# Runki2018/litehandnet

Hardware: AMD Instinct MI355X
Metric: images/sec fwd+bwd @256x256 bs64 litehandnet (higher is better)
Workload: dtype f32; 1 GPU; litehandnet variant B (MSRB hourglass litehourglass.py) C=128, 256x256x3 -> 21x64x64, per-GPU batch 64, train-mode BN, fwd + TopdownHeatmapLoss + bwd + fused Adam; global_batch=64, parallelism=dp1

## Files before the change

### include/lhn.h

```cpp
#ifndef LHN_H
#define LHN_H
#include <stdint.h>
#ifdef __cplusplus
extern "C" {
#endif

#define LHN_VERSION 3
#define LHN_STAT_REPLICAS 32

typedef struct lhn_view {
  float*       data;
  const float* table;
  const float* gate;
  int32_t N, H, W;
  int32_t cstride;
  int32_t coff;
  int32_t C;
  const void* pend;
} lhn_view;

typedef struct lhn_gradview {
  const float* dz;
  const float* dpool;
  const float* coef;
// ... 190 lines not shown
                   void* stream);

int lhn_att_mlp_fwd(const float* pooled, const float* gamma, const float* beta, float* rmean, float* rvar,
                    int64_t* nbt, const float* w3 , const float* b3, const float* wl ,
                    const float* bl, const float* dropmask , float* gate, int gate_stride,
                    int gate_coff, float* save, int N, int C, float eps, float momentum, int training, int stage,
                    double* gsum, double count_scale, void* stream);
int lhn_att_mlp_bwd(const float* pooled, const float* gamma, const float* beta, const float* w3, const float* wl,
                    const float* dropmask, float* save, const float* dgate , float* dpool, int cstride,
                    int coff, int H, int W, float* dgamma, float* dbeta, float* dw3, float* db3, float* dwl,
                    float* dbl, int N, int C, int stage, double* gsum, double count_scale, float pgrad_scale,
                    void* stream);

int lhn_se_mlp_fwd(const float* pooled, const float* w1 , const float* b1, const float* w2 ,
                   const float* b2, float* gate, int gate_stride, int gate_coff, float* save, int N, int C, int J,
                   void* stream);
int lhn_se_mlp_fwd2(const float* pooled, const float* w1, const float* b1, const float* w2, const float* b2, float* gate,
                    int gate_stride, int gate_coff, float* save, int N, int C, int J, int mode, void* stream);
int lhn_se_mlp_bwd2(const float* pooled, const float* w1, const float* w2, const float* save, const float* dgate,
                    float* dpool, int cstride, int coff, int H, int W, float* dw1, float* db1, float* dw2, float* db2, int N,
                    int C, int J, int mode, void* stream);
int lhn_se_mlp_bwd(const float* pooled, const float* w1, const float* w2, const float* save, const float* dgate ,
                   float* dpool , int cstride, int coff, int H, int W, float* dw1, float* db1, float* dw2,
                   float* db2, int N, int C, int J, void* stream);

int lhn_bn_bwd_reduce(const lhn_view* y, const lhn_gradview* g, const float* save_mean_invstd,
                      double* sums , const lhn_bnbwdfin* fin , void* stream);
int lhn_bn_bwd_finalize(const double* sums, const float* gamma, const float* save_mean_invstd,
                        float* coef, int cstride, int coff, int C, double count, float* dgamma, float* dbeta,
                        float pgrad_scale , void* stream);
int lhn_bn_bwd_finalize2(const double* sums, const float* gamma, const float* save_mean_invstd, float* coef, int cstride,
                         int coff, int C, int stat_channels, double count, float* dgamma, float* dbeta, float pgrad_scale,
                         void* stream);
int lhn_conv_pw_bwd(const lhn_view* x, const float* w, const lhn_view* y, const lhn_gradview* gy,
                    float* dx , int dx_accumulate, float* dw,
                    float* dbias, int stride, const float* dy_nchw, int nrep, int64_t rep_stride, void* stream);
int lhn_conv_pw_bwd2(const lhn_view* x, const float* w, const lhn_view* y, const lhn_gradview* gy, float* dx,
                     int dx_accumulate, float* dw, float* dbias, int stride, const float* dy_nchw, int nrep, int64_t rep_stride,
                     const lhn_pw_opts* opts, void* stream);
int lhn_conv_dw_bwd(const lhn_view* x, const float* w, const lhn_view* y, const lhn_gradview* gy, float* dx,
                    int dx_accumulate, float* dw, int k, int stride, int pad, int dil, int nrep, int64_t rep_stride,
                    void* stream);
int lhn_conv_dw_bwd2(const lhn_view* x, const float* w, const lhn_view* y, const lhn_gradview* gy, float* dx, int dx_accumulate,
                     float* dw, int k, int stride, int pad, int dil, int nrep, int64_t rep_stride, double* bn_sums,
                     const float* bn_save, int bn_C, int bn_coff, void* stream);
int lhn_conv_dw_bwd3(const lhn_view* x, const float* w, const lhn_view* y, const lhn_gradview* gy, float* dx, int dx_accumulate,
                     float* dw, int k, int stride, int pad, int dil, int nrep, int64_t rep_stride, const float* dx_add0,
                     const float* dx_add1, void* stream);
int lhn_conv_stem_bwd(const float* img, const lhn_view* y, const lhn_gradview* gy, float* dw, int Hi, int Wi,
                      int k, int stride, int pad, int nrep, int64_t rep_stride, void* stream);
int lhn_conv_kxk_bwd(const lhn_view* x, const float* w, const lhn_view* y, const lhn_gradview* gy, float* dx,
                     int dx_accumulate, float* dw, int stride, int nrep, int64_t rep_stride,
                     float* wt_scratch , void* stream);
int lhn_plan_run_range(void* plan, int phase, int64_t step_begin, int64_t step_end, void* workspace,
                       void* const* params, void* const* grads, void* const* io, int training, int grad_replicas,
                       int64_t grad_rep_stride, double count_scale, float pgrad_scale, void* stream);
int lhn_fold_stat_replicas(double* stats, int64_t n, int nrep, void* stream);
int lhn_reduce_replicas(float* out, const float* part, int64_t n, int nrep, int64_t rep_stride, void* stream);
int lhn_ew_bwd(const lhn_view* srcs, int nsrc, const lhn_view* dst, const float* ddst, float out_slope,
               float* const* dsrcs, const int* accumulate, void* stream);
int lhn_ew_bwd2(const lhn_view* src, const lhn_view* dst, const float* ddst, const float* dst_dpool, float out_slope,
                float* dsrc, int accumulate, void* stream);
int lhn_maxpool2_bwd(const lhn_view* x, const lhn_view* y, const float* dy, float* dx, int dx_accumulate,
                     void* stream);
int lhn_maxpool2_bwd2(const lhn_view* x, const lhn_view* y, const float* dy, float* dx, int dx_accumulate, const lhn_bnsum* bns,
                      void* stream);
int lhn_maxpool2_bwd3(const lhn_view* x, const lhn_view* y, const float* dy, float* dx, int dx_accumulate, const lhn_bnsum* bns,
                      const lhn_grad_adds* adds , void* stream);
int lhn_ew_bwd3(const lhn_view* src, const lhn_view* dst, const float* ddst, const float* dst_dpool, float out_slope, float* dsrc,
                int accumulate, const lhn_bnsum* bns, void* stream);
int lhn_ew_bwd_multi(const lhn_view* srcs, int nsrc, const lhn_view* dst, const float* ddst, const float* dst_dpool, float out_slope,
                     float* const* dsrcs, const int* accumulate, const lhn_bnsum* const* bns, void* stream);
int lhn_avgpool_bwd3(const lhn_view* x, const float* dout, int OH, int OW, int out_cstride, int out_coff, float* dx,
                     int dx_accumulate, const lhn_bnsum* bns, void* stream);
int lhn_conv_pw_bwd3(const lhn_view* x, const float* w, const lhn_view* y, const lhn_gradview* gy, float* dx, int dx_accumulate,
                     float* dw, float* dbias, int stride, const float* dy_nchw, int nrep, int64_t rep_stride,
                     const lhn_pw_opts* opts, const lhn_bnsum* bns , void* stream);
int lhn_conv_dw_bwd4(const lhn_view* x, const float* w, const lhn_view* y, const lhn_gradview* gy, float* dx, int dx_accumulate,
                     float* dw, int k, int stride, int pad, int dil, int nrep, int64_t rep_stride, const lhn_bnsum* bns,
                     const float* dx_add0, const float* dx_add1, const lhn_bnbwdsrc* fin, void* stream);
int lhn_conv_pw_bwd4(const lhn_view* x, const float* w, const lhn_view* y, const lhn_gradview* gy, float* dx, int dx_accumulate,
                     float* dw, float* dbias, int stride, const float* dy_nchw, int nrep, int64_t rep_stride,
                     const lhn_pw_opts* opts, const lhn_bnsum* bns, const lhn_bnbwdsrc* fin, void* stream);
int lhn_avgpool_bwd(const lhn_view* x, const float* dout , int OH, int OW, float* dx,
                    int dx_accumulate, void* stream);
int lhn_gate_bwd_reduce(const lhn_view* y, const float* dz, float* dgate , void* stream);
typedef struct lhn_bn_slices {
  const float* save[2];
  double*      sums[2];
  int32_t      lo[2], C[2];
  int32_t      n;
} lhn_bn_slices;
int lhn_gate_bwd_reduce2(const lhn_view* y, const float* dz, float* dgate , float* tsum,
                         const lhn_bn_slices* slices, void* stream);
int lhn_gate_bwd_reduce3(const lhn_view* y, const float* dz, float* dgate, float* tsum, const lhn_bn_slices* slices, int prezeroed,
                         void* stream);
typedef struct lhn_gatesum {
  float*               dgate;
  const lhn_bn_slices* slices;
} lhn_gatesum;
int lhn_conv_pw_bwd5(const lhn_view* x, const float* w, const lhn_view* y, const lhn_gradview* gy, float* dx, int dx_accumulate,
                     float* dw, float* dbias, int stride, const float* dy_nchw, int nrep, int64_t rep_stride,
                     const lhn_pw_opts* opts, const lhn_bnsum* bns, const lhn_bnbwdsrc* fin, const lhn_gatesum* gs, void* stream);
#define LHN_PW_BWD_DZ_DEAD 1
int lhn_conv_pw_bwd6(const lhn_view* x, const float* w, const lhn_view* y, const lhn_gradview* gy, float* dx, int dx_accumulate,
                     float* dw, float* dbias, int stride, const float* dy_nchw, int nrep, int64_t rep_stride,
                     const lhn_pw_opts* opts, const lhn_bnsum* bns, const lhn_bnbwdsrc* fin, const lhn_gatesum* gs, int flags,
                     void* stream);
int lhn_avgpool_fwd3(const lhn_view* x, float* out , int OH, int OW, float* pstat ,
                     const lhn_bn_slices* slices, void* stream);
int lhn_ca_mlp_bwd2(const float* pooled, const float* w3, const float* gamma, const float* w1, const float* w2,
                    const float* dropmask, const float* save, const float* dgate, float* dpool, int cstride, int coff, int H,
                    int W, float* dw3, float* dgamma, float* dbeta, float* dw1, float* db1, float* dw2, float* db2, int N, int C,
                    int stage, double* gsum, double count_scale, float pgrad_scale, const float* tsum, const float* pstat,
                    const lhn_bn_slices* slices, void* stream);
int lhn_avgpool_fwd4(const lhn_view* x, float* out, int OH, int OW, float* pstat, const lhn_bn_slices* slices,
                     const lhn_view* copy_src, void* stream);
int lhn_ca_mlp_bwd(const float* pooled, const float* w3, const float* gamma, const float* w1, const float* w2,
                   const float* dropmask, const float* save, const float* dgate, float* dpool ,
                   int cstride, int coff, int H, int W, float* dw3, float* dgamma, float* dbeta, float* dw1,
                   float* db1, float* dw2, float* db2, int N, int C, int stage, double* gsum, double count_scale,
                   float pgrad_scale, void* stream);

int lhn_cbam_layout(int N, int H, int W, int C, int64_t* save_off , int64_t* scratch_off );
int lhn_cbam_fwd(const lhn_view* p, const lhn_view* r, const float* w1, const float* w2, const float* w7, const lhn_view* out,
                 float* save, void* stream);
int lhn_cbam_bwd(const lhn_view* p, const lhn_view* r, const float* w1, const float* w2, const float* w7, const lhn_view* out,
                 const float* dout, float* dp, float* dr, float* dw1, float* dw2, float* dw7, const float* save, float* scratch,
                 void* stream);

int lhn_adam_step(float* param, const float* grad, float* exp_avg, float* exp_avg_sq, int64_t n, double lr, double beta1,
                  double beta2, double eps, double weight_decay, int64_t step, void* stream);

typedef struct lhn_op {
  int32_t kind;
  int32_t in_buf[3], in_coff[3], in_C[3];
  int32_t reserved[6];
  int32_t out_buf, out_coff, out_C;
  int32_t p[12];
  int64_t ws[12];
  int32_t i[8];
  float   f[8];
} lhn_op;

typedef struct lhn_buf {
  int64_t data_off, table_off, gate_off, grad_off, dpool_off, coef_off;
  int32_t N, H, W, C;
} lhn_buf;

void* lhn_plan_create(const lhn_buf* bufs, int nbufs, const lhn_op* fwd, int nfwd, const lhn_op* bwd, int nbwd);
void  lhn_plan_destroy(void* plan);
int   lhn_plan_head_gate_fold(void* plan);
int   lhn_plan_pw_dz_dead(void* plan, int bwd_index);
#define LHN_RUN_TABLES_CURRENT 2
#define LHN_RUN_GRAPH 4
int   lhn_plan_run(void* plan, int phase, void* workspace, void* const* params, void* const* grads,
                   void* const* io, int training, int grad_replicas, int64_t grad_rep_stride, void* stream);

#ifdef __cplusplus
}
#endif
#endif
```

### litehandnet_amd/_lib.py

```python
import ctypes as C
import os

import torch

_HERE = os.path.dirname(os.path.abspath(__file__))
LIB_PATH = os.path.join(_HERE, "liblhn.so")
_lib = None


class LhnError(RuntimeError):
    pass


class View(C.Structure):
    _fields_ = [("data", C.c_void_p), ("table", C.c_void_p), ("gate", C.c_void_p),
                ("N", C.c_int32), ("H", C.c_int32), ("W", C.c_int32),
                ("cstride", C.c_int32), ("coff", C.c_int32), ("C", C.c_int32), ("pend", C.c_void_p)]


class GradView(C.Structure):
    _fields_ = [("dz", C.c_void_p), ("dpool", C.c_void_p), ("coef", C.c_void_p)]


class Op(C.Structure):
    _fields_ = [("kind", C.c_int32),
                ("in_buf", C.c_int32 * 3), ("in_coff", C.c_int32 * 3), ("in_C", C.c_int32 * 3), ("reserved", C.c_int32 * 6),
                ("out_buf", C.c_int32), ("out_coff", C.c_int32), ("out_C", C.c_int32),
                ("p", C.c_int32 * 12), ("ws", C.c_int64 * 12), ("i", C.c_int32 * 8), ("f", C.c_float * 8)]


class Buf(C.Structure):
    _fields_ = [("data_off", C.c_int64), ("table_off", C.c_int64), ("gate_off", C.c_int64),
                ("grad_off", C.c_int64), ("dpool_off", C.c_int64), ("coef_off", C.c_int64),
                ("N", C.c_int32), ("H", C.c_int32), ("W", C.c_int32), ("C", C.c_int32)]


SYMBOLS = [
    "lhn_version", "lhn_deterministic", "lhn_last_error", "lhn_device_ok",
    "lhn_heatmap_encode", "lhn_heatmap_argmax", "lhn_heatmap_refine", "lhn_transform_preds",
    "lhn_heatmap_decode", "lhn_heatmap_decode_dark", "lhn_heatmap_decode_dark_udp", "lhn_heatmap_nms", "lhn_heatmap_topk", "lhn_pck_accuracy",
    "lhn_eval_state_bytes", "lhn_eval_accumulate", "lhn_eval_finalize",
    "lhn_loss_balanced_mse_fwd", "lhn_loss_balanced_mse_bwd", "lhn_affine_warp_normalize", "lhn_affine_warp_normalize2", "lhn_random_flip", "lhn_hsv_jitter", "lhn_simdr_encode", "lhn_simdr_loss_fwd", "lhn_simdr_loss_bwd",
    "lhn_conv_pw_fwd", "lhn_conv_pw_fwd2", "lhn_conv_pw_bwd2", "lhn_conv_dw_fwd", "lhn_conv_dw_fwd2", "lhn_conv_dw_fwd3", "lhn_conv_pw_dw3_fwd", "lhn_conv_dw3_pw_fwd", "lhn_msrb_round_scratch_bytes", "lhn_msrb_round_fwd", "lhn_bottleneck_fwd", "lhn_stem_tail_fwd", "lhn_conv_stem_fwd", "lhn_conv_kxk_fwd", "lhn_conv_kxk_fwd_bf16x3",
    "lhn_bn_finalize", "lhn_table_fill", "lhn_table_bias", "lhn_fold_bn", "lhn_ew_fwd", "lhn_ew_fwd2", "lhn_ew_fwd3", "lhn_ew_mul_bwd", "lhn_bilinear_bwd", "lhn_shuffle2_fwd", "lhn_shuffle2_bwd", "lhn_bn_finalize2", "lhn_bn_bwd_finalize2", "lhn_maxpool2_fwd", "lhn_avgpool_fwd", "lhn_avgpool_fwd2", "lhn_avgpool_bwd2", "lhn_se_mlp_fwd2", "lhn_se_mlp_bwd2", "lhn_ca_mlp_fwd", "lhn_att_mlp_fwd", "lhn_att_mlp_bwd", "lhn_se_mlp_fwd", "lhn_se_mlp_bwd",
    "lhn_bn_bwd_reduce", "lhn_bn_bwd_finalize", "lhn_conv_pw_bwd", "lhn_conv_dw_bwd", "lhn_conv_dw_bwd2", "lhn_conv_dw_bwd3", "lhn_conv_dw_bwd4", "lhn_conv_pw_bwd4", "lhn_conv_pw_bwd5", "lhn_conv_pw_bwd6", "lhn_plan_head_gate_fold", "lhn_plan_pw_dz_dead", "lhn_conv_stem_bwd",
    "lhn_conv_kxk_bwd", "lhn_ew_bwd", "lhn_ew_bwd2", "lhn_maxpool2_bwd", "lhn_maxpool2_bwd2", "lhn_maxpool2_bwd3", "lhn_ew_bwd3", "lhn_ew_bwd_multi", "lhn_avgpool_bwd3", "lhn_conv_pw_bwd3", "lhn_avgpool_bwd", "lhn_gate_bwd_reduce", "lhn_gate_bwd_reduce2", "lhn_gate_bwd_reduce3", "lhn_adam_step", "lhn_avgpool_fwd3", "lhn_avgpool_fwd4", "lhn_ca_mlp_bwd2",
    "lhn_ca_mlp_bwd", "lhn_reduce_replicas", "lhn_fold_stat_replicas", "lhn_plan_create", "lhn_plan_destroy", "lhn_plan_run", "lhn_plan_run_range",
    "lhn_cbam_layout", "lhn_cbam_fwd", "lhn_cbam_bwd",
]


def lib():
    global _lib
    if _lib is None:
        if not os.path.exists(LIB_PATH):
            raise LhnError(f"{LIB_PATH} is missing: run `python -m litehandnet_amd.build` "
                           "(hipcc --offload-arch=gfx950); there is no CPU fallback")
        _lib = C.CDLL(LIB_PATH)
        _lib.lhn_last_error.restype = C.c_char_p
        _lib.lhn_plan_create.restype = C.c_void_p
        _lib.lhn_plan_destroy.restype = None
        _lib.lhn_eval_state_bytes.restype = C.c_int64
        _lib.lhn_conv_dw3_pw_fwd.argtypes = [C.c_void_p, C.c_void_p, C.c_int, C.c_void_p, C.c_void_p, C.c_void_p, C.c_void_p, C.c_void_p]
        _lib.lhn_conv_dw3_pw_fwd.restype = C.c_int
        _lib.lhn_msrb_round_scratch_bytes.argtypes = [C.c_int, C.c_int, C.c_int, C.c_int]
        _lib.lhn_msrb_round_scratch_bytes.restype = C.c_int64
        _lib.lhn_msrb_round_fwd.argtypes = [C.c_void_p, C.c_void_p, C.c_void_p, C.c_void_p, C.c_void_p, C.c_void_p, C.c_void_p, C.c_int, C.c_int,
                                            C.c_void_p, C.c_void_p]
        _lib.lhn_msrb_round_fwd.restype = C.c_int
        _lib.lhn_bottleneck_fwd.argtypes = [C.c_void_p, C.c_int] + [C.c_void_p] * 8 + [C.c_float, C.c_void_p, C.c_void_p, C.c_void_p]
        _lib.lhn_bottleneck_fwd.restype = C.c_int
        _lib.lhn_stem_tail_fwd.argtypes = [C.c_void_p, C.c_int] + [C.c_void_p] * 14
        _lib.lhn_stem_tail_fwd.restype = C.c_int
        _lib.lhn_conv_kxk_fwd_bf16x3.argtypes = [C.c_void_p, C.c_void_p, C.c_void_p, C.c_void_p, C.c_int, C.c_void_p]
        _lib.lhn_conv_kxk_fwd_bf16x3.restype = C.c_int
        _lib.lhn_cbam_layout.argtypes = [C.c_int, C.c_int, C.c_int, C.c_int, C.c_void_p, C.c_void_p]
        _lib.lhn_cbam_layout.restype = C.c_int
        _lib.lhn_cbam_fwd.argtypes = [C.c_void_p] * 8
        _lib.lhn_cbam_fwd.restype = C.c_int
        _lib.lhn_cbam_bwd.argtypes = [C.c_void_p] * 15
        _lib.lhn_cbam_bwd.restype = C.c_int
    return _lib


def cbam_layout(N, H, W, Cc):
    sv, sc = (C.c_int64 * 10)(), (C.c_int64 * 8)()
    check(lib().lhn_cbam_layout(N, H, W, Cc, sv, sc), "lhn_cbam_layout")
    return list(sv), list(sc)


def check(status, what=""):
    if status != 0:
        raise LhnError(f"{what}: status {status}: {lib().lhn_last_error().decode()}")


def require_device(t=None):
    if not torch.cuda.is_available():
        raise LhnError("no GPU visible: litehandnet_amd has no CPU fallback")
    if t is not None and not t.is_cuda:
        raise LhnError("tensor must live on the GPU (litehandnet_amd has no CPU fallback)")


def ptr(t):
    return C.c_void_p(0) if t is None else C.c_void_p(t.data_ptr())


def stream():
    return C.c_void_p(torch.cuda.current_stream().cuda_stream)


def f32c(t, name="tensor"):
    require_device(t)
    if t.dtype != torch.float32:
        t = t.float()
    return t.contiguous()
```

### litehandnet_amd/csrc/k_conv_dw.hip

```cpp
#include <stdlib.h>
#include "lhn_common.h"

template <int K>
__global__ void __launch_bounds__(256) k_dw_fwd(lhn_view x, const float* __restrict__ w, lhn_view y,
                                                double* __restrict__ stats, int stride, int pad, int dil, lhn_bnfin fin,
                                                int ) {
  extern __shared__ __attribute__((aligned(16))) float smem[];
  const int C = x.C, C4 = C >> 2;
  constexpr int KK = K * K;
  float* Ws = smem;
  f4* red = reinterpret_cast<f4*>(smem + KK * C);
  const int tid = threadIdx.x;
  const int c4 = tid % C4, pl = tid / C4, PL = 256 / C4;
  const int cin = x.coff + 4 * c4, cout = y.coff + 4 * c4;
  const Xf4 xf = lhn_load_xf(x, cin);
  for (int i = tid; i < KK * C; i += 256) {
    const int c = i / KK, t = i - c * KK;
    Ws[t * C + c] = w ? w[i] : 1.f;
  }
  __syncthreads();
  f4 wt[KK];
#pragma unroll
  for (int t = 0; t < KK; ++t) wt[t] = *reinterpret_cast<const f4*>(Ws + t * C + 4 * c4);
  const int rows = y.N * y.H;
// ... 210 lines not shown
      for (int r = 0; r < 16; ++r) {
        const int64_t pix = pbase + (r & 3) + 8 * (r >> 2);
        if (pix < total) {
          y.data[pix * y.cstride + y.coff + l31] = acc[r];
          if (cnt == 0) kk = acc[r];
          const float d = acc[r] - kk;
          s += d;
          q += d * d;
          ++cnt;
        }
      }
    }
  }
  if (stats) {
    const double k0 = kk, c0 = cnt;
    double sd = (double)s + c0 * k0, qd = (double)q + 2.0 * k0 * (double)s + c0 * k0 * k0;
    sd += __shfl_xor(sd, 32, 64);
    qd += __shfl_xor(qd, 32, 64);
    if (lh == 0) {
      redd[wave][l31] = sd;
      redd[wave][CO + l31] = qd;
    }
    __syncthreads();
    if (tid < 2 * CO) {
      double* st = stats + (size_t)(blockIdx.x % LHN_STAT_REPLICAS) * 2 * CO;
      atomicAdd(st + tid, redd[0][tid] + redd[1][tid] + redd[2][tid] + redd[3][tid]);
    }
    if (fin.counter && lhn_last_block(fin.counter)) lhn_bn_finalize_block(fin, stats);
  }
}


__global__ void __launch_bounds__(256, 2) k_stem7_fwd_mfma(const float* __restrict__ img, const float* __restrict__ w, lhn_view y,
                                                        double* __restrict__ stats, int Hi, int Wi, int stride, int pad, lhn_bnfin fin) {
  constexpr int CO = 64, T = 147, TP = 160, NKS = TP / 2, LDV = TP + 4, BMP = 64, G = 4, NR = 6, NV = NR * 7;
  extern __shared__ __attribute__((aligned(16))) float smem[];
  float* Vs = smem;
  double* redd = reinterpret_cast<double*>(smem + BMP * LDV);
  const int tid = threadIdx.x, lane = tid & 63, wave = __builtin_amdgcn_readfirstlane(tid >> 6), l31 = lane & 31, lh = lane >> 5;
  const int cot = wave & 1, pg = wave >> 1, co = cot * 32 + l31;
  float wreg[NKS];
#pragma unroll
  for (int ks = 0; ks < NKS; ++ks) {
    const int tap = NKS * lh + ks;
    wreg[ks] = tap < T ? w[co * T + tap] : 0.f;
  }
  const int p = tid & (BMP - 1), g = tid >> 6;
  for (int t = T + g; t < TP; t += G) Vs[p * LDV + t] = 0.f;
  const int64_t total = (int64_t)y.N * y.H * y.W;
  const int64_t ntiles = (total + BMP - 1) / BMP;
  float v[NV];
  auto issue = [&](int64_t tile) __attribute__((always_inline)) {
    const int64_t pix = tile * BMP + p;
    const int64_t pc = pix < total ? pix : total - 1;
    const int wo = (int)(pc % y.W);
    const int64_t r = pc / y.W;
    const int ho = (int)(r % y.H), n = (int)(r / y.H);
    const float* base = img + (int64_t)n * 3 * Hi * Wi;
    const int iw0 = wo * stride - pad;
#pragma unroll
    for (int jr = 0; jr < NR; ++jr) {
      const int row = min(g + G * jr, 20), c = row / 7, kh = row - 7 * c;
      const int ih = ho * stride - pad + kh, ihc = min(max(ih, 0), Hi - 1);
      const float* rb = base + ((int64_t)c * Hi + ihc) * Wi;
#pragma unroll
      for (int kw = 0; kw < 7; ++kw) {
        const int iw = iw0 + kw, iwc = min(max(iw, 0), Wi - 1);
        const float q = rb[iwc];
        v[jr * 7 + kw] = (ih == ihc && iw == iwc) ? q : 0.f;
      }
    }
  };
  float s = 0.f, q = 0.f, kk = 0.f;
  int cnt = 0;
  int64_t tile = blockIdx.x;
  if (tile < ntiles) issue(tile);
  for (; tile < ntiles; tile += gridDim.x) {
    __syncthreads();
#pragma unroll
    for (int jr = 0; jr < NR; ++jr)
      if (g + G * jr < 21)
#pragma unroll
        for (int kw = 0; kw < 7; ++kw) Vs[p * LDV + (g + G * jr) * 7 + kw] = v[jr * 7 + kw];
    __syncthreads();
    if (tile + gridDim.x < ntiles) issue(tile + gridDim.x);
    const f4* ap = reinterpret_cast<const f4*>(Vs + (pg * 32 + l31) * LDV + NKS * lh);
    f16v acc;
#pragma unroll
    for (int r = 0; r < 16; ++r) acc[r] = 0.f;
#pragma unroll
    for (int c = 0; c < NKS / 4; ++c) {
      if ((c & 3) == 0) asm volatile("" ::: "memory");
      const f4 a = ap[c];
      acc = __builtin_amdgcn_mfma_f32_32x32x2f32(a.x, wreg[4 * c + 0], acc, 0, 0, 0);
      acc = __builtin_amdgcn_mfma_f32_32x32x2f32(a.y, wreg[4 * c + 1], acc, 0, 0, 0);
      acc = __builtin_amdgcn_mfma_f32_32x32x2f32(a.z, wreg[4 * c + 2], acc, 0, 0, 0);
      acc = __builtin_amdgcn_mfma_f32_32x32x2f32(a.w, wreg[4 * c + 3], acc, 0, 0, 0);
    }
    const int64_t pbase = tile * BMP + pg * 32 + 4 * lh;
#pragma unroll
    for (int r = 0; r < 16; ++r) {
      const int64_t pix = pbase + (r & 3) + 8 * (r >> 2);
      if (pix < total) {
        y.data[pix * y.cstride + y.coff + co] = acc[r];
        if (cnt == 0) kk = acc[r];
        const float d = acc[r] - kk;
        s += d;
        q += d * d;
        ++cnt;
      }
    }
  }
  if (stats) {
    const double k0 = kk, c0 = cnt;
    double sd = (double)s + c0 * k0, qd = (double)q + 2.0 * k0 * (double)s + c0 * k0 * k0;
    sd += __shfl_xor(sd, 32, 64);
    qd += __shfl_xor(qd, 32, 64);
    __syncthreads();
    if (lh == 0) {
      redd[pg * 2 * CO + co] = sd;
      redd[pg * 2 * CO + CO + co] = qd;
    }
    __syncthreads();
    if (tid < 2 * CO) {
      double* st = stats + (size_t)(blockIdx.x % LHN_STAT_REPLICAS) * 2 * CO;
      atomicAdd(st + tid, redd[tid] + redd[2 * CO + tid]);
    }
    if (fin.counter && lhn_last_block(fin.counter)) lhn_bn_finalize_block(fin, stats);
  }
}

static inline int grid_for(int64_t items_per_block_total, int per_block, int cap_per_cu) {
  int64_t g = (items_per_block_total + per_block - 1) / per_block;
  const int64_t cap = (int64_t)lhn_num_cus() * cap_per_cu;
  if (g > cap) g = cap;
  if (g < 1) g = 1;
  return (int)g;
}
static inline bool pow2(int v) { return v > 0 && (v & (v - 1)) == 0; }

struct DwExtra {
  lhn_view v;
  float coef[2];
  int n;
  float* sum_out;
  int so_cstride, so_coff;
};

int lhn_dwk_fwd_lds(const lhn_view* x, const float* w, const lhn_view* y, double* stats, int k, int dil, lhn_bnfin fin,
                    hipStream_t s, const DwExtra* ex);
struct DwBnSum;
static int dws2_fwd(const lhn_view* x, const float* w, const lhn_view* y, double* stats, lhn_bnfin fin, hipStream_t s);
static int dws2_bwd(const lhn_view* x, const float* w, const lhn_view* y, const lhn_gradview* gy, float* dx, int dx_acc, float* dw,
                    int nrep, int64_t rep_stride, hipStream_t s);
int lhn_dwk_bwd_lds(const lhn_view* x, const float* w, const lhn_view* y, const lhn_gradview* gy, float* dx, int dx_acc,
                    float* dw, int k, int dil, int nrep, int64_t rep_stride, hipStream_t s, const DwBnSum* bs,
                    const lhn_bnbwdsrc* fs = nullptr);
static bool lhn_dw_bwd_v1();
static bool lhn_dw_force_gather() {
  static int v = -1;
  if (v < 0) {
    const char* e = getenv("LHN_DW_GATHER");
    v = (e && e[0] == '1') ? 1 : 0;
  }
  return v == 1;
}

static int dw_fwd_extra(const lhn_view* x, const float* w, const lhn_view* y, double* stats, int k, int stride, int pad, int dil,
                        lhn_bnfin fin, const lhn_view* extra, const float* coef, const lhn_view* so, hipStream_t s);

extern "C" int lhn_conv_dw_fwd3(const lhn_view* x, const float* w, const lhn_view* y, double* stats, int k, int stride,
                                int pad, int dil, const lhn_bnfin* finp, const lhn_view* extra, const float* coef2,
                                const lhn_view* sum_out, void* stream) {
  if (!extra) {
    LHN_CHECK_ARG(!sum_out, "lhn_conv_dw_fwd3: sum_out without a second source");
    return lhn_conv_dw_fwd(x, w, y, stats, k, stride, pad, dil, finp, stream);
  }
  lhn_bnfin fin;
  if (finp && stats) fin = *finp; else fin.counter = nullptr;
  LHN_CHECK_ARG(lhn_view_ok(x) && lhn_view_ok(y) && lhn_view_ok(extra) && w && coef2, "lhn_conv_dw_fwd2: bad view / null pointer");
  LHN_CHECK_ARG(extra->C == x->C && extra->N == x->N && extra->H == x->H && extra->W == x->W, "lhn_conv_dw_fwd2: extra source geometry");
  LHN_CHECK_ARG(x->C == y->C && y->N == x->N && y->H == x->H && y->W == x->W, "lhn_conv_dw_fwd2: same-size output");
  LHN_CHECK_ARG(!sum_out || (sum_out->data && sum_out->C == x->C && sum_out->N == x->N && sum_out->H == x->H && sum_out->W == x->W &&
                             sum_out->cstride % 4 == 0 && sum_out->coff % 4 == 0 && sum_out->coff + sum_out->C <= sum_out->cstride),
                "lhn_conv_dw_fwd3: sum_out geometry (same pixels and channels as x)");
  const int rc = dw_fwd_extra(x, w, y, stats, k, stride, pad, dil, fin, extra, coef2, sum_out, (hipStream_t)stream);
  LHN_CHECK_ARG(rc == 1, "lhn_conv_dw_fwd2: a second source needs k=3, stride 1, 'same' padding, W >= 8 (got k=%d s=%d C=%d W=%d)",
                k, stride, x->C, y->W);
  LHN_CHECK_LAUNCH("lhn_conv_dw_fwd2");
  return 0;
}

extern "C" int lhn_conv_dw_fwd2(const lhn_view* x, const float* w, const lhn_view* y, double* stats, int k, int stride,
                                int pad, int dil, const lhn_bnfin* finp, const lhn_view* extra, const float* coef2, void* stream) {
  return lhn_conv_dw_fwd3(x, w, y, stats, k, stride, pad, dil, finp, extra, coef2, nullptr, stream);
}

extern "C" int lhn_conv_dw_fwd(const lhn_view* x, const float* w, const lhn_view* y, double* stats, int k, int stride,
                               int pad, int dil, const lhn_bnfin* finp, void* stream) {
  lhn_bnfin fin;
  if (finp && stats) fin = *finp; else fin.counter = nullptr;
  LHN_CHECK_ARG(lhn_view_ok(x) && lhn_view_ok(y) && (w || k == 1), "lhn_conv_dw_fwd: bad view / null pointer (w may be NULL = ones only for k=1)");
  LHN_CHECK_ARG(x->C == y->C && x->C % 4 == 0 && x->C <= 512, "lhn_conv_dw_fwd: channels %d -> %d (multiple of 4, <= 512)", x->C, y->C);
  LHN_CHECK_ARG((k == 1 || k == 3 || k == 5 || k == 7) && stride >= 1 && dil >= 1 && pad >= 0, "lhn_conv_dw_fwd: k=%d stride=%d dil=%d", k, stride, dil);
  const int Ho = (x->H + 2 * pad - dil * (k - 1) - 1) / stride + 1, Wo = (x->W + 2 * pad - dil * (k - 1) - 1) / stride + 1;
  LHN_CHECK_ARG(y->N == x->N && y->H == Ho && y->W == Wo, "lhn_conv_dw_fwd: output %dx%d, expected %dx%d", y->H, y->W, Ho, Wo);
  const size_t lds = (size_t)(k * k * x->C) * 4 + 256 * 2 * 16;
  const int grid = grid_for((int64_t)y->N * Ho, 1, 8);
  hipStream_t s = (hipStream_t)stream;
  LHN_CHECK_ARG(lhn_no_pend(x), "lhn_conv_dw_fwd: lhn_view.pend is reserved (NULL)");
  const int px = 0;
  DwExtra ex0;
  ex0.n = 0;
  ex0.sum_out = nullptr;
  if (w && stride == 1 && pad == dil * (k - 1) / 2 && x->C % 4 == 0 && y->W >= 8 && !lhn_dw_force_gather() &&
      lhn_dwk_fwd_lds(x, w, y, stats, k, dil, fin, s, &ex0)) {
  } else if (w && k == 3 && stride == 2 && pad == 1 && dil == 1 && x->C % 4 == 0 && !lhn_dw_force_gather() &&
             dws2_fwd(x, w, y, stats, fin, s)) {
  } else if (k == 3)
    hipLaunchKernelGGL((k_dw_fwd<3>), dim3(grid), dim3(256), lds, s, *x, w, *y, stats, stride, pad, dil, fin, px);
  else if (k == 7)
    hipLaunchKernelGGL((k_dw_fwd<7>), dim3(grid), dim3(256), lds, s, *x, w, *y, stats, stride, pad, dil, fin, px);
  else if (k == 1)
    hipLaunchKernelGGL((k_dw_fwd<1>), dim3(grid), dim3(256), lds, s, *x, w, *y, stats, stride, pad, dil, fin, px);
  else if (k == 5)
    hipLaunchKernelGGL((k_dw_fwd<5>), dim3(grid), dim3(256), lds, s, *x, w, *y, stats, stride, pad, dil, fin, px);
  LHN_CHECK_LAUNCH("lhn_conv_dw_fwd");
  return 0;
}

extern "C" int lhn_conv_stem_fwd(const float* img, const float* w, const lhn_view* y, double* stats, int Hi, int Wi, int k,
                                 int stride, int pad, const lhn_bnfin* finp, void* stream) {
  lhn_bnfin fin;
  if (finp && stats) fin = *finp; else fin.counter = nullptr;
  LHN_CHECK_ARG(img && w && lhn_view_ok(y), "lhn_conv_stem_fwd: bad view / null pointer");
  LHN_CHECK_ARG(y->C % 8 == 0 && pow2(y->C / 8) && y->C <= 256, "lhn_conv_stem_fwd: Cout=%d", y->C);
  LHN_CHECK_ARG((k == 1 || k == 3 || k == 5 || k == 7) && stride >= 1, "lhn_conv_stem_fwd: k=%d", k);
  const int Ho = (Hi + 2 * pad - k) / stride + 1, Wo = (Wi + 2 * pad - k) / stride + 1;
  LHN_CHECK_ARG(y->H == Ho && y->W == Wo, "lhn_conv_stem_fwd: output %dx%d, expected %dx%d", y->H, y->W, Ho, Wo);
  const int PL = 256 / (y->C / 8);
  const size_t lds = (size_t)(3 * k * k * y->C) * 4 + 256 * 16 * 4;
  const bool mfma = !lhn_dw_force_gather() && ((k == 7 && y->C == 64) || (k == 3 && y->C == 32));
  LHN_CHECK_ARG(mfma || lds <= 65536, "lhn_conv_stem_fwd: k=%d Cout=%d needs %zu B of LDS (limit 65536 B)", k, y->C, lds);
  if (k == 7 && y->C == 64 && !lhn_dw_force_gather()) {
    const size_t lds7 = (size_t)64 * 164 * 4 + 2 * 2 * 64 * 8;
    static LhnKernelCfg cfg7;
    int per_cu = 1;
    if (!lhn_kernel_cfg(cfg7, &k_stem7_fwd_mfma, lds7, 3, &per_cu)) {
      lhn_set_error("lhn_conv_stem_fwd: cannot reserve %zu B of LDS", lds7);
      return 2;
    }
    const int64_t ntiles = ((int64_t)y->N * Ho * Wo + 63) / 64;
    int grid = lhn_num_cus() * per_cu;
    if (grid > ntiles) grid = (int)ntiles;
    hipLaunchKernelGGL(k_stem7_fwd_mfma, dim3(grid), dim3(256), lds7, (hipStream_t)stream, img, w, *y, stats, Hi, Wi, stride, pad, fin);
  } else if (k == 3 && y->C == 32 && !lhn_dw_force_gather()) {
    hipLaunchKernelGGL(k_stem3_fwd_mfma, dim3(grid_for((int64_t)y->N * Ho * Wo, 256, 3)), dim3(256), 0, (hipStream_t)stream, img, w, *y,
                       stats, Hi, Wi, stride, pad, fin);
  } else
    hipLaunchKernelGGL(k_stem_fwd, dim3(grid_for((int64_t)y->N * Ho * Wo, PL, 8)), dim3(256), lds, (hipStream_t)stream, img,
                       w, *y, stats, Hi, Wi, k, stride, pad, fin);
  LHN_CHECK_LAUNCH("lhn_conv_stem_fwd");
  return 0;
}

__device__ __forceinline__ f4 dw_load_dy(const lhn_view& y, const lhn_gradview& g, const Xf4& xf, const Gr4& gr,
                                         int64_t pix, int n, int h, int w, int ca) {
  const f4 raw = *reinterpret_cast<const f4*>(y.data + pix * y.cstride + ca);
  const f4 dz = *reinterpret_cast<const f4*>(g.dz + pix * y.cstride + ca);
  const f4 du = lhn_grad_du(y, g, xf, raw, dz, n, h, w, ca);
  return gr.A * du + gr.B * raw + gr.Cc;
}

__device__ __forceinline__ f4 dw_dy_at(const lhn_view& y, const lhn_gradview& g, const Xf4& xf, const Gr4& gr, f4 gate,
                                       size_t off, int n, int h, int w, int ca) {
  const f4 raw = *reinterpret_cast<const f4*>(y.data + off);
  f4 e = *reinterpret_cast<const f4*>(g.dz + off) * gate;
  const f4 u = raw * xf.sc + xf.sh;
  const f4 dl = (f4){u.x > 0.f ? 1.f : xf.sl.x, u.y > 0.f ? 1.f : xf.sl.y, u.z > 0.f ? 1.f : xf.sl.z, u.w > 0.f ? 1.f : xf.sl.w};
  if (g.dpool) e += lhn_dpool_sum(g, y, n, h, w, ca);
  const f4 du = e * dl;
  return gr.A * du + gr.B * raw + gr.Cc;
}

template <int K>
__global__ void __launch_bounds__(256) k_dw_bwd_data(lhn_view x, const float* __restrict__ w, lhn_view y, lhn_gradview gy,
                                                     float* __restrict__ dx, int accumulate, int stride, int pad, int dil) {
  extern __shared__ __attribute__((aligned(16))) float smem[];
  const int C = x.C, C4 = C >> 2;
  constexpr int KK = K * K;
  float* Ws = smem;
  const int tid = threadIdx.x;
  for (int i = tid; i < KK * C; i += 256) {
    const int c = i / KK, t = i - c * KK;
    Ws[t * C + c] = w ? w[i] : 1.f;
  }
  __syncthreads();
  const int c4 = tid % C4, pl = tid / C4, PL = 256 / C4;
  const int cx = x.coff + 4 * c4, cy = y.coff + 4 * c4;
  const Xf4 yxf = lhn_load_xf(y, cy);
  const Gr4 ygr = lhn_load_coef(gy, y.cstride, cy);
  f4 wt[KK];
#pragma unroll
  for (int t = 0; t < KK; ++t) wt[t] = *reinterpret_cast<const f4*>(Ws + t * C + 4 * c4);
  const int rows = x.N * x.H;
  for (int row = blockIdx.x; row < rows; row += gridDim.x) {
    const int n = row / x.H, hi = row - n * x.H;
// ... 184 lines not shown
#pragma unroll
        for (int kw = 0; kw < 3; ++kw) {
          const int iw = wo * stride - pad + kw, iwc = min(max(iw, 0), Wi - 1);
          const float t = plane[(int64_t)ihc * Wi + iwc];
          v[c * 9 + kh * 3 + kw] = (ih == ihc && iw == iwc) ? t : 0.f;
        }
      }
    }
  };
  int64_t tile = blockIdx.x;
  if (tile < ntiles) issue(tile);
  for (; tile < ntiles; tile += gridDim.x) {
    __syncthreads();
#pragma unroll
    for (int j = 0; j < 8; ++j) {
      const int p = prow + 32 * j;
      const int64_t pix = tile * 256 + p;
      f4 d = (f4){0.f, 0.f, 0.f, 0.f};
      if (pix < total) {
        const int wo = (int)(pix % y.W);
        const int64_t r = pix / y.W;
        const f4 du = lhn_grad_du(y, gy, yxf, yraw[j], zraw[j], (int)(r / y.H), (int)(r % y.H), wo, cy);
        d = ygr.A * du + ygr.B * yraw[j] + ygr.Cc;
      }
      *reinterpret_cast<f4*>(dYs + p * LDY + 4 * c4) = d;
    }
#pragma unroll
    for (int t = 0; t < 27; ++t) Vs[tid * LDV + t] = v[t];
    __syncthreads();
    if (tile + gridDim.x < ntiles) issue(tile + gridDim.x);
    const float* ar = dYs + (wave * 64 + lh) * LDY + l31;
    const float* br = Vs + (wave * 64 + lh) * LDV + l31;
#pragma unroll 8
    for (int ks = 0; ks < 32; ++ks) acc = __builtin_amdgcn_mfma_f32_32x32x2f32(ar[2 * ks * LDY], br[2 * ks * LDV], acc, 0, 0, 0);
  }
  __syncthreads();
  float* part = dYs;
#pragma unroll
  for (int r = 0; r < 16; ++r) part[(wave * 16 + r) * 64 + lane] = acc[r];
  __syncthreads();
  dw += (size_t)(blockIdx.x % nrep) * rep_stride;
  for (int i = tid; i < CO * 27; i += 256) {
    const int co = i / 27, t = i - co * 27;
    const int r = (co & 3) + 4 * (co >> 3), ln = t + 32 * ((co >> 2) & 1);
    const float v = part[(0 * 16 + r) * 64 + ln] + part[(1 * 16 + r) * 64 + ln] + part[(2 * 16 + r) * 64 + ln] + part[(3 * 16 + r) * 64 + ln];
    atomicAdd(dw + i, v);
  }
}


__global__ void __launch_bounds__(256, 2) k_stem7_bwd_mfma(const float* __restrict__ img, lhn_view y, lhn_gradview gy, float* __restrict__ dw,
                                                           int Hi, int Wi, int stride, int pad, int nrep, int64_t rep_stride) {
  constexpr int CO = 64, T = 147, LDY = CO + 4, LDV = 161, BMP = 64, G = 4, NR = 6;
  extern __shared__ __attribute__((aligned(16))) float smem[];
  float* dYs = smem;
  float* Vs = smem + BMP * LDY;
  const int tid = threadIdx.x, lane = tid & 63, wave = __builtin_amdgcn_readfirstlane(tid >> 6), l31 = lane & 31, lh = lane >> 5;
  const int c4 = tid & 15, prow = tid >> 4;
  const int cy = y.coff + 4 * c4;
  const Xf4 yxf = lhn_load_xf(y, cy);
  const Gr4 ygr = lhn_load_coef(gy, y.cstride, cy);
  const int p = tid & (BMP - 1), g = tid >> 6;
  for (int t = T + g; t < 160; t += G) Vs[p * LDV + t] = 0.f;
  f16v acc[3];
#pragma unroll
  for (int i = 0; i < 3; ++i)
#pragma unroll
    for (int r = 0; r < 16; ++r) acc[i][r] = 0.f;
  const int64_t total = (int64_t)y.N * y.H * y.W;
  const int64_t ntiles = (total + BMP - 1) / BMP;
  f4 yraw[4], zraw[4];
  float v[NR * 7];
  auto issue = [&](int64_t tile) __attribute__((always_inline)) {
#pragma unroll
    for (int j = 0; j < 4; ++j) {
      int64_t pix = tile * BMP + prow + 16 * j;
      pix = pix < total ? pix : total - 1;
      yraw[j] = *reinterpret_cast<const f4*>(y.data + pix * y.cstride + cy);
      zraw[j] = *reinterpret_cast<const f4*>(gy.dz + pix * y.cstride + cy);
    }
    const int64_t pix = tile * BMP + p;
    const int64_t pc = pix < total ? pix : total - 1;
    const int wo = (int)(pc % y.W);
    const int64_t r = pc / y.W;
    const int ho = (int)(r % y.H), n = (int)(r / y.H);
    const float* base = img + (int64_t)n * 3 * Hi * Wi;
    const int iw0 = wo * stride - pad;
#pragma unroll
    for (int jr = 0; jr < NR; ++jr) {
      const int row = min(g + G * jr, 20), c = row / 7, kh = row - 7 * c;
      const int ih = ho * stride - pad + kh, ihc = min(max(ih, 0), Hi - 1);
      const float* rb = base + ((int64_t)c * Hi + ihc) * Wi;
#pragma unroll
      for (int kw = 0; kw < 7; ++kw) {
        const int iw = iw0 + kw, iwc = min(max(iw, 0), Wi - 1);
        const float q = rb[iwc];
        v[jr * 7 + kw] = (ih == ihc && iw == iwc) ? q : 0.f;
      }
    }
  };
  int64_t tile = blockIdx.x;
  if (tile < ntiles) issue(tile);
  for (; tile < ntiles; tile += gridDim.x) {
    __syncthreads();
#pragma unroll
    for (int j = 0; j < 4; ++j) {
      const int pp = prow + 16 * j;
      const int64_t pix = tile * BMP + pp;
      f4 d = (f4){0.f, 0.f, 0.f, 0.f};
      if (pix < total) {
        const int wo = (int)(pix % y.W);
        const int64_t r = pix / y.W;
        const f4 du = lhn_grad_du(y, gy, yxf, yraw[j], zraw[j], (int)(r / y.H), (int)(r % y.H), wo, cy);
        d = ygr.A * du + ygr.B * yraw[j] + ygr.Cc;
      }
      *reinterpret_cast<f4*>(dYs + pp * LDY + 4 * c4) = d;
    }
#pragma unroll
    for (int jr = 0; jr < NR; ++jr)
      if (g + G * jr < 21)
#pragma unroll
        for (int kw = 0; kw < 7; ++kw) Vs[p * LDV + (g + G * jr) * 7 + kw] = v[jr * 7 + kw];
    __syncthreads();
    if (tile + gridDim.x < ntiles) issue(tile + gridDim.x);
#pragma unroll
    for (int i = 0; i < 3; ++i) {
      const int job = wave + 4 * i;
      if (job < 10) {
        const float* ar = dYs + lh * LDY + (job & 1) * 32 + l31;
        const float* br = Vs + lh * LDV + (job >> 1) * 32 + l31;
#pragma unroll 8
        for (int ks = 0; ks < 32; ++ks) acc[i] = __builtin_amdgcn_mfma_f32_32x32x2f32(ar[2 * ks * LDY], br[2 * ks * LDV], acc[i], 0, 0, 0);
      }
    }
  }
  dw += (size_t)(blockIdx.x % nrep) * rep_stride;
#pragma unroll
  for (int i = 0; i < 3; ++i) {
    const int job = wave + 4 * i;
    if (job < 10) {
      const int t = (job >> 1) * 32 + l31;
#pragma unroll
      for (int r = 0; r < 16; ++r) {
        const int co = (job & 1) * 32 + (r & 3) + 8 * (r >> 2) + 4 * lh;
        if (t < T) atomicAdd(dw + co * T + t, acc[i][r]);
      }
    }
  }
}

static int dw_bwd_fused(const lhn_view* x, const float* w, const lhn_view* y, const lhn_gradview* gy, float* dx, float* dw, int k,
                        int dil, int nrep, int64_t rep_stride, double* bn_sums, const float* bn_save, int bn_C, int bn_coff, hipStream_t s);

extern "C" int lhn_conv_dw_bwd2(const lhn_view* x, const float* w, const lhn_view* y, const lhn_gradview* gy, float* dx,
                                int dx_accumulate, float* dw, int k, int stride, int pad, int dil, int nrep, int64_t rep_stride,
                                double* bn_sums, const float* bn_save, int bn_C, int bn_coff, void* stream) {
  if (!bn_sums) return lhn_conv_dw_bwd(x, w, y, gy, dx, dx_accumulate, dw, k, stride, pad, dil, nrep, rep_stride, stream);
  if (nrep < 1) nrep = 1;
  LHN_CHECK_ARG(lhn_view_ok(x) && lhn_view_ok(y) && gy && gy->dz && w && dw && dx && bn_save && lhn_no_pend(x) && lhn_no_pend(y),
                "lhn_conv_dw_bwd2: bad view / null pointer");
  LHN_CHECK_ARG(!dx_accumulate && !x->gate && stride == 1 && pad == dil * (k - 1) / 2 && x->C % 32 == 0 && x->W >= 8 && x->C == y->C &&
                    bn_coff >= 0 && bn_coff + x->C <= bn_C,
                "lhn_conv_dw_bwd2: fused BatchNorm sums need this convolution to be the only, ungated, stride-1 reader of x (dx stored)");
  const int rc = dw_bwd_fused(x, w, y, gy, dx, dw, k, dil, nrep, rep_stride, bn_sums, bn_save, bn_C, bn_coff, (hipStream_t)stream);
  LHN_CHECK_ARG(rc == 1, "lhn_conv_dw_bwd2: fused BatchNorm sums are built for the 3x3 / dilation 1 kernel (k=%d dil=%d)", k, dil);
  LHN_CHECK_LAUNCH("lhn_conv_dw_bwd2");
  return 0;
}

static int dw_bwd_addends(const lhn_view* x, const float* w, const lhn_view* y, const lhn_gradview* gy, float* dx, int dx_acc, float* dw,
                          int k, int dil, int nrep, int64_t rep_stride, const float* a0, const float* a1, hipStream_t s);

extern "C" int lhn_conv_dw_bwd3(const lhn_view* x, const float* w, const lhn_view* y, const lhn_gradview* gy, float* dx,
                                int dx_accumulate, float* dw, int k, int stride, int pad, int dil, int nrep, int64_t rep_stride,
                                const float* dx_add0, const float* dx_add1, void* stream) {
  if (!dx_add0 && !dx_add1) return lhn_conv_dw_bwd(x, w, y, gy, dx, dx_accumulate, dw, k, stride, pad, dil, nrep, rep_stride, stream);
  if (nrep < 1) nrep = 1;
  LHN_CHECK_ARG(lhn_view_ok(x) && lhn_view_ok(y) && gy && gy->dz && w && dw && dx && lhn_no_pend(x) && lhn_no_pend(y),
                "lhn_conv_dw_bwd3: bad view / null pointer");
  LHN_CHECK_ARG(stride == 1 && pad == dil * (k - 1) / 2 && x->C % 4 == 0 && x->W >= 8 && x->C == y->C,
                "lhn_conv_dw_bwd3: gradient addends need the tiled stride-1 kernel (W >= 8)");
  const int rc = dw_bwd_addends(x, w, y, gy, dx, dx_accumulate, dw, k, dil, nrep, rep_stride, dx_add0 ? dx_add0 : dx_add1,
                                dx_add0 ? dx_add1 : nullptr, (hipStream_t)stream);
  LHN_CHECK_ARG(rc == 1, "lhn_conv_dw_bwd3: no tiled kernel for k=%d dil=%d", k, dil);
  LHN_CHECK_LAUNCH("lhn_conv_dw_bwd3");
  return 0;
}

extern "C" int lhn_conv_dw_bwd(const lhn_view* x, const float* w, const lhn_view* y, const lhn_gradview* gy, float* dx,
                               int dx_accumulate, float* dw, int k, int stride, int pad, int dil, int nrep, int64_t rep_stride,
                               void* stream) {
  if (nrep < 1) nrep = 1;
  LHN_CHECK_ARG(lhn_view_ok(x) && lhn_view_ok(y) && gy && gy->dz && ((w && dw) || k == 1) && lhn_no_pend(x) && lhn_no_pend(y), "lhn_conv_dw_bwd: bad view / null pointer");
  LHN_CHECK_ARG(x->C == y->C && x->C % 4 == 0 && x->C <= 512, "lhn_conv_dw_bwd: channels");
  LHN_CHECK_ARG(k == 1 || k == 3 || k == 7, "lhn_conv_dw_bwd: k=%d (1, 3 or 7)", k);
  hipStream_t s = (hipStream_t)stream;
  if (w && dw && stride == 1 && pad == dil * (k - 1) / 2 && x->C % 4 == 0 && x->W >= 8 && !lhn_dw_force_gather() &&
      lhn_dwk_bwd_lds(x, w, y, gy, dx, dx_accumulate, dw, k, dil, nrep, rep_stride, s, nullptr)) {
    LHN_CHECK_LAUNCH("lhn_conv_dw_bwd");
    return 0;
  }
  if (w && dw && k == 3 && stride == 2 && pad == 1 && dil == 1 && x->C % 4 == 0 && !lhn_dw_force_gather() &&
      dws2_bwd(x, w, y, gy, dx, dx_accumulate, dw, nrep, rep_stride, s)) {
    LHN_CHECK_LAUNCH("lhn_conv_dw_bwd");
    return 0;
  }
  if (dx) {
    const size_t lds = (size_t)(k * k * x->C) * 4;
    const int g = grid_for((int64_t)x->N * x->H, 1, 8);
    if (k == 3)
      hipLaunchKernelGGL((k_dw_bwd_data<3>), dim3(g), dim3(256), lds, s, *x, w, *y, *gy, dx, dx_accumulate, stride, pad, dil);
    else if (k == 1)
      hipLaunchKernelGGL((k_dw_bwd_data<1>), dim3(g), dim3(256), lds, s, *x, w, *y, *gy, dx, dx_accumulate, stride, pad, dil);
    else
      hipLaunchKernelGGL((k_dw_bwd_data<7>), dim3(g), dim3(256), lds, s, *x, w, *y, *gy, dx, dx_accumulate, stride, pad, dil);
  }
  const int gw = grid_for((int64_t)y->N * y->H, 1, 4);
  if (!dw) {
  } else if (k == 1) {
    hipLaunchKernelGGL((k_dw_bwd_weight<1, 1>), dim3(gw), dim3(256), 0, s, *x, *y, *gy, dw, stride, pad, dil, 0, nrep, rep_stride);
  } else if (k == 3) {
    hipLaunchKernelGGL((k_dw_bwd_weight<3, 3>), dim3(gw), dim3(256), 0, s, *x, *y, *gy, dw, stride, pad, dil, 0, nrep, rep_stride);
  } else {
    for (int kh = 0; kh < 7; ++kh)
      hipLaunchKernelGGL((k_dw_bwd_weight<7, 1>), dim3(gw), dim3(256), 0, s, *x, *y, *gy, dw, stride, pad, dil, kh, nrep, rep_stride);
  }
  LHN_CHECK_LAUNCH("lhn_conv_dw_bwd");
  return 0;
}

static int dw_bwd_fin(const lhn_view* x, const float* w, const lhn_view* y, const lhn_gradview* gy, float* dx, int dx_acc, float* dw, int k,
                      int dil, int nrep, int64_t rep_stride, const lhn_bnsum* bns, const float* a0, const float* a1, const lhn_bnbwdsrc* fin,
                      hipStream_t s);
static bool dw_bwd_folds(const lhn_view* x, const float* w, const float* dw, int k, int stride, int pad, int dil, bool has_ext) {
  return w && dw && k == 3 && stride == 1 && (dil == 1 || dil == 2) && pad == dil && x->C % 4 == 0 && x->W >= 8 && !lhn_dw_bwd_v1() &&
         (has_ext || !lhn_dw_force_gather());
}
extern "C" int lhn_conv_dw_bwd4(const lhn_view* x, const float* w, const lhn_view* y, const lhn_gradview* gy, float* dx,
                                int dx_accumulate, float* dw, int k, int stride, int pad, int dil, int nrep, int64_t rep_stride,
                                const lhn_bnsum* bns, const float* dx_add0, const float* dx_add1, const lhn_bnbwdsrc* fin,
                                void* stream) {
  const bool has_bns = bns && bns->sums, has_add = dx_add0 || dx_add1;
  LHN_CHECK_ARG(!(has_bns && has_add), "lhn_conv_dw_bwd4: producer sums and gradient addends exclude each other");
  const bool folds = fin && fin->sums;
  if (folds) {
    LHN_CHECK_ARG(lhn_view_ok(x) && lhn_view_ok(y) && gy && gy->dz && gy->coef && fin->save_mean_invstd && fin->count > 0 &&
                      fin->stat_channels >= y->C && x->C == y->C && lhn_no_pend(x) && lhn_no_pend(y),
                  "lhn_conv_dw_bwd4: finalize source needs gy->coef, saved statistics and stat_channels >= C");
    if (!dw_bwd_folds(x, w, dw, k, stride, pad, dil, has_bns || has_add)) {
      const int rc = lhn_bn_bwd_finalize2(fin->sums, fin->gamma, fin->save_mean_invstd, const_cast<float*>(gy->coef), y->cstride, y->coff,
                                          y->C, fin->stat_channels, fin->count, fin->dgamma, fin->dbeta, fin->pgrad_scale, stream);
      if (rc) return rc;
    }
  }
  if (!folds || !dw_bwd_folds(x, w, dw, k, stride, pad, dil, has_bns || has_add)) {
    if (has_add) return lhn_conv_dw_bwd3(x, w, y, gy, dx, dx_accumulate, dw, k, stride, pad, dil, nrep, rep_stride, dx_add0, dx_add1, stream);
    return lhn_conv_dw_bwd2(x, w, y, gy, dx, dx_accumulate, dw, k, stride, pad, dil, nrep, rep_stride, has_bns ? bns->sums : nullptr,
                            has_bns ? bns->save : nullptr, has_bns ? bns->C : 0, has_bns ? bns->coff : 0, stream);
  }
  if (nrep < 1) nrep = 1;
  LHN_CHECK_ARG(x->C <= 512 && (!has_add || dx), "lhn_conv_dw_bwd4: channels / addends without dx");
  if (has_bns)
    LHN_CHECK_ARG(dx && bns->save && !dx_accumulate && !x->gate && dil == 1 && x->C % 32 == 0 && bns->coff >= 0 && bns->coff + x->C <= bns->C,
                  "lhn_conv_dw_bwd4: fused BatchNorm sums need this convolution to be the only, ungated, stride-1 reader of x (dx stored, dilation 1)");
  const int rc = dw_bwd_fin(x, w, y, gy, dx, dx_accumulate, dw, k, dil, nrep, rep_stride, has_bns ? bns : nullptr, dx_add0 ? dx_add0 : dx_add1,
                            dx_add0 ? dx_add1 : nullptr, fin, (hipStream_t)stream);
  LHN_CHECK_ARG(rc == 1, "lhn_conv_dw_bwd4: no row kernel for k=%d dil=%d", k, dil);
  LHN_CHECK_LAUNCH("lhn_conv_dw_bwd4");
  return 0;
}

extern "C" int lhn_conv_stem_bwd(const float* img, const lhn_view* y, const lhn_gradview* gy, float* dw, int Hi, int Wi, int k,
                                 int stride, int pad, int nrep, int64_t rep_stride, void* stream) {
  if (nrep < 1) nrep = 1;
  LHN_CHECK_ARG(img && lhn_view_ok(y) && gy && gy->dz && dw, "lhn_conv_stem_bwd: bad view / null pointer");
  LHN_CHECK_ARG(pow2(y->C / 4) && y->C <= 256 && (k == 1 || k == 3 || k == 7), "lhn_conv_stem_bwd: Cout=%d k=%d", y->C, k);
  const int PL = 256 / (y->C / 4);
  const int g = grid_for((int64_t)y->N * y->H * y->W, PL, 4);
  if (k == 7 && y->C == 64 && !lhn_dw_force_gather()) {
    const size_t lds = (size_t)64 * (68 + 161) * 4;
    static LhnKernelCfg cfg7;
    int per_cu = 1;
    if (!lhn_kernel_cfg(cfg7, &k_stem7_bwd_mfma, lds, 2, &per_cu)) {
      lhn_set_error("lhn_conv_stem_bwd: cannot reserve %zu B of LDS", lds);
      return 2;
    }
    const int64_t ntiles = ((int64_t)y->N * y->H * y->W + 63) / 64;
    int grid = lhn_num_cus() * per_cu;
    if (grid > ntiles) grid = (int)ntiles;
    hipLaunchKernelGGL(k_stem7_bwd_mfma, dim3(grid), dim3(256), lds, (hipStream_t)stream, img, *y, *gy, dw, Hi, Wi, stride, pad, nrep, rep_stride);
  } else if (k == 3 && y->C == 32 && !lhn_dw_force_gather()) {
    const size_t lds = (size_t)256 * (36 + 33) * 4;
    static LhnKernelCfg cfg;
    int per_cu = 1;
    if (!lhn_kernel_cfg(cfg, &k_stem3_bwd_mfma, lds, 2, &per_cu)) {
      lhn_set_error("lhn_conv_stem_bwd: cannot reserve %zu B of LDS", lds);
      return 2;
    }
    const int64_t ntiles = ((int64_t)y->N * y->H * y->W + 255) / 256;
    int grid = lhn_num_cus() * per_cu;
    if (grid > ntiles) grid = (int)ntiles;
    hipLaunchKernelGGL(k_stem3_bwd_mfma, dim3(grid), dim3(256), lds, (hipStream_t)stream, img, *y, *gy, dw, Hi, Wi, stride, pad, nrep, rep_stride);
  } else if (k == 3)
    hipLaunchKernelGGL((k_stem_bwd<3, 3>), dim3(g), dim3(256), 0, (hipStream_t)stream, img, *y, *gy, dw, Hi, Wi, stride, pad, nrep, rep_stride, 0);
  else if (k == 1)
    hipLaunchKernelGGL((k_stem_bwd<1, 1>), dim3(g), dim3(256), 0, (hipStream_t)stream, img, *y, *gy, dw, Hi, Wi, stride, pad, nrep, rep_stride, 0);
  else
    for (int kh = 0; kh < 7; ++kh)
      hipLaunchKernelGGL((k_stem_bwd<7, 1>), dim3(g), dim3(256), 0, (hipStream_t)stream, img, *y, *gy, dw, Hi, Wi, stride, pad, nrep, rep_stride, kh);
  LHN_CHECK_LAUNCH("lhn_conv_stem_bwd");
  return 0;
}

// ... 645 lines not shown
  const int per_cu = lds > 80 * 1024 ? 1 : (lds > 52 * 1024 ? 2 : 3);
  static LhnKernelCfg cfg;
  (void)lhn_kernel_cfg(cfg, &k_dwk_fwd_lds<K, DIL, NS>, lds, 4, nullptr);
  const int grid = dw3_grid(ntile, cg, per_cu * 2);
  hipLaunchKernelGGL((k_dwk_fwd_lds<K, DIL, NS>), dim3(grid), dim3(256), lds, s, *x, w, *y, stats, th, tw, cg, fin, ps, ex, dw3_xchunk(grid, cg));
}
template <int K, int DIL, bool BNS = false, bool FOLD = false>
static void launch_dwk_bwd(const lhn_view* x, const float* w, const lhn_view* y, const lhn_gradview* gy, float* dx, int dx_acc,
                           float* dw, int nrep, int64_t rep_stride, hipStream_t s, int ps = 1, const DwBnSum* bsp = nullptr,
                           const lhn_bnbwdsrc* fsp = nullptr) {
  constexpr int TH = 8, TW = 16, P = DIL * (K - 1) / 2;
  DwBnSum bs;
  if (bsp) bs = *bsp; else { bs.sums = nullptr; bs.save = nullptr; bs.C = bs.coff = 0; bs.add[0] = bs.add[1] = nullptr; }
  lhn_bnbwdsrc fs;
  if (FOLD && fsp) fs = *fsp; else memset(&fs, 0, sizeof(fs));
  const int cg = (x->C + 31) / 32;
  const int sh = (x->H + ps - 1) / ps, sw = (x->W + ps - 1) / ps;
  const int th = (sh + TH - 1) / TH, tw = (sw + TW - 1) / TW, ntile = x->N * ps * ps * th * tw * cg;
  const size_t lds = (size_t)((TH + 2 * P) * (TW + 2 * P) * 16 + 256 + 2 * K * K * 8 + (BNS ? TH * TW * 8 + 16 : 0) + (FOLD ? 24 : 0)) * 16;
  static LhnKernelCfg cfg;
  (void)lhn_kernel_cfg(cfg, &k_dwk_bwd_lds<K, DIL, BNS, FOLD>, lds, 4, nullptr);
  const int grid = dw3_grid(ntile, cg, 4);
  hipLaunchKernelGGL((k_dwk_bwd_lds<K, DIL, BNS, FOLD>), dim3(grid), dim3(256), lds, s, *x, w, *y, *gy, dx, dx_acc, dw, th, tw,
                     cg, nrep, rep_stride, ps, bs, dw3_xchunk(grid, cg), fs);
}
template <int DIL, bool BNS = false>
static void launch_dw3_bwd_rows(const lhn_view* x, const float* w, const lhn_view* y, const lhn_gradview* gy, float* dx, int dx_acc,
                                float* dw, int nrep, int64_t rep_stride, hipStream_t s, int ps = 1, const DwBnSum* bsp = nullptr,
                                const lhn_bnbwdsrc* fsp = nullptr) {
  constexpr int P = DIL, R = 2 * P + 2, WW = 32 + 2 * P;
  DwBnSum bs;
  if (bsp) bs = *bsp; else { bs.sums = nullptr; bs.save = nullptr; bs.C = bs.coff = 0; bs.add[0] = bs.add[1] = nullptr; }
  lhn_bnbwdsrc fs;
  if (fsp) fs = *fsp; else memset(&fs, 0, sizeof(fs));
  static_assert(R * WW * 8 * 16 >= 2 * LHN_FIN_THREADS * 8, "dy ring holds the replica fold's partials");
  const int cg = (x->C + 31) / 32;
  const int sh = (x->H + ps - 1) / ps, sw = (x->W + ps - 1) / ps;
  const int nstrips = (sw + 31) / 32;
  const size_t lds = (size_t)(2 * R * WW * 8 + 2 * 9 * 8 + 16 + (BNS ? R * 32 * 8 : 0)) * 16;
  static LhnKernelCfg cfg;
  int per_cu = 1;
  (void)lhn_kernel_cfg(cfg, &k_dw3_bwd_rows<DIL, BNS>, lds, 8, &per_cu);
  const int base = x->N * ps * ps * nstrips * cg;
  int nch = (lhn_num_cus() * per_cu + base - 1) / base;
  nch = std::max(1, std::min(nch, (sh + 7) / 8));
  const int CH = (sh + nch - 1) / nch;
  nch = (sh + CH - 1) / CH;
  const int ntile = base * nch;
  const int grid = dw3_grid(ntile, cg, per_cu);
  hipLaunchKernelGGL((k_dw3_bwd_rows<DIL, BNS>), dim3(grid), dim3(256), lds, s, *x, w, *y, *gy, dx, dx_acc, dw, nstrips, nch, CH, cg,
                     nrep, rep_stride, ps, bs, fs);
}
static bool lhn_dw_bwd_v1() {
  static int v = -1;
  if (v < 0) {
    const char* e = getenv("LHN_DW_BWD_V1");
    v = (e && e[0] == '1') ? 1 : 0;
  }
  return v == 1;
}
static bool dw_bwd_small(const lhn_view* x) {
  static int v = -1;
  if (v < 0) {
    const char* e = getenv("LHN_DW_BWD_SMALL");
    v = (e && e[0] == '0') ? 0 : 1;
  }
  return v == 1 && (int64_t)x->H * x->W <= 256;
}


struct DwS2 {
  static constexpr int TH = 4, TW = 16, XH = 2 * TH + 1, XW = 2 * TW + 1, XPIX = XH * XW, DH = TH + 1, DW = TW + 1, DPIX = DH * DW;
};

__global__ void __launch_bounds__(256) k_dws2_fwd_lds(lhn_view x, const float* __restrict__ w, lhn_view y, double* __restrict__ stats,
                                                      int tiles_h, int tiles_w, int cgroups, lhn_bnfin fin) {
  using T = DwS2;
  extern __shared__ __attribute__((aligned(16))) float smem[];
  f4* tx = reinterpret_cast<f4*>(smem);
  f4* red = tx + T::XPIX * 8;
  f4* wl = red + 512;
  const int tid = threadIdx.x, c4 = tid & 7, pl = tid >> 3;
  const int ntile = y.N * tiles_h * tiles_w * cgroups;
  const int cg = blockIdx.x % cgroups;
  const int cvalid = min(8, (x.C - cg * 32) >> 2);
  const bool cok = c4 < cvalid;
  const int c4e = cok ? c4 : 0;
  const int cin = x.coff + cg * 32 + 4 * c4e, cout = y.coff + cg * 32 + 4 * c4e;
  for (int i = tid; i < 72; i += 256) {
    const int k = i >> 3, cc = cg * 32 + 4 * min(i & 7, cvalid - 1);
    wl[i] = (f4){w[(cc + 0) * 9 + k], w[(cc + 1) * 9 + k], w[(cc + 2) * 9 + k], w[(cc + 3) * 9 + k]};
  }
  const Xf4 xf = lhn_load_xf(x, cin);
  double sd[4] = {0, 0, 0, 0}, qd[4] = {0, 0, 0, 0};
  constexpr int NIT = (T::XPIX + 31) / 32;
  for (int t = blockIdx.x; t < ntile; t += gridDim.x) {
    int r = t / cgroups;
    const int tw = r % tiles_w;
    r /= tiles_w;
    const int th = r % tiles_h, n = r / tiles_h;
    const int h0 = 2 * th * T::TH - 1, w0 = 2 * tw * T::TW - 1;
    const f4 gate = x.gate ? *reinterpret_cast<const f4*>(x.gate + (size_t)n * x.cstride + cin) : (f4){1.f, 1.f, 1.f, 1.f};
    const float* xin = x.data + (size_t)n * x.H * x.W * x.cstride + cin;
    f4 raw[NIT];
#pragma unroll
    for (int it = 0; it < NIT; ++it) {
      const int i = min(pl + 32 * it, T::XPIX - 1);
      const int ph = i / T::XW, pw = i - ph * T::XW;
      const int ih = min(max(h0 + ph, 0), x.H - 1), iw = min(max(w0 + pw, 0), x.W - 1);
      raw[it] = *reinterpret_cast<const f4*>(xin + ((size_t)ih * x.W + iw) * x.cstride);
    }
    __syncthreads();
#pragma unroll
    for (int it = 0; it < NIT; ++it) {
      const int i = pl + 32 * it;
      if (i < T::XPIX) {
        const int ph = i / T::XW, pw = i - ph * T::XW;
        const int ih = h0 + ph, iw = w0 + pw;
        const bool inb = ih >= 0 && ih < x.H && iw >= 0 && iw < x.W;
        tx[i * 8 + c4] = inb ? lhn_apply_xf(raw[it], xf) * gate : (f4){0.f, 0.f, 0.f, 0.f};
      }
    }
    __syncthreads();
    f4 s = (f4){0.f, 0.f, 0.f, 0.f}, q = s, kk = s;
    int cnt = 0;
#pragma unroll
    for (int j = 0; j < 2; ++j) {
      const int o = pl + 32 * j, oh = o / T::TW, ow = o - oh * T::TW;
      const int ho = th * T::TH + oh, wo = tw * T::TW + ow;
      if (cok && ho < y.H && wo < y.W) {
        f4 acc = (f4){0.f, 0.f, 0.f, 0.f};
#pragma unroll
        for (int a = 0; a < 3; ++a)
#pragma unroll
          for (int b = 0; b < 3; ++b) acc += tx[((2 * oh + a) * T::XW + 2 * ow + b) * 8 + c4] * wl[(a * 3 + b) * 8 + c4];
        *reinterpret_cast<f4*>(y.data + ((size_t)(n * y.H + ho) * y.W + wo) * y.cstride + cout) = acc;
        if (cnt == 0) kk = acc;
        const f4 d = acc - kk;
        s += d;
        q += d * d;
        ++cnt;
      }
    }
    lhn_unshift4(sd, qd, s, q, kk, cnt);
  }
  if (stats) {
    const int C = x.C;
    double* st = stats + (size_t)((blockIdx.x / cgroups) % LHN_STAT_REPLICAS) * 2 * C + cg * 32;
    lhn_block_stat_atomics_d(sd, qd, 8, reinterpret_cast<double*>(red), st, st + C, cvalid);
    if (fin.counter && lhn_last_block(fin.counter)) lhn_bn_finalize_block(fin, stats);
  }
}

__global__ void __launch_bounds__(256, 2) k_dws2_bwd_lds(lhn_view x, const float* __restrict__ w, lhn_view y, lhn_gradview gy,
                                                      float* __restrict__ dx, int dx_acc, float* __restrict__ dw, int tiles_h,
                                                      int tiles_w, int cgroups, int nrep, int64_t rep_stride) {
  using T = DwS2;
  extern __shared__ __attribute__((aligned(16))) float smem[];
  f4* tx = reinterpret_cast<f4*>(smem);
  f4* tdy = tx + T::XPIX * 8;
  f4* wl = tdy + T::DPIX * 8;
  const int tid = threadIdx.x, c4 = tid & 7, pl = tid >> 3;
  const int ntile = y.N * tiles_h * tiles_w * cgroups;
  const int cg = blockIdx.x % cgroups;
  const int cvalid = min(8, (x.C - cg * 32) >> 2);
  const bool cok = c4 < cvalid;
  const int c4e = cok ? c4 : 0;
  const int cx = x.coff + cg * 32 + 4 * c4e, cy = y.coff + cg * 32 + 4 * c4e;
  const Xf4 xxf = lhn_load_xf(x, cx), yxf = lhn_load_xf(y, cy);
  const Gr4 ygr = lhn_load_coef(gy, y.cstride, cy);
  for (int i = tid; i < 72; i += 256) {
    const int k = i >> 3, cc = cg * 32 + 4 * min(i & 7, cvalid - 1);
    wl[i] = (f4){w[(cc + 0) * 9 + k], w[(cc + 1) * 9 + k], w[(cc + 2) * 9 + k], w[(cc + 3) * 9 + k]};
  }
  f4 accw[9];
#pragma unroll
  for (int k = 0; k < 9; ++k) accw[k] = (f4){0.f, 0.f, 0.f, 0.f};
  constexpr int NITX = (T::XPIX + 31) / 32, NITD = (T::DPIX + 31) / 32;
  for (int t = blockIdx.x; t < ntile; t += gridDim.x) {
    int r = t / cgroups;
    const int tw = r % tiles_w;
    r /= tiles_w;
    const int th = r % tiles_h, n = r / tiles_h;
    const int h0 = 2 * th * T::TH - 1, w0 = 2 * tw * T::TW - 1;
    const int oh0 = th * T::TH, ow0 = tw * T::TW;
    const f4 xgate = x.gate ? *reinterpret_cast<const f4*>(x.gate + (size_t)n * x.cstride + cx) : (f4){1.f, 1.f, 1.f, 1.f};
    f4 rx[NITX], ry[NITD], rz[NITD];
#pragma unroll
    for (int it = 0; it < NITX; ++it) {
      const int i = min(pl + 32 * it, T::XPIX - 1);
      const int ph = i / T::XW, pw = i - ph * T::XW;
      const int ih = min(max(h0 + ph, 0), x.H - 1), iw = min(max(w0 + pw, 0), x.W - 1);
      rx[it] = *reinterpret_cast<const f4*>(x.data + ((size_t)(n * x.H + ih) * x.W + iw) * x.cstride + cx);
    }
#pragma unroll
    for (int it = 0; it < NITD; ++it) {
      const int i = min(pl + 32 * it, T::DPIX - 1);
      const int ph = i / T::DW, pw = i - ph * T::DW;
      const int ho = min(oh0 + ph, y.H - 1), wo = min(ow0 + pw, y.W - 1);
      const size_t off = ((size_t)(n * y.H + ho) * y.W + wo) * y.cstride + cy;
      ry[it] = *reinterpret_cast<const f4*>(y.data + off);
      rz[it] = *reinterpret_cast<const f4*>(gy.dz + off);
    }
    __syncthreads();
#pragma unroll
    for (int it = 0; it < NITX; ++it) {
      const int i = pl + 32 * it;
      if (i < T::XPIX) {
        const int ph = i / T::XW, pw = i - ph * T::XW;
        const int ih = h0 + ph, iw = w0 + pw;
        const bool inb = ih >= 0 && ih < x.H && iw >= 0 && iw < x.W;
        tx[i * 8 + c4] = inb ? lhn_apply_xf(rx[it], xxf) * xgate : (f4){0.f, 0.f, 0.f, 0.f};
      }
    }
#pragma unroll
    for (int it = 0; it < NITD; ++it) {
      const int i = pl + 32 * it;
      if (i < T::DPIX) {
        const int ph = i / T::DW, pw = i - ph * T::DW;
        const int ho = oh0 + ph, wo = ow0 + pw;
        f4 d = (f4){0.f, 0.f, 0.f, 0.f};
        if (ho < y.H && wo < y.W) {
          const f4 du = lhn_grad_du(y, gy, yxf, ry[it], rz[it], n, ho, wo, cy);
          d = ygr.A * du + ygr.B * ry[it] + ygr.Cc;
        }
        tdy[i * 8 + c4] = d;
      }
    }
    __syncthreads();
#pragma unroll
    for (int j = 0; j < 2; ++j) {
      const int o = pl + 32 * j, oh = o / T::TW, ow = o - oh * T::TW;
      const f4 dyc = tdy[(oh * T::DW + ow) * 8 + c4];
#pragma unroll
      for (int a = 0; a < 3; ++a)
#pragma unroll
        for (int b = 0; b < 3; ++b) accw[a * 3 + b] += dyc * tx[((2 * oh + a) * T::XW + 2 * ow + b) * 8 + c4];
    }
    if (dx && cok) {
      const int c = pl, iw = 2 * ow0 + c;
      const int nb = (c & 1) ? 2 : 1;
      const int bA = (c & 1) ? 0 : 1, colA = (c & 1) ? (c + 1) >> 1 : c >> 1, colB = (c - 1) >> 1;
      if (iw < x.W) {
#pragma unroll
        for (int rr = 0; rr < 2 * T::TH; ++rr) {
          const int ih = 2 * oh0 + rr;
          if (ih < x.H) {
            f4 accx = (f4){0.f, 0.f, 0.f, 0.f};
            if ((rr & 1) == 0) {
              const f4* drow = tdy + ((rr >> 1) * T::DW) * 8 + c4;
              accx += drow[colA * 8] * wl[(3 + bA) * 8 + c4];
              if (nb == 2) accx += drow[colB * 8] * wl[(3 + 2) * 8 + c4];
            } else {
              const f4* d0 = tdy + (((rr + 1) >> 1) * T::DW) * 8 + c4;
              const f4* d2 = tdy + (((rr - 1) >> 1) * T::DW) * 8 + c4;
              accx += d0[colA * 8] * wl[(0 + bA) * 8 + c4] + d2[colA * 8] * wl[(6 + bA) * 8 + c4];
              if (nb == 2) accx += d0[colB * 8] * wl[(0 + 2) * 8 + c4] + d2[colB * 8] * wl[(6 + 2) * 8 + c4];
            }
            float* o = dx + ((size_t)(n * x.H + ih) * x.W + iw) * x.cstride + cx;
            if (dx_acc) accx += *reinterpret_cast<const f4*>(o);
            *reinterpret_cast<f4*>(o) = accx;
          }
        }
      }
    }
  }
  float* dwr = dw + (size_t)((blockIdx.x / cgroups) % nrep) * rep_stride;
#pragma unroll
  for (int k = 0; k < 9; ++k)
#pragma unroll
    for (int o = 8; o < 64; o <<= 1) {
      accw[k].x += __shfl_xor(accw[k].x, o, 64);
      accw[k].y += __shfl_xor(accw[k].y, o, 64);
      accw[k].z += __shfl_xor(accw[k].z, o, 64);
      accw[k].w += __shfl_xor(accw[k].w, o, 64);
    }
  __syncthreads();
  if ((tid & 63) < 8)
#pragma unroll
    for (int k = 0; k < 9; ++k) tdy[(k * 4 + (tid >> 6)) * 8 + c4] = accw[k];
  __syncthreads();
  if (tid < 72) {
    const int k = tid >> 3, cc = tid & 7;
    const f4 sacc = tdy[(k * 4 + 0) * 8 + cc] + tdy[(k * 4 + 1) * 8 + cc] + tdy[(k * 4 + 2) * 8 + cc] + tdy[(k * 4 + 3) * 8 + cc];
    const int cb = cg * 32 + 4 * cc;
    if (cc < cvalid) {
      atomicAdd(dwr + (cb + 0) * 9 + k, sacc.x);
      atomicAdd(dwr + (cb + 1) * 9 + k, sacc.y);
      atomicAdd(dwr + (cb + 2) * 9 + k, sacc.z);
      atomicAdd(dwr + (cb + 3) * 9 + k, sacc.w);
    }
  }
}

static int dws2_fwd(const lhn_view* x, const float* w, const lhn_view* y, double* stats, lhn_bnfin fin, hipStream_t s) {
  using T = DwS2;
  const int cg = (x->C + 31) / 32;
  const int th = (y->H + T::TH - 1) / T::TH, tw = (y->W + T::TW - 1) / T::TW, ntile = y->N * th * tw * cg;
  size_t lds = (size_t)(T::XPIX * 8 + 512 + 72) * 16;
  static LhnKernelCfg cfg;
  if (!lhn_kernel_cfg(cfg, &k_dws2_fwd_lds, lds, 4, nullptr)) return 0;
  hipLaunchKernelGGL(k_dws2_fwd_lds, dim3(dw3_grid(ntile, cg, 6)), dim3(256), lds, s, *x, w, *y, stats, th, tw, cg, fin);
  return 1;
}
static int dws2_bwd(const lhn_view* x, const float* w, const lhn_view* y, const lhn_gradview* gy, float* dx, int dx_acc, float* dw,
                    int nrep, int64_t rep_stride, hipStream_t s) {
  using T = DwS2;
  const int cg = (x->C + 31) / 32;
  const int th = (y->H + T::TH - 1) / T::TH, tw = (y->W + T::TW - 1) / T::TW, ntile = y->N * th * tw * cg;
  const size_t lds = (size_t)((T::XPIX + T::DPIX) * 8 + 72) * 16;
  static LhnKernelCfg cfg;
  if (!lhn_kernel_cfg(cfg, &k_dws2_bwd_lds, lds, 4, nullptr)) return 0;
  hipLaunchKernelGGL(k_dws2_bwd_lds, dim3(dw3_grid(ntile, cg, 4)), dim3(256), lds, s, *x, w, *y, *gy, dx, dx_acc, dw, th, tw, cg, nrep, rep_stride);
  return 1;
}

int lhn_dwk_fwd_lds(const lhn_view* x, const float* w, const lhn_view* y, double* stats, int k, int dil, lhn_bnfin fin,
                    hipStream_t s, const DwExtra* ex) {
  if (ex && ex->n > 0) {
    if (k == 3 && dil == 1) launch_dwk_fwd<3, 1, 2>(x, w, y, stats, fin, s, 1, ex);
    else if (k == 3 && dil == 2 && y->W >= 16) launch_dwk_fwd<3, 1, 2>(x, w, y, stats, fin, s, 2, ex);
    else return 0;
    return 1;
  }
  if (k == 3 && dil == 1) launch_dwk_fwd<3, 1>(x, w, y, stats, fin, s, 1, ex);
  else if (k == 3 && dil == 2 && y->W >= 16) launch_dwk_fwd<3, 1>(x, w, y, stats, fin, s, 2, ex);
  else if (k == 3 && dil == 2) launch_dwk_fwd<3, 2>(x, w, y, stats, fin, s, 1, ex);
  else if (k == 7 && dil == 1) launch_dwk_fwd<7, 1>(x, w, y, stats, fin, s, 1, ex);
  else return 0;
  return 1;
}
int lhn_dwk_bwd_lds(const lhn_view* x, const float* w, const lhn_view* y, const lhn_gradview* gy, float* dx, int dx_acc,
                    float* dw, int k, int dil, int nrep, int64_t rep_stride, hipStream_t s, const DwBnSum* bs,
                    const lhn_bnbwdsrc* fs) {
  if (fs && (lhn_dw_bwd_v1() || k != 3)) return 0;
  const bool small = k == 3 && dil == 1 && dw_bwd_small(x);
  if (bs && bs->sums) {
    if (!(k == 3 && dil == 1 && dx && !dx_acc)) return 0;
    if (lhn_dw_bwd_v1()) launch_dwk_bwd<3, 1, true>(x, w, y, gy, dx, dx_acc, dw, nrep, rep_stride, s, 1, bs);
    else if (small) launch_dwk_bwd<3, 1, true, true>(x, w, y, gy, dx, dx_acc, dw, nrep, rep_stride, s, 1, bs, fs);
    else launch_dw3_bwd_rows<1, true>(x, w, y, gy, dx, dx_acc, dw, nrep, rep_stride, s, 1, bs, fs);
    return 1;
  }
  const bool v1 = lhn_dw_bwd_v1();
  if (k == 3 && dil == 1) {
    if (v1) launch_dwk_bwd<3, 1>(x, w, y, gy, dx, dx_acc, dw, nrep, rep_stride, s, 1, bs);
    else if (small) launch_dwk_bwd<3, 1, false, true>(x, w, y, gy, dx, dx_acc, dw, nrep, rep_stride, s, 1, bs, fs);
    else launch_dw3_bwd_rows<1>(x, w, y, gy, dx, dx_acc, dw, nrep, rep_stride, s, 1, bs, fs);
  } else if (k == 3 && dil == 2 && x->W >= 16) {
    if (v1) launch_dwk_bwd<3, 1>(x, w, y, gy, dx, dx_acc, dw, nrep, rep_stride, s, 2, bs);
    else launch_dw3_bwd_rows<1>(x, w, y, gy, dx, dx_acc, dw, nrep, rep_stride, s, 2, bs, fs);
  } else if (k == 3 && dil == 2) {
    if (v1) launch_dwk_bwd<3, 2>(x, w, y, gy, dx, dx_acc, dw, nrep, rep_stride, s, 1, bs);
    else launch_dw3_bwd_rows<2>(x, w, y, gy, dx, dx_acc, dw, nrep, rep_stride, s, 1, bs, fs);
  } else if (k == 7 && dil == 1) launch_dwk_bwd<7, 1>(x, w, y, gy, dx, dx_acc, dw, nrep, rep_stride, s, 1, bs);
  else return 0;
  return 1;
}

static int dw_fwd_extra(const lhn_view* x, const float* w, const lhn_view* y, double* stats, int k, int stride, int pad, int dil,
                        lhn_bnfin fin, const lhn_view* extra, const float* coef, const lhn_view* so, hipStream_t s) {
  if (!(stride == 1 && pad == dil * (k - 1) / 2 && x->C % 4 == 0 && y->W >= 8)) return 0;
  if (!lhn_no_pend(x) || !lhn_no_pend(extra)) return 0;
  DwExtra ex;
  ex.v = *extra;
  ex.coef[0] = coef[0];
  ex.coef[1] = coef[1];
  ex.n = 1;
  ex.sum_out = so ? so->data : nullptr;
  ex.so_cstride = so ? so->cstride : 0;
  ex.so_coff = so ? so->coff : 0;
  return lhn_dwk_fwd_lds(x, w, y, stats, k, dil, fin, s, &ex);
}

static int dw_bwd_addends(const lhn_view* x, const float* w, const lhn_view* y, const lhn_gradview* gy, float* dx, int dx_acc, float* dw,
                          int k, int dil, int nrep, int64_t rep_stride, const float* a0, const float* a1, hipStream_t s) {
  DwBnSum bs;
  bs.sums = nullptr;
  bs.save = nullptr;
  bs.C = bs.coff = 0;
  bs.add[0] = a0;
  bs.add[1] = a1;
  return lhn_dwk_bwd_lds(x, w, y, gy, dx, dx_acc, dw, k, dil, nrep, rep_stride, s, &bs);
}

static int dw_bwd_fin(const lhn_view* x, const float* w, const lhn_view* y, const lhn_gradview* gy, float* dx, int dx_acc, float* dw, int k,
                      int dil, int nrep, int64_t rep_stride, const lhn_bnsum* bns, const float* a0, const float* a1, const lhn_bnbwdsrc* fin,
                      hipStream_t s) {
  DwBnSum bs;
  bs.sums = bns ? bns->sums : nullptr;
  bs.save = bns ? bns->save : nullptr;
  bs.C = bns ? bns->C : 0;
  bs.coff = bns ? bns->coff : 0;
  bs.add[0] = a0;
  bs.add[1] = a1;
  return lhn_dwk_bwd_lds(x, w, y, gy, dx, dx_acc, dw, k, dil, nrep, rep_stride, s, &bs, fin);
}

static int dw_bwd_fused(const lhn_view* x, const float* w, const lhn_view* y, const lhn_gradview* gy, float* dx, float* dw, int k,
                        int dil, int nrep, int64_t rep_stride, double* bn_sums, const float* bn_save, int bn_C, int bn_coff, hipStream_t s) {
  DwBnSum bs;
  bs.sums = bn_sums;
  bs.save = bn_save;
  bs.C = bn_C;
  bs.coff = bn_coff;
  bs.add[0] = bs.add[1] = nullptr;
  return lhn_dwk_bwd_lds(x, w, y, gy, dx, 0, dw, k, dil, nrep, rep_stride, s, &bs);
}
```

### litehandnet_amd/csrc/k_conv_pw.hip

```cpp
#include <stdlib.h>
#include "lhn_common.h"

struct PwGeom {
  int wstride, kvalid, wrows, yacc, statC;
  int64_t nchw_bstride;
};

template <int CIN>
__device__ __forceinline__ void pw_stage_w(float* Ws, int LDA, const float* __restrict__ w, int rows_pad, const PwGeom& g) {
  constexpr int C4 = CIN / 4;
  const bool vec = (g.wstride % 4 == 0) && (g.kvalid % 4 == 0) && ((reinterpret_cast<uintptr_t>(w) & 15) == 0);
  for (int i = threadIdx.x; i < rows_pad * C4; i += 256) {
    const int co = i / C4, k4 = i % C4;
    f4 v = (f4){0.f, 0.f, 0.f, 0.f};
    if (co < g.wrows) {
      const float* r = w + (int64_t)co * g.wstride + k4 * 4;
      if (vec) {
        if (4 * k4 < g.kvalid) v = *reinterpret_cast<const f4*>(r);
      } else {
        if (4 * k4 + 0 < g.kvalid) v.x = r[0];
        if (4 * k4 + 1 < g.kvalid) v.y = r[1];
        if (4 * k4 + 2 < g.kvalid) v.z = r[2];
        if (4 * k4 + 3 < g.kvalid) v.w = r[3];
      }
// ... 757 lines not shown
      f16v accx[NDX];
#pragma unroll
      for (int t = 0; t < NDX; ++t)
#pragma unroll
        for (int r = 0; r < 16; ++r) accx[t][r] = 0.f;
      const float* arow = dYs + (mt * 32 + l31) * LDY + 4 * lh;
#pragma unroll 2
      for (int kc = 0; kc < COP / 8; ++kc) {
        const f4 a = *reinterpret_cast<const f4*>(arow + kc * 8);
        const float* wr = Ws + (kc * 8 + 4 * lh) * LDW + l31;
#pragma unroll
        for (int t = 0; t < NDX; ++t) {
          const int jt = (wave >> 1) + 2 * t;
          if (NTI % 2 == 0 || jt < NTI) {
            accx[t] = __builtin_amdgcn_mfma_f32_32x32x2f32(a.x, wr[0 * LDW + 32 * jt], accx[t], 0, 0, 0);
            accx[t] = __builtin_amdgcn_mfma_f32_32x32x2f32(a.y, wr[1 * LDW + 32 * jt], accx[t], 0, 0, 0);
            accx[t] = __builtin_amdgcn_mfma_f32_32x32x2f32(a.z, wr[2 * LDW + 32 * jt], accx[t], 0, 0, 0);
            accx[t] = __builtin_amdgcn_mfma_f32_32x32x2f32(a.w, wr[3 * LDW + 32 * jt], accx[t], 0, 0, 0);
          }
        }
      }
#pragma unroll
      for (int t = 0; t < NDX; ++t) {
        const int jt = (wave >> 1) + 2 * t;
        if (jt < NTI) {
#pragma unroll
          for (int r = 0; r < 16; ++r) {
            const int m = tile * 64 + mt * 32 + (r & 3) + 8 * (r >> 2) + 4 * lh;
            if (m < M && 32 * jt + l31 < x.C) {
              float* o = dx + in_pix(m) * x.cstride + x.coff + 32 * jt + l31;
              if (BNS) {
                const float raw = x.data[(int64_t)m * x.cstride + x.coff + 32 * jt + l31];
                const float du = accx[t][r] * (raw * b_sc[t] + b_sh[t] > 0.f ? 1.f : b_sl[t]);
                b_s[t] += du;
                b_q[t] += du * ((raw - b_mean[t]) * b_inv[t]);
              }
              *o = dx_acc ? *o + accx[t][r] : accx[t][r];
            }
          }
        }
      }
    }
    __syncthreads();
  }

  if (BNS) {
    float* bred = Xs;
#pragma unroll
    for (int t = 0; t < NB; ++t) {
      const int jt = (wave >> 1) + 2 * t;
      const float ss = b_s[t] + __shfl_xor(b_s[t], 32, 64), qq = b_q[t] + __shfl_xor(b_q[t], 32, 64);
      if (jt < NTI && lh == 0) {
        bred[((jt * 2 + (wave & 1)) * 2 + 0) * 32 + l31] = ss;
        bred[((jt * 2 + (wave & 1)) * 2 + 1) * 32 + l31] = qq;
      }
    }
    __syncthreads();
    if (tid < NTI * 32 && tid < x.C) {
      const int jt = tid >> 5, c = tid & 31;
      double* st = bs.sums + (size_t)(blockIdx.x % LHN_STAT_REPLICAS) * 2 * bs.C + bs.coff + tid;
      atomicAdd(st, (double)bred[((jt * 2 + 0) * 2 + 0) * 32 + c] + (double)bred[((jt * 2 + 1) * 2 + 0) * 32 + c]);
      atomicAdd(st + bs.C, (double)bred[((jt * 2 + 0) * 2 + 1) * 32 + c] + (double)bred[((jt * 2 + 1) * 2 + 1) * 32 + c]);
    }
    __syncthreads();
  }
  dw += (size_t)(blockIdx.x % nrep) * rep_stride;
#pragma unroll
  for (int t = 0; t < NDW; ++t) {
    const int dwave = DW_HI ? wave - 2 : wave;
    const int tl = dwave >= 0 ? (dwave + DWW * t) / KS : T;
    if (tl < T) {
      const int it = tl / NTI, jt = tl % NTI;
#pragma unroll
      for (int r = 0; r < 16; ++r) {
        const int co = 32 * it + (r & 3) + 8 * (r >> 2) + 4 * lh;
        if (co < geo.wrows && 32 * jt + l31 < geo.kvalid) atomicAdd(dw + (int64_t)co * geo.wstride + 32 * jt + l31, accw[t][r]);
      }
    }
  }
  if (dbias) {
    if (NCHW) {
    } else {
      f4* bred = reinterpret_cast<f4*>(dYs);
      bred[yr0 * YC4 + yc4] = ych_ok ? bsum : (f4){0.f, 0.f, 0.f, 0.f};
      __syncthreads();
      if (tid < YC4 && 4 * tid < cout) {
        f4 t = (f4){0.f, 0.f, 0.f, 0.f};
        for (int j = 0; j < YRP; ++j) t += bred[j * YC4 + tid];
        float* db = dbias + (size_t)(blockIdx.x % nrep) * rep_stride + 4 * tid;
        if (4 * tid + 0 < geo.wrows) atomicAdd(db + 0, t.x);
        if (4 * tid + 1 < geo.wrows) atomicAdd(db + 1, t.y);
        if (4 * tid + 2 < geo.wrows) atomicAdd(db + 2, t.z);
        if (4 * tid + 3 < geo.wrows) atomicAdd(db + 3, t.w);
      }
    }
  }
}

__global__ void __launch_bounds__(256) k_bias_grad_nchw(const float* __restrict__ dy, float* __restrict__ db, int N, int C,
                                                        int HW, int64_t bstride) {
  const int co = blockIdx.x;
  double s = 0;
  for (int n = blockIdx.y; n < N; n += gridDim.y) {
    const float* p = dy + (int64_t)n * bstride + (int64_t)co * HW;
    float a = 0.f;
    for (int i = threadIdx.x; i < HW; i += blockDim.x) a += p[i];
    s += a;
  }
  s = lhn_wave_sum_d(s);
  __shared__ double red[4];
  if ((threadIdx.x & 63) == 0) red[threadIdx.x >> 6] = s;
  __syncthreads();
  if (threadIdx.x == 0) atomicAdd(db + co, (float)(red[0] + red[1] + red[2] + red[3]));
}

template <int CIN, int NTO, bool NCHW, bool BNS = false>
static int launch_pw_bwd_t(const lhn_view* x, const float* w, const lhn_view* y, const lhn_gradview* gy, float* dx, int dx_acc,
                         float* dw, float* dbias, int stride, const float* dy_nchw, int cout, int nrep, int64_t rep_stride,
                         const PwGeom& geo, hipStream_t s, const lhn_bnsum& bs) {
  const int M = y->N * y->H * y->W;
  const int ntiles = (M + 63) / 64;
  constexpr int COP = 32 * NTO;
  const size_t lds = (size_t)(COP * (CIN + 4) + 64 * (COP + 4) + 64 * (CIN + 4)) * sizeof(float);
  static LhnKernelCfg cfg;
  int per_cu = 1;
  if (!lhn_kernel_cfg(cfg, &k_pw_bwd<CIN, NTO, NCHW, BNS>, lds, 4, &per_cu)) {
    lhn_set_error("lhn_conv_pw_bwd: cannot reserve %zu B of LDS", lds);
    return 2;
  }
  int grid = lhn_num_cus() * per_cu;
  if (grid > ntiles) grid = ntiles;
  lhn_gradview g = *gy;
  hipLaunchKernelGGL((k_pw_bwd<CIN, NTO, NCHW, BNS>), dim3(grid), dim3(256), lds, s, *x, w, *y, g, dx, dx_acc, dw, dbias, stride, dy_nchw,
                     cout, M, ntiles, nrep, rep_stride, geo, bs);
  if (dbias && dy_nchw)
    hipLaunchKernelGGL(k_bias_grad_nchw, dim3(geo.wrows, lhn_deterministic_mode() ? 1 : (y->N < 16 ? y->N : 16)), dim3(256), 0, s, dy_nchw, dbias, y->N, cout,
                       y->H * y->W, geo.nchw_bstride);
  return 0;
}

template <int CIN, int NTO>
static int launch_pw_bwd(const lhn_view* x, const float* w, const lhn_view* y, const lhn_gradview* gy, float* dx, int dx_acc,
                         float* dw, float* dbias, int stride, const float* dy_nchw, int cout, int nrep, int64_t rep_stride,
                         const PwGeom& geo, hipStream_t s, const lhn_bnsum& bs) {
  if (dy_nchw) return launch_pw_bwd_t<CIN, NTO, true>(x, w, y, gy, dx, dx_acc, dw, dbias, stride, dy_nchw, cout, nrep, rep_stride, geo, s, bs);
  if constexpr (CIN * NTO * 32 < 64 * 128) {
    if (bs.sums && dx && stride == 1)
      return launch_pw_bwd_t<CIN, NTO, false, true>(x, w, y, gy, dx, dx_acc, dw, dbias, stride, dy_nchw, cout, nrep, rep_stride, geo, s, bs);
  }
  if (bs.sums) return -1;
  return launch_pw_bwd_t<CIN, NTO, false>(x, w, y, gy, dx, dx_acc, dw, dbias, stride, dy_nchw, cout, nrep, rep_stride, geo, s, bs);
}

template <int CIN, int COUT, int PX, int PF, bool DYST, bool BNS, int OCC>
__global__ void __launch_bounds__(256, OCC) k_pw_bwd_wr(lhn_view x, const float* __restrict__ w, lhn_view y, lhn_gradview gy,
                                                        float* __restrict__ dx, int dx_acc, float* __restrict__ dw, float* __restrict__ dbias,
                                                        int M, int ntiles, int nrep, int64_t rep_stride, lhn_bnsum bs, lhn_bnbwdsrc fs) {
  constexpr int NTI = CIN / 32, NTO = COUT / 32, LDY = COUT + 4, LDX = CIN + 4;
  constexpr bool ONE = NTI == 1;
  constexpr int NDW = ONE ? 1 : NTO * NTI / 4;
  constexpr int KW = ONE ? 32 : PX;
  constexpr int NDX = (NTI == 4 && PX == 64) ? 2 : 1;
  constexpr int NWC = 4 / NTI;
  static_assert(ONE ? (NTO == 1 && PX == 128) : ((NTI == 2 || NTI == 4) && (NTO == 2 || NTO == 4) && (PX == 64 || (PX == 32 && NTI == 4))),
                "32 -> 32 at 128 pixels; 64 / 128 channels on either side at 64 (or 32) pixels");
  static_assert(!BNS || NDX == 1, "reader-side sums: one dX sub-tile per wave");
  extern __shared__ __attribute__((aligned(16))) float smem[];
  float* dYs = smem;
  float* Xs = dYs + PX * LDY;
  float* xt = Xs + PX * LDX;
  float* yt = xt + 3 * CIN;
  float* cf = yt + 3 * COUT;
  float* Xr = cf + 3 * COUT;
  const int tid = threadIdx.x, lane = tid & 63, wave = __builtin_amdgcn_readfirstlane(tid >> 6), l31 = lane & 31, lh = lane >> 5;
  const int HoWo = y.H * y.W;
  float* dzw = const_cast<float*>(gy.dz);

  constexpr int XC4 = CIN / 4, XRP = 256 / XC4, XPF = PX / XRP;
  constexpr int YC4 = COUT / 4, YRP = 256 / YC4, YPF = PX / YRP;
  constexpr int ZCH = YPF < 4 ? YPF : 4;
  const int xc4 = tid % XC4, xr0 = tid / XC4, xabs = x.coff + 4 * xc4;
  const int yc4 = tid % YC4, yr0 = tid / YC4, yabs = y.coff + 4 * yc4;

  f4 xraw[XPF], yraw[YPF], ydz[YPF];
  auto issue = [&](int tile) __attribute__((always_inline)) {
#pragma unroll
    for (int p = 0; p < XPF; ++p) {
      const int m = min(tile * PX + xr0 + p * XRP, M - 1);
      xraw[p] = *reinterpret_cast<const f4*>(x.data + (int64_t)m * x.cstride + xabs);
    }
#pragma unroll
    for (int p = 0; p < YPF; ++p) {
      const int m = min(tile * PX + yr0 + p * YRP, M - 1);
      if (PF >= 1) yraw[p] = *reinterpret_cast<const f4*>(y.data + (int64_t)m * y.cstride + yabs);
      if (PF >= 2) ydz[p] = *reinterpret_cast<const f4*>(gy.dz + (int64_t)m * y.cstride + yabs);
    }
  };
  f4 bsum = (f4){0.f, 0.f, 0.f, 0.f};
  auto commit = [&](int tile) __attribute__((always_inline)) {
    Xf4 xxf;
    xxf.sc = *reinterpret_cast<const f4*>(xt + 4 * xc4);
    xxf.sh = *reinterpret_cast<const f4*>(xt + CIN + 4 * xc4);
    xxf.sl = *reinterpret_cast<const f4*>(xt + 2 * CIN + 4 * xc4);
#pragma unroll
    for (int p = 0; p < XPF; ++p) {
      const int row = xr0 + p * XRP, m = tile * PX + row;
      f4 v = (f4){0.f, 0.f, 0.f, 0.f};
      if (m < M) {
        v = lhn_apply_xf(xraw[p], xxf);
        if (!BNS && x.gate) v *= *reinterpret_cast<const f4*>(x.gate + (int64_t)(m / HoWo) * x.cstride + xabs);
      }
      *reinterpret_cast<f4*>(Xs + row * LDX + 4 * xc4) = v;
      if (BNS) *reinterpret_cast<f4*>(Xr + row * CIN + 4 * xc4) = m < M ? xraw[p] : (f4){0.f, 0.f, 0.f, 0.f};
    }
    Xf4 yxf;
    Gr4 ygr;
    yxf.sc = *reinterpret_cast<const f4*>(yt + 4 * yc4);
    yxf.sh = *reinterpret_cast<const f4*>(yt + COUT + 4 * yc4);
    yxf.sl = *reinterpret_cast<const f4*>(yt + 2 * COUT + 4 * yc4);
    ygr.A = *reinterpret_cast<const f4*>(cf + 4 * yc4);
    ygr.B = *reinterpret_cast<const f4*>(cf + COUT + 4 * yc4);
    ygr.Cc = *reinterpret_cast<const f4*>(cf + 2 * COUT + 4 * yc4);
#pragma unroll
    for (int p = 0; p < YPF; ++p) {
      if (PF < 2 && p % ZCH == 0) {
#pragma unroll
        for (int q = p; q < p + ZCH; ++q) {
          const int mq = min(tile * PX + yr0 + q * YRP, M - 1);
          if (PF < 1) yraw[q] = *reinterpret_cast<const f4*>(y.data + (int64_t)mq * y.cstride + yabs);
          ydz[q] = *reinterpret_cast<const f4*>(gy.dz + (int64_t)mq * y.cstride + yabs);
        }
      }
      const int row = yr0 + p * YRP, m = tile * PX + row;
      f4 v = (f4){0.f, 0.f, 0.f, 0.f};
      if (m < M) {
        int n = 0, h = 0, ww = 0;
        if (y.gate || gy.dpool) {
          n = m / HoWo;
          const int r = m - n * HoWo;
          h = r / y.W;
          ww = r - h * y.W;
        }
        const f4 du = lhn_grad_du(y, gy, yxf, yraw[p], ydz[p], n, h, ww, yabs);
        v = ygr.A * du + ygr.B * yraw[p] + ygr.Cc;
        bsum += v;
        if (DYST) *reinterpret_cast<f4*>(dzw + (int64_t)m * y.cstride + yabs) = v;
      }
      *reinterpret_cast<f4*>(dYs + row * LDY + 4 * yc4) = v;
    }
  };

  int tile = blockIdx.x;
  if (tile < ntiles) issue(tile);
  static_assert(PX * LDY * sizeof(float) >= 2 * LHN_FIN_THREADS * sizeof(double), "dYs holds the replica fold's partials");
  LhnBwdPre fpre;
  if (fs.sums) {
    fpre = lhn_bn_bwd_pre(fs, 0, COUT);
    lhn_bn_bwd_fold_part_ct<COUT>(fs.sums, fs.stat_channels, reinterpret_cast<double*>(dYs));
  }
  for (int i = tid; i < CIN; i += 256) {
    xt[i] = x.table ? x.table[x.coff + i] : 1.f;
    xt[CIN + i] = x.table ? x.table[x.cstride + x.coff + i] : 0.f;
    xt[2 * CIN + i] = x.table ? x.table[2 * x.cstride + x.coff + i] : 1.f;
  }
  for (int i = tid; i < COUT; i += 256) {
    yt[i] = y.table ? y.table[y.coff + i] : 1.f;
    yt[COUT + i] = y.table ? y.table[y.cstride + y.coff + i] : 0.f;
    yt[2 * COUT + i] = y.table ? y.table[2 * y.cstride + y.coff + i] : 1.f;
    if (fs.sums) continue;
    cf[i] = gy.coef ? gy.coef[y.coff + i] : 1.f;
    cf[COUT + i] = gy.coef ? gy.coef[y.cstride + y.coff + i] : 0.f;
    cf[2 * COUT + i] = gy.coef ? gy.coef[2 * y.cstride + y.coff + i] : 0.f;
  }
  const int jt = NTI == 4 ? wave : NTI == 2 ? wave >> 1 : 0;
  const int mt0 = NTI == 4 ? 0 : NTI == 2 ? (wave & 1) : wave;
  float wreg[COUT / 2];
#pragma unroll
  for (int k = 0; k < COUT / 2; ++k) wreg[k] = dx ? w[(int64_t)((k >> 2) * 8 + 4 * lh + (k & 3)) * CIN + 32 * jt + l31] : 0.f;
  f16v accw[NDW];
#pragma unroll
  for (int t = 0; t < NDW; ++t)
#pragma unroll
    for (int r = 0; r < 16; ++r) accw[t][r] = 0.f;
  float b_sc = 1.f, b_sh = 0.f, b_sl = 1.f, b_mean = 0.f, b_inv = 0.f, b_s = 0.f, b_q = 0.f;
  if (BNS) {
    const int ci = 32 * jt + l31;
    if (x.table) {
      b_sc = x.table[x.coff + ci];
      b_sh = x.table[x.cstride + x.coff + ci];
      b_sl = x.table[2 * x.cstride + x.coff + ci];
    }
    b_mean = bs.save[bs.coff + ci];
    b_inv = bs.save[bs.C + bs.coff + ci];
  }
  double* const bst = BNS ? bs.sums + (size_t)(blockIdx.x % LHN_STAT_REPLICAS) * 2 * bs.C + bs.coff + (tid & (CIN - 1)) : nullptr;
  const int bsC = BNS ? bs.C : 0;
  if (fs.sums) {
    __syncthreads();
    if (tid < COUT)
      lhn_bn_bwd_coef_put(lhn_bn_bwd_coef(reinterpret_cast<const double*>(dYs), COUT, LHN_FIN_THREADS / COUT, tid, fpre.gamma, fpre.mean,
                                          fpre.inv, fs.count),
                          fs, const_cast<float*>(gy.coef), y.cstride, y.coff, tid, cf, COUT, tid, blockIdx.x == 0);
  }
  __syncthreads();

  for (; tile < ntiles; tile += gridDim.x) {
    commit(tile);
    __syncthreads();
    if (tile + (int)gridDim.x < ntiles) issue(tile + gridDim.x);
    {
      const float* ap = dYs + ((ONE ? 32 * wave : 0) + lh) * LDY + l31 + (ONE ? 0 : 32 * (wave / NTI));
      const float* bp = Xs + ((ONE ? 32 * wave : 0) + lh) * LDX + l31 + (ONE ? 0 : 32 * (wave % NTI));
#pragma unroll 4
      for (int ks = 0; ks < KW / 2; ++ks) {
        const float b = bp[(2 * ks) * LDX];
        float a[NDW];
#pragma unroll
        for (int t = 0; t < NDW; ++t) a[t] = ap[(2 * ks) * LDY + 32 * (4 / NTI) * t];
#pragma unroll
        for (int t = 0; t < NDW; ++t) accw[t] = __builtin_amdgcn_mfma_f32_32x32x2f32(a[t], b, accw[t], 0, 0, 0);
      }
    }
    if (dx) {
      f16v accx[NDX];
#pragma unroll
      for (int hh = 0; hh < NDX; ++hh)
#pragma unroll
        for (int r = 0; r < 16; ++r) accx[hh][r] = 0.f;
      const float* arow = dYs + (mt0 * 32 + l31) * LDY + 4 * lh;
#pragma unroll
      for (int kc = 0; kc < COUT / 8; ++kc) {
#pragma unroll
        for (int hh = 0; hh < NDX; ++hh) {
          const f4 a = *reinterpret_cast<const f4*>(arow + hh * 32 * LDY + kc * 8);
          accx[hh] = __builtin_amdgcn_mfma_f32_32x32x2f32(a.x, wreg[kc * 4 + 0], accx[hh], 0, 0, 0);
          accx[hh] = __builtin_amdgcn_mfma_f32_32x32x2f32(a.y, wreg[kc * 4 + 1], accx[hh], 0, 0, 0);
          accx[hh] = __builtin_amdgcn_mfma_f32_32x32x2f32(a.z, wreg[kc * 4 + 2], accx[hh], 0, 0, 0);
          accx[hh] = __builtin_amdgcn_mfma_f32_32x32x2f32(a.w, wreg[kc * 4 + 3], accx[hh], 0, 0, 0);
        }
      }
      const int cs = x.cstride;
#pragma unroll
      for (int hh = 0; hh < NDX; ++hh) {
        const int mbase = tile * PX + (mt0 + hh) * 32 + 4 * lh;
        float* o = dx + (int64_t)mbase * cs + x.coff + 32 * jt + l31;
        if (BNS) {
          const float* xr = Xr + ((mt0 + hh) * 32 + 4 * lh) * CIN + 32 * jt + l31;
#pragma unroll
          for (int r = 0; r < 16; ++r) {
            const float raw = xr[((r & 3) + 8 * (r >> 2)) * CIN];
            const float du = accx[hh][r] * (raw * b_sc + b_sh > 0.f ? 1.f : b_sl);
            b_s += du;
            b_q += du * ((raw - b_mean) * b_inv);
          }
        }
        if (tile * PX + PX <= M) {
          if (dx_acc) {
#pragma unroll
            for (int r = 0; r < 16; ++r) o[((r & 3) + 8 * (r >> 2)) * cs] += accx[hh][r];
          } else {
#pragma unroll
            for (int r = 0; r < 16; ++r) o[((r & 3) + 8 * (r >> 2)) * cs] = accx[hh][r];
          }
        } else if constexpr (BNS) {
          float* ot = dx + (int64_t)(tile * PX + (mt0 + hh) * 32) * cs + x.coff + 32 * jt + l31;
#pragma unroll
          for (int r = 0; r < 16; ++r) {
            const int ro = (r & 3) + 8 * (r >> 2) + 4 * lh;
            if (tile * PX + (mt0 + hh) * 32 + ro < M) ot[(int64_t)ro * cs] = dx_acc ? ot[(int64_t)ro * cs] + accx[hh][r] : accx[hh][r];
          }
        } else {
#pragma unroll
          for (int r = 0; r < 16; ++r) {
            const int ro = (r & 3) + 8 * (r >> 2);
            if (mbase + ro < M) o[ro * cs] = dx_acc ? o[ro * cs] + accx[hh][r] : accx[hh][r];
          }
        }
      }
    }
    __syncthreads();
  }

  if (BNS) {
    float* bred = Xs;
    const float ss = b_s + __shfl_xor(b_s, 32, 64), qq = b_q + __shfl_xor(b_q, 32, 64);
    if (lh == 0) {
      bred[((jt * NWC + mt0) * 2 + 0) * 32 + l31] = ss;
      bred[((jt * NWC + mt0) * 2 + 1) * 32 + l31] = qq;
    }
    __syncthreads();
    if (tid < CIN) {
      const int jc = tid >> 5, c = tid & 31;
      double ds = 0.0, dq = 0.0;
#pragma unroll
      for (int v = 0; v < NWC; ++v) {
        ds += (double)bred[((jc * NWC + v) * 2 + 0) * 32 + c];
        dq += (double)bred[((jc * NWC + v) * 2 + 1) * 32 + c];
      }
      atomicAdd(bst, ds);
      atomicAdd(bst + bsC, dq);
    }
  }
  dw += (size_t)(blockIdx.x % nrep) * rep_stride;
  if constexpr (ONE) {
    float* wred = dYs;
#pragma unroll
    for (int r = 0; r < 16; ++r) wred[(wave * 16 + r) * 64 + lane] = accw[0][r];
    __syncthreads();
#pragma unroll
    for (int q = 0; q < 4; ++q) {
      const int r = 4 * q + wave, co = (r & 3) + 8 * (r >> 2) + 4 * lh;
      const float v = ((wred[r * 64 + lane] + wred[(16 + r) * 64 + lane]) + wred[(32 + r) * 64 + lane]) + wred[(48 + r) * 64 + lane];
      atomicAdd(dw + (int64_t)co * CIN + l31, v);
    }
    if (dbias) __syncthreads();
  } else {
#pragma unroll
    for (int t = 0; t < NDW; ++t) {
      const int it = wave / NTI + (4 / NTI) * t, jw = wave % NTI;
#pragma unroll
      for (int r = 0; r < 16; ++r) {
        const int co = 32 * it + (r & 3) + 8 * (r >> 2) + 4 * lh;
        atomicAdd(dw + (int64_t)co * CIN + 32 * jw + l31, accw[t][r]);
      }
    }
  }
  if (dbias) {
    f4* bred = reinterpret_cast<f4*>(dYs);
    bred[yr0 * YC4 + yc4] = bsum;
    __syncthreads();
    if (tid < YC4) {
      f4 t = (f4){0.f, 0.f, 0.f, 0.f};
      for (int j = 0; j < YRP; ++j) t += bred[j * YC4 + tid];
      float* db = dbias + (size_t)(blockIdx.x % nrep) * rep_stride + 4 * tid;
      atomicAdd(db + 0, t.x);
      atomicAdd(db + 1, t.y);
      atomicAdd(db + 2, t.z);
      atomicAdd(db + 3, t.w);
    }
  }
}

template <int CIN, int COUT, int PX, int PF, bool DYST = true, bool BNS = false, int OCC = 2>
static int launch_pw_bwd_wr(const lhn_view* x, const float* w, const lhn_view* y, const lhn_gradview* gy, float* dx, int dx_acc, float* dw,
                            float* dbias, int nrep, int64_t rep_stride, hipStream_t s, const lhn_bnsum& bs, const lhn_bnbwdsrc* fsp = nullptr) {
  const int M = y->N * y->H * y->W, ntiles = (M + PX - 1) / PX;
  lhn_bnbwdsrc fs;
  if (fsp) fs = *fsp; else memset(&fs, 0, sizeof(fs));
  const size_t lds = (size_t)(PX * (COUT + 4) + PX * (CIN + 4) + 3 * CIN + 6 * COUT + (BNS ? PX * CIN : 0)) * sizeof(float);
  static LhnKernelCfg cfg;
  int per_cu = 1;
  if (!lhn_kernel_cfg(cfg, &k_pw_bwd_wr<CIN, COUT, PX, PF, DYST, BNS, OCC>, lds, OCC, &per_cu)) {
    lhn_set_error("lhn_conv_pw_bwd: cannot reserve %zu B of LDS", lds);
    return 2;
  }
  int grid = lhn_num_cus() * per_cu;
  if (grid > ntiles) grid = ntiles;
  hipLaunchKernelGGL((k_pw_bwd_wr<CIN, COUT, PX, PF, DYST, BNS, OCC>), dim3(grid), dim3(256), lds, s, *x, w, *y, *gy, dx, dx_acc, dw, dbias,
                     M, ntiles, nrep, rep_stride, bs, fs);
  return 0;
}

static bool pw_bwd_narrow_off() {
  static int off = -1;
  if (off < 0) {
    const char* e = getenv("LHN_PW_BWD_NARROW");
    off = (e && e[0] == '0') ? 1 : 0;
  }
  return off == 1;
}

static bool pw_bwd_split_forced() {
  static int on = -1;
  if (on < 0) {
    const char* e = getenv("LHN_PW_BWD_SPLIT");
    on = (e && e[0] == '1') ? 1 : 0;
  }
  return on == 1;
}

int lhn_pw_bwd_split(const lhn_view* x, const float* w, const lhn_view* y, const lhn_gradview* gy, float* dx, int dx_accumulate,
                     float* dw, float* dbias, int nrep, int64_t rep_stride, hipStream_t s);

extern "C" int lhn_conv_pw_bwd2(const lhn_view* x, const float* w, const lhn_view* y, const lhn_gradview* gy, float* dx,
                                int dx_accumulate, float* dw, float* dbias, int stride, const float* dy_nchw, int nrep,
                                int64_t rep_stride, const lhn_pw_opts* opts, void* stream) {
  return lhn_conv_pw_bwd3(x, w, y, gy, dx, dx_accumulate, dw, dbias, stride, dy_nchw, nrep, rep_stride, opts, nullptr, stream);
}
extern "C" int lhn_conv_pw_bwd3(const lhn_view* x, const float* w, const lhn_view* y, const lhn_gradview* gy, float* dx,
                                int dx_accumulate, float* dw, float* dbias, int stride, const float* dy_nchw, int nrep,
                                int64_t rep_stride, const lhn_pw_opts* opts, const lhn_bnsum* bns, void* stream) {
  return lhn_conv_pw_bwd4(x, w, y, gy, dx, dx_accumulate, dw, dbias, stride, dy_nchw, nrep, rep_stride, opts, bns, nullptr, stream);
}
extern "C" int lhn_conv_pw_bwd4(const lhn_view* x, const float* w, const lhn_view* y, const lhn_gradview* gy, float* dx,
                                int dx_accumulate, float* dw, float* dbias, int stride, const float* dy_nchw, int nrep,
                                int64_t rep_stride, const lhn_pw_opts* opts, const lhn_bnsum* bns, const lhn_bnbwdsrc* fin, void* stream) {
  return lhn_conv_pw_bwd5(x, w, y, gy, dx, dx_accumulate, dw, dbias, stride, dy_nchw, nrep, rep_stride, opts, bns, fin, nullptr, stream);
}
static int pw_bwd_run(const lhn_view* x, const float* w, const lhn_view* y, const lhn_gradview* gy, float* dx, int dx_accumulate, float* dw,
                      float* dbias, int stride, const float* dy_nchw, int nrep, int64_t rep_stride, const lhn_pw_opts* opts,
                      const lhn_bnsum* bns, const lhn_bnbwdsrc* fin, const lhn_gatesum* gs, bool* gs_done, int flags, void* stream);
extern "C" int lhn_conv_pw_bwd5(const lhn_view* x, const float* w, const lhn_view* y, const lhn_gradview* gy, float* dx,
                                int dx_accumulate, float* dw, float* dbias, int stride, const float* dy_nchw, int nrep,
                                int64_t rep_stride, const lhn_pw_opts* opts, const lhn_bnsum* bns, const lhn_bnbwdsrc* fin,
                                const lhn_gatesum* gs, void* stream) {
  return lhn_conv_pw_bwd6(x, w, y, gy, dx, dx_accumulate, dw, dbias, stride, dy_nchw, nrep, rep_stride, opts, bns, fin, gs, 0, stream);
}
extern "C" int lhn_conv_pw_bwd6(const lhn_view* x, const float* w, const lhn_view* y, const lhn_gradview* gy, float* dx,
                                int dx_accumulate, float* dw, float* dbias, int stride, const float* dy_nchw, int nrep,
                                int64_t rep_stride, const lhn_pw_opts* opts, const lhn_bnsum* bns, const lhn_bnbwdsrc* fin,
                                const lhn_gatesum* gs, int flags, void* stream) {
  if (gs && !gs->dgate) gs = nullptr;
  if (gs) LHN_CHECK_ARG(lhn_view_ok(x) && dx && !dx_accumulate && stride == 1 && (!gs->slices || (gs->slices->n >= 0 && gs->slices->n <= 2)),
                        "lhn_conv_pw_bwd5: gate sums need a stored dx (no accumulate), stride 1 and 0..2 BatchNorm slices");
  bool gs_done = false;
  const int rc = pw_bwd_run(x, w, y, gy, dx, dx_accumulate, dw, dbias, stride, dy_nchw, nrep, rep_stride, opts, bns, fin, gs, &gs_done, flags, stream);
  if (rc || !gs || gs_done) return rc;
  lhn_view xv = *x;
  xv.gate = nullptr;
  return lhn_gate_bwd_reduce3(&xv, dx, gs->dgate, gs->dgate + (size_t)x->N * x->cstride, gs->slices, 1, stream);
}
static int pw_bwd_run(const lhn_view* x, const float* w, const lhn_view* y, const lhn_gradview* gy, float* dx, int dx_accumulate, float* dw,
                      float* dbias, int stride, const float* dy_nchw, int nrep, int64_t rep_stride, const lhn_pw_opts* opts,
                      const lhn_bnsum* bns, const lhn_bnbwdsrc* fin, const lhn_gatesum* gs, bool* gs_done, int flags, void* stream) {
  if (nrep < 1) nrep = 1;
  if (fin && !fin->sums) fin = nullptr;
  lhn_bnsum bs;
  memset(&bs, 0, sizeof(bs));
  if (bns && bns->sums) {
    LHN_CHECK_ARG(x && y && bns->save && dx && stride == 1 && x->C <= 128 && y->C <= 128 && x->C * y->C < 64 * 128 && !x->gate && x->table &&
                      bns->coff >= 0 && bns->coff + x->C <= bns->C,
                  "lhn_conv_pw_bwd3: BatchNorm sums ride in the fused kernel only (stride 1, Cin * Cout < 8192, ungated input inside the producer's channels)");
    bs = *bns;
  }
  LHN_CHECK_ARG(lhn_view_ok(x) && w && y && gy && dw && lhn_no_pend(x) && lhn_no_pend(y), "lhn_conv_pw_bwd: bad view / null pointer");
  LHN_CHECK_ARG(stride == 1 || stride == 2, "lhn_conv_pw_bwd: stride %d", stride);
  LHN_CHECK_ARG(stride == 1 || !dx || dx_accumulate, "lhn_conv_pw_bwd: stride-2 dgrad only accumulates into a zeroed gradient");
  if (!dy_nchw) LHN_CHECK_ARG(lhn_view_ok(y) && gy->dz, "lhn_conv_pw_bwd: bad output view / missing dz");
  const int Cout = y->C, Cin = x->C, HoWo = y->H * y->W;
  const int wcols = (opts && opts->w_cols > 0) ? opts->w_cols : Cin, wrows = (opts && opts->w_rows > 0) ? opts->w_rows : Cout;
  LHN_CHECK_ARG(wcols <= Cin && wcols > Cin - 4 && wrows <= Cout, "lhn_conv_pw_bwd: weight [%d][%d] does not fit views %d -> %d",
                wrows, wcols, Cin, Cout);
  const int64_t bstride = (opts && opts->nchw_batch_stride > 0) ? opts->nchw_batch_stride : (int64_t)Cout * HoWo;
  hipStream_t s = (hipStream_t)stream;
  const bool wr_wide = !bs.sums && stride == 1 && !dy_nchw && wcols == Cin && wrows == Cout && !pw_bwd_split_forced() && !pw_wr_off() &&
                       ((Cin == 128 && Cout == 128) || (Cin == 64 && Cout == 128) || (Cin == 128 && Cout == 64));
  const bool wr_narrow = stride == 1 && !dy_nchw && wcols == Cin && wrows == Cout && Cin == Cout && (Cin == 64 || Cin == 32) &&
                         !pw_bwd_narrow_off() && !pw_wr_off();
  if (dy_nchw && lhn_head_stream_on() && !pw_wr_off() && stride == 1 && !bs.sums && !fin && Cin == HEAD_CIN && wcols == Cin && Cout <= 32 && wrows == Cout &&
      HoWo % 4 == 0 && bstride % 4 == 0 && (!gs || (HoWo % 64 == 0 && !lhn_deterministic_mode())) &&
      ((reinterpret_cast<uintptr_t>(dy_nchw) | reinterpret_cast<uintptr_t>(x->data)) & 15) == 0) {
    const int rc = lhn_head_bwd(x, w, dy_nchw, dx, dx_accumulate, dw, dbias, Cout, HoWo, bstride, nrep, rep_stride, gs, s);
    if (rc) return rc;
    LHN_CHECK_LAUNCH("lhn_conv_pw_bwd");
    *gs_done = gs != nullptr;
    return 0;
  }
  if (fin) {
    LHN_CHECK_ARG(!dy_nchw && gy->coef && fin->save_mean_invstd && fin->count > 0 && fin->stat_channels >= Cout,
                  "lhn_conv_pw_bwd4: finalize source needs gy->coef, saved statistics and stat_channels >= Cout");
    if (!wr_wide && !wr_narrow) {
      const int rc = lhn_bn_bwd_finalize2(fin->sums, fin->gamma, fin->save_mean_invstd, const_cast<float*>(gy->coef), y->cstride, y->coff,
                                          Cout, fin->stat_channels, fin->count, fin->dgamma, fin->dbeta, fin->pgrad_scale, stream);
      if (rc) return rc;
      fin = nullptr;
    }
  }
  if (wr_wide) {
    int rc = -1;
#define PWB_WIDE(CI, CO, PXV, PFV) \
  if (Cin == CI && Cout == CO)     \
    rc = dz_dead ? launch_pw_bwd_wr<CI, CO, PXV, PFV, false>(x, w, y, gy, dx, dx_accumulate, dw, dbias, nrep, rep_stride, s, bs, fin) \
                 : launch_pw_bwd_wr<CI, CO, PXV, PFV, true>(x, w, y, gy, dx, dx_accumulate, dw, dbias, nrep, rep_stride, s, bs, fin);
    const bool dz_dead = (flags & LHN_PW_BWD_DZ_DEAD) != 0;
    PWB_WIDE(128, 128, 32, 1) PWB_WIDE(64, 128, 64, 1) PWB_WIDE(128, 64, 64, 2)
#undef PWB_WIDE
    if (rc == 0) {
      LHN_CHECK_LAUNCH("lhn_conv_pw_bwd");
      return 0;
    }
    if (rc > 0) return rc;
  }
  if (wr_narrow) {
    int rc;
    if (Cin == 64) rc = bs.sums ? launch_pw_bwd_wr<64, 64, 64, 2, false, true>(x, w, y, gy, dx, dx_accumulate, dw, dbias, nrep, rep_stride, s, bs, fin)
                                : launch_pw_bwd_wr<64, 64, 64, 2, false, false>(x, w, y, gy, dx, dx_accumulate, dw, dbias, nrep, rep_stride, s, bs, fin);
    else rc = bs.sums ? launch_pw_bwd_wr<32, 32, 128, 2, false, true>(x, w, y, gy, dx, dx_accumulate, dw, dbias, nrep, rep_stride, s, bs, fin)
                      : launch_pw_bwd_wr<32, 32, 128, 2, false, false, 3>(x, w, y, gy, dx, dx_accumulate, dw, dbias, nrep, rep_stride, s, bs, fin);
    if (rc) return rc;
    LHN_CHECK_LAUNCH("lhn_conv_pw_bwd");
    return 0;
  }
  if (!bs.sums && stride == 1 && !dy_nchw && Cin * Cout >= 64 * 128 && Cout % 32 == 0 && Cin % 32 == 0 && Cout <= 256 && wcols == Cin && wrows == Cout) {
    const int rc = lhn_pw_bwd_split(x, w, y, gy, dx, dx_accumulate, dw, dbias, nrep, rep_stride, s);
    if (rc == 0) {
      LHN_CHECK_LAUNCH("lhn_conv_pw_bwd");
      return 0;
    }
    if (rc > 0) return rc;
  }
  for (int co0 = 0; co0 < Cout; co0 += 128) {
    const int cc = Cout - co0 < 128 ? Cout - co0 : 128, nto = (cc + 31) / 32 == 3 ? 4 : (cc + 31) / 32;
    for (int k0 = 0; k0 < Cin; k0 += 128) {
      const int kc = Cin - k0 < 128 ? Cin - k0 : 128, ci = kc <= 32 ? 32 : pw_cin_tile(kc);
      lhn_view xv = *x, yv = *y;
      xv.coff += k0;
      xv.C = kc;
      if (!dy_nchw) {
        yv.coff += co0;
        yv.C = cc;
      }
      PwGeom g;
      g.wstride = wcols;
      g.kvalid = wcols - k0 < kc ? wcols - k0 : kc;
      g.wrows = wrows - co0 < cc ? (wrows - co0 < 0 ? 0 : wrows - co0) : cc;
      g.yacc = 0;
      g.statC = Cout;
      g.nchw_bstride = bstride;
      const float* wv = w + (int64_t)co0 * wcols + k0;
      float* dwv = dw + (int64_t)co0 * wcols + k0;
      float* dbv = (dbias && k0 == 0) ? dbias + co0 : nullptr;
      const float* dyv = dy_nchw ? dy_nchw + (int64_t)co0 * HoWo : nullptr;
      const int acc = dx_accumulate || co0 > 0;
      int rc = -1;
#define PWB_CASE(CI, NTV) \
  if (ci == CI && nto == NTV) rc = launch_pw_bwd<CI, NTV>(&xv, wv, &yv, gy, dx, acc, dwv, dbv, stride, dyv, cc, nrep, rep_stride, g, s, bs);
      PWB_CASE(32, 1) PWB_CASE(32, 2) PWB_CASE(32, 4) PWB_CASE(64, 1) PWB_CASE(64, 2) PWB_CASE(64, 4) PWB_CASE(128, 1)
      PWB_CASE(128, 2) PWB_CASE(128, 4)
#undef PWB_CASE
      LHN_CHECK_ARG(rc != -1, "lhn_conv_pw_bwd: unsupported channels Cin=%d Cout=%d", Cin, Cout);
      if (rc) return rc;
    }
  }
  LHN_CHECK_LAUNCH("lhn_conv_pw_bwd");
  return 0;
}

extern "C" int lhn_conv_pw_bwd(const lhn_view* x, const float* w, const lhn_view* y, const lhn_gradview* gy, float* dx,
                               int dx_accumulate, float* dw, float* dbias, int stride, const float* dy_nchw, int nrep,
                               int64_t rep_stride, void* stream) {
  return lhn_conv_pw_bwd2(x, w, y, gy, dx, dx_accumulate, dw, dbias, stride, dy_nchw, nrep, rep_stride, nullptr, stream);
}
```

### litehandnet_amd/csrc/lhn_plan.cpp

```cpp
#include <stdint.h>
#include <stdlib.h>
#include <string.h>
#include <vector>
#include "lhn_common.h"

static lhn_bnsum mkbns(void* ws, int64_t sums_off, int64_t save_off, int C, int coff) {
  lhn_bnsum b;
  memset(&b, 0, sizeof(b));
  if (sums_off >= 0 && save_off >= 0 && C > 0) {
    b.sums = reinterpret_cast<double*>(static_cast<char*>(ws) + sums_off);
    b.save = reinterpret_cast<const float*>(static_cast<char*>(ws) + save_off);
    b.C = C;
    b.coff = coff;
  }
  return b;
}

enum {
  OP_STEM = 1, OP_PW = 2, OP_DW = 3, OP_KXK = 4, OP_FINALIZE = 5, OP_EW = 6, OP_MAXPOOL = 7, OP_AVGPOOL = 8,
  OP_CA_MLP = 9, OP_TABLE_FILL = 10, OP_MEMSET = 11, OP_ATT_MLP = 12, OP_SE_MLP = 13, OP_SHUFFLE = 14,
  OP_PWDW = 15, OP_DWPW = 16, OP_MSRB = 17, OP_CBAM = 18, OP_BNECK = 19, OP_STEMTAIL = 20,
  OP_STEM_BWD = 101, OP_PW_BWD = 102, OP_DW_BWD = 103, OP_KXK_BWD = 104, OP_BN_BWD = 105, OP_EW_BWD = 106,
  OP_MAXPOOL_BWD = 107, OP_AVGPOOL_BWD = 108, OP_GATE_REDUCE = 109, OP_CA_MLP_BWD = 110, OP_ATT_MLP_BWD = 111, OP_SE_MLP_BWD = 112,
  OP_SHUFFLE_BWD = 113, OP_CBAM_BWD = 114,
};

struct GraphEntry {
  int phase, training, nrep, seen;
  int64_t rstr;
  void *ws, *io0, *io1;
  uint64_t phash, ghash;
  hipGraphExec_t exec;
  uint64_t last_use;
};

struct Plan {
  std::vector<lhn_buf> bufs;
  std::vector<lhn_op> fwd, bwd;
  std::vector<uint8_t> pw_dz_dead;
  std::vector<GraphEntry> graphs;
  uint64_t tick = 0;
  int graph_misses = 0;
};

static inline char* at(void* ws, int64_t off) { return off < 0 ? nullptr : static_cast<char*>(ws) + off; }

static lhn_view mkview(const Plan* P, void* ws, int buf, int coff, int C, bool with_gate = true) {
  const lhn_buf& b = P->bufs[buf];
  lhn_view v;
  v.pend = nullptr;
  v.data = reinterpret_cast<float*>(at(ws, b.data_off));
  v.table = reinterpret_cast<const float*>(at(ws, b.table_off));
  v.gate = with_gate ? reinterpret_cast<const float*>(at(ws, b.gate_off)) : nullptr;
  v.N = b.N; v.H = b.H; v.W = b.W;
  v.cstride = b.C; v.coff = coff; v.C = C;
  return v;
}
static lhn_gradview mkgrad(const Plan* P, void* ws, int buf, bool use_coef) {
  const lhn_buf& b = P->bufs[buf];
  lhn_gradview g;
  g.dz = reinterpret_cast<const float*>(at(ws, b.grad_off));
  g.dpool = reinterpret_cast<const float*>(at(ws, b.dpool_off));
  g.coef = use_coef ? reinterpret_cast<const float*>(at(ws, b.coef_off)) : nullptr;
  return g;
}
template <typename T>
static inline T* prm(void* const* arr, int idx) { return idx < 0 ? nullptr : static_cast<T*>(arr[idx]); }
static lhn_bn_slices mkslices(void* ws, const int32_t* pk, const int64_t* sv, const int64_t* sm) {
  lhn_bn_slices s;
  memset(&s, 0, sizeof(s));
  for (int k = 0; k < 2; ++k)
    if (pk[k] > 0 && sv[k] >= 0) {
      const int j = s.n++;
      s.lo[j] = pk[k] >> 16;
      s.C[j] = pk[k] & 0xffff;
      s.save[j] = reinterpret_cast<const float*>(at(ws, sv[k]));
      s.sums[j] = (sm && sm[k] >= 0) ? reinterpret_cast<double*>(at(ws, sm[k])) : nullptr;
    }
  return s;
}

static bool conv_has_bn(const lhn_op& o) { return o.p[2] >= 0 || o.p[3] >= 0 || o.ws[1] >= 0; }
static lhn_bnfin mkfin(const Plan* P, void* ws, const lhn_op& o, void* const* params) {
  const lhn_buf& b = P->bufs[o.out_buf];
  lhn_bnfin f;
  f.counter = reinterpret_cast<uint32_t*>(at(ws, o.ws[2]));
  f.gamma = prm<const float>(params, o.p[2]);
  f.beta = prm<const float>(params, o.p[3]);
  f.running_mean = prm<float>(params, o.p[4]);
  f.running_var = prm<float>(params, o.p[5]);
  f.num_batches_tracked = prm<int64_t>(params, o.p[6]);
  f.table = reinterpret_cast<float*>(at(ws, b.table_off));
  f.save_mean_invstd = reinterpret_cast<float*>(at(ws, o.ws[1]));
  f.count = (double)b.N * b.H * b.W;
  f.cstride = b.C; f.coff = o.out_coff; f.C = o.out_C;
  f.eps = o.f[0]; f.momentum = o.f[1]; f.slope = o.f[2];
  f.conv_bias = prm<const float>(params, o.p[1]);
  return f;
}
static bool fuse_finalize() {
  static int v = -1;
  if (v < 0) {
    const char* e = getenv("LHN_FUSE_FINALIZE");
    v = (e && e[0] == '1') ? 1 : 0;
  }
  return v == 1;
}
static bool bwd_fin_consumer() {
  static int v = -1;
  if (v < 0) {
    const char* e = getenv("LHN_BWD_FIN_CONSUMER");
    v = (e && e[0] == '0') ? 0 : 1;
  }
  return v == 1;
}
bool lhn_head_stream_on();
static bool head_gate_fold_at(const Plan* P, const std::vector<lhn_op>& ops, size_t oi) {
  if (!lhn_head_stream_on() || lhn_deterministic_mode() || oi + 1 >= ops.size()) return false;
  const lhn_op &o = ops[oi], &nx = ops[oi + 1];
  if (o.kind != OP_PW_BWD || !o.i[1] || o.i[0] != 1 || o.i[2] != 1 || o.in_buf[0] < 0) return false;
  if (o.in_C[0] != 128 || o.out_C > 32 || o.i[3] || o.i[4]) return false;
  const lhn_buf& b = P->bufs[o.in_buf[0]];
  return o.in_coff[0] == 0 && o.in_C[0] == b.C && b.gate_off >= 0 && nx.kind == OP_GATE_REDUCE && nx.out_buf == o.in_buf[0] &&
         nx.out_coff == 0 && nx.out_C == b.C && nx.ws[3] >= 0 && nx.ws[4] >= 0;
}
static bool pw_bwd_dy_store() {
  static int v = -1;
  if (v < 0) {
    const char* e = getenv("LHN_PW_BWD_DY_STORE");
    v = (e && e[0] == '1') ? 1 : 0;
  }
  return v == 1;
}
static bool pw_dz_dead_at(const Plan* P, const std::vector<lhn_op>& ops, size_t oi) {
  const lhn_op& o = ops[oi];
  if (o.kind != OP_PW_BWD || o.i[1] || o.out_buf < 0 || P->bufs[o.out_buf].grad_off < 0) return false;
  auto grad_bytes = [&](int buf, int64_t* lo, int64_t* hi) {
    const lhn_buf& b = P->bufs[buf];
    *lo = b.grad_off;
    *hi = b.grad_off + (int64_t)sizeof(float) * b.N * b.H * b.W * b.C;
    return b.grad_off >= 0;
  };
  int64_t lo, hi;
  grad_bytes(o.out_buf, &lo, &hi);
  const int oC = P->bufs[o.out_buf].C;
  auto touches = [&](int buf, int coff, int C) {
    int64_t a, b;
    if (buf < 0 || !grad_bytes(buf, &a, &b) || a >= hi || lo >= b) return false;
    return a != lo || P->bufs[buf].C != oC || (coff < o.out_coff + o.out_C && o.out_coff < coff + C);
  };
  for (size_t k = oi + 1; k < ops.size(); ++k) {
    const lhn_op& q = ops[k];
    if (q.kind == OP_MEMSET) {
      if (q.ws[0] < hi && lo < q.ws[0] + q.ws[1]) return false;
      continue;
    }
    if (touches(q.out_buf, q.out_coff, q.out_C)) return false;
    for (int s = 0; s < 3; ++s)
      if (touches(q.in_buf[s], q.in_coff[s], q.in_C[s])) return false;
    for (int s = 0; s < 12; ++s)
      if (q.ws[s] >= lo && q.ws[s] < hi) return false;
  }
  return true;
}

static int sep_finalize(const lhn_bnfin& f, const double* stats, int training, void* stream, int creal = 0, int repeat = 1) {
  int rc = 0;
  for (int r = 0; r < (training ? (repeat < 1 ? 1 : repeat) : 1) && !rc; ++r)
    rc = lhn_bn_finalize2(training ? stats : nullptr, f.gamma, f.beta, f.running_mean, f.running_var,
                          training ? f.num_batches_tracked : nullptr, f.table, f.cstride, f.coff, creal > 0 ? creal : f.C, f.C,
                          training ? f.save_mean_invstd : nullptr, f.count, f.eps, f.momentum, f.slope, training, f.conv_bias, stream);
  return rc;
}

extern "C" {

void* lhn_plan_create(const lhn_buf* bufs, int nbufs, const lhn_op* fwd, int nfwd, const lhn_op* bwd, int nbwd) {
  if (!bufs || nbufs <= 0 || !fwd || nfwd <= 0) {
    lhn_set_error("lhn_plan_create: empty plan");
    return nullptr;
  }
  Plan* p = new Plan();
  p->bufs.assign(bufs, bufs + nbufs);
  p->fwd.assign(fwd, fwd + nfwd);
  if (bwd && nbwd > 0) p->bwd.assign(bwd, bwd + nbwd);
  for (const auto* lst : {&p->fwd, &p->bwd})
    for (const lhn_op& o : *lst) {
      bool ok = o.out_buf < nbufs;
      for (int k = 0; k < 3; ++k) ok = ok && o.in_buf[k] < nbufs;
      if (!ok) {
        lhn_set_error("lhn_plan_create: op kind %d references buffer out of range", o.kind);
        delete p;
        return nullptr;
      }
    }
  p->pw_dz_dead.resize(p->bwd.size());
  for (size_t oi = 0; oi < p->bwd.size(); ++oi) p->pw_dz_dead[oi] = pw_dz_dead_at(p, p->bwd, oi) ? 1 : 0;
  return p;
}

int lhn_plan_head_gate_fold(void* plan) {
  const Plan* p = static_cast<const Plan*>(plan);
  if (!p) return -1;
  for (size_t oi = 0; oi + 1 < p->bwd.size(); ++oi)
    if (head_gate_fold_at(p, p->bwd, oi)) return (int)oi + 1;
  return -1;
}

int lhn_plan_pw_dz_dead(void* plan, int bwd_index) {
  const Plan* p = static_cast<const Plan*>(plan);
  if (!p || bwd_index < 0 || (size_t)bwd_index >= p->pw_dz_dead.size()) return -1;
  return p->pw_dz_dead[bwd_index];
}

void lhn_plan_destroy(void* plan) {
  Plan* p = static_cast<Plan*>(plan);
  if (!p) return;
  for (GraphEntry& g : p->graphs)
    if (g.exec) (void)hipGraphExecDestroy(g.exec);
  delete p;
}

static int run_ops(const Plan* P, int phase, void* ws, void* const* params, void* const* grads, void* const* io, int mode,
                   int nrep, int64_t rstr, void* stream, size_t sb = 0, size_t se = (size_t)-1, double cscale = 1.0,
                   float pscale = 1.f) {
  const int training = mode & 1;
  const bool skip_tables = (mode & 2) != 0 && !training;
  const std::vector<lhn_op>& ops = phase == 0 ? P->fwd : P->bwd;
  hipStream_t s = static_cast<hipStream_t>(stream);
  int rc = 0;
  const bool whole = (sb == 0 && se >= 2 * ops.size());
  lhn_bnbwdsrc cfin;
  size_t cfin_for = (size_t)-1;
  size_t gfold_at = (size_t)-1;
  for (size_t oi = 0; oi < ops.size() && rc == 0; ++oi) {
    const lhn_op& o = ops[oi];
    const bool deferred = false;
    const bool is_conv = o.kind == OP_STEM || o.kind == OP_PW || o.kind == OP_DW || o.kind == OP_KXK;
    const bool fz = is_conv && training && fuse_finalize() && whole && !(o.kind == OP_PW && o.i[2] > 0) &&
                    !((o.kind == OP_PW || o.kind == OP_DW) && (int)o.f[3] > 1);
    const bool h0 = 2 * oi >= sb && 2 * oi < se, h1 = 2 * oi + 1 >= sb && 2 * oi + 1 < se;
    if (!h0 && !h1) continue;
    const bool two_half = o.kind == OP_STEM || o.kind == OP_PW || o.kind == OP_DW || o.kind == OP_KXK || o.kind == OP_CA_MLP ||
                          o.kind == OP_ATT_MLP || o.kind == OP_BN_BWD || o.kind == OP_CA_MLP_BWD || o.kind == OP_ATT_MLP_BWD;
    if (!two_half && !h0) continue;
    const int stage = (h0 && h1) ? 0 : (h0 ? 1 : 2);
    switch (o.kind) {
      case OP_MEMSET: {
        if (hipMemsetAsync(at(ws, o.ws[0]), 0, (size_t)o.ws[1], s) != hipSuccess) {
          lhn_set_error("lhn_plan_run: memset failed");
          rc = 2;
        }
        break;
      }
      case OP_TABLE_FILL: {
        if (skip_tables) break;
        const lhn_buf& b = P->bufs[o.out_buf];
        if (o.i[0])
          rc = lhn_table_bias(reinterpret_cast<float*>(at(ws, b.table_off)), b.C, o.out_coff, o.out_C, prm<const float>(params, o.p[0]), o.f[2], stream);
        else
          rc = lhn_table_fill(reinterpret_cast<float*>(at(ws, b.table_off)), b.C, o.out_coff, o.out_C, o.f[0], o.f[1], o.f[2], stream);
        break;
      }
      case OP_STEM: {
        lhn_view y = mkview(P, ws, o.out_buf, o.out_coff, o.out_C);
        const bool bn = conv_has_bn(o);
        lhn_bnfin fin;
        if (bn) {
          fin = mkfin(P, ws, o, params);
          fin.count *= cscale;
        }
        if (h0) rc = lhn_conv_stem_fwd(static_cast<const float*>(io[0]), prm<const float>(params, o.p[0]), &y,
                               (training && o.ws[0] >= 0) ? reinterpret_cast<double*>(at(ws, o.ws[0])) : nullptr, o.i[3], o.i[4], o.i[0], o.i[1],
                               o.i[2], (bn && fz) ? &fin : nullptr, stream);
        if (!rc && bn && h1 && !skip_tables && !deferred && !fz) rc = sep_finalize(fin, reinterpret_cast<const double*>(at(ws, o.ws[0])), training, stream);
        break;
      }
      case OP_PW: {
        lhn_view x = mkview(P, ws, o.in_buf[0], o.in_coff[0], o.in_C[0]);
        lhn_view y;
        float* nchw = nullptr;
        if (o.i[1]) {
          y = x;
          y.data = nullptr; y.table = nullptr; y.gate = nullptr; y.pend = nullptr;
          y.cstride = o.out_C; y.coff = 0; y.C = o.out_C;
          nchw = static_cast<float*>(io[1]);
        } else {
          y = mkview(P, ws, o.out_buf, o.out_coff, o.out_C);
        }
        const bool bn = !o.i[1] && conv_has_bn(o);
        lhn_bnfin fin;
        if (bn) {
          fin = mkfin(P, ws, o, params);
          fin.count *= cscale;
        }
        lhn_pw_opts po;
        memset(&po, 0, sizeof(po));
        po.w_rows = o.i[2]; po.w_cols = o.i[3];
        lhn_view extra[2];
        if (o.i[6] > 1) {
          po.n_extra = o.i[6] - 1;
          for (int e = 0; e < po.n_extra; ++e) {
            extra[e] = mkview(P, ws, o.in_buf[e + 1], o.in_coff[e + 1], o.in_C[e + 1]);
          }
          po.extra = extra;
          for (int e = 0; e < 3; ++e) po.coef[e] = o.f[4 + e];
        }
        lhn_view sumv;
        if (o.i[6] > 1 && o.ws[4] >= 0) {
          sumv = x;
          sumv.data = reinterpret_cast<float*>(at(ws, o.ws[4]));
          sumv.table = nullptr; sumv.gate = nullptr; sumv.pend = nullptr;
          sumv.cstride = (int)(o.ws[5] >> 16); sumv.coff = (int)(o.ws[5] & 0xffff);
          po.sum_out = &sumv;
        }
        if (nchw && o.i[5] > 1) {
          const int64_t khw = (int64_t)o.out_C * y.H * y.W;
          nchw += (int64_t)o.i[4] * khw;
          po.nchw_batch_stride = (int64_t)o.i[5] * khw;
        }
        if (h0) rc = lhn_conv_pw_fwd2(&x, prm<const float>(params, o.p[0]), bn ? nullptr : prm<const float>(params, o.p[1]), &y,
                              (training && o.ws[0] >= 0) ? reinterpret_cast<double*>(at(ws, o.ws[0])) : nullptr, o.i[0], nchw,
                              (bn && fz) ? &fin : nullptr, &po, stream);
        if (!rc && bn && h1 && !skip_tables && !deferred && !fz)
          rc = sep_finalize(fin, reinterpret_cast<const double*>(at(ws, o.ws[0])), training, stream, o.i[2], (int)o.f[3]);
        break;
      }
      case OP_DW: {
        lhn_view x = mkview(P, ws, o.in_buf[0], o.in_coff[0], o.in_C[0]);
        lhn_view y = mkview(P, ws, o.out_buf, o.out_coff, o.out_C);
        const bool bn = conv_has_bn(o);
        lhn_bnfin fin;
        if (bn) {
          fin = mkfin(P, ws, o, params);
          fin.count *= cscale;
        }
        lhn_view extra;
        const float coef2[2] = {o.f[4], o.f[5]};
        if (o.i[6] > 1) {
          extra = mkview(P, ws, o.in_buf[1], o.in_coff[1], o.in_C[1]);
        }
        lhn_view sumv;
        const bool so = o.i[6] > 1 && o.ws[4] >= 0;
        if (so) {
          sumv = x;
          sumv.data = reinterpret_cast<float*>(at(ws, o.ws[4]));
          sumv.table = nullptr; sumv.gate = nullptr; sumv.pend = nullptr;
          sumv.cstride = (int)(o.ws[5] >> 16); sumv.coff = (int)(o.ws[5] & 0xffff);
        }
        if (h0) rc = lhn_conv_dw_fwd3(&x, prm<const float>(params, o.p[0]), &y,
                              (training && o.ws[0] >= 0) ? reinterpret_cast<double*>(at(ws, o.ws[0])) : nullptr, o.i[0], o.i[1], o.i[2], o.i[3],
                              (bn && fz) ? &fin : nullptr, o.i[6] > 1 ? &extra : nullptr, coef2,
                              so ? &sumv : nullptr, stream);
        if (!rc && bn && h1 && !skip_tables && !deferred && !fz)
          rc = sep_finalize(fin, reinterpret_cast<const double*>(at(ws, o.ws[0])), training, stream, 0, (int)o.f[3]);
        break;
      }
      case OP_KXK: {
        lhn_view x = mkview(P, ws, o.in_buf[0], o.in_coff[0], o.in_C[0]);
        lhn_view y = mkview(P, ws, o.out_buf, o.out_coff, o.out_C);
        const bool bn = conv_has_bn(o);
        lhn_bnfin fin;
        if (bn) {
          fin = mkfin(P, ws, o, params);
          fin.count *= cscale;
// ... 83 lines not shown
        const bool two = o.i[6] > 1;
        if (two) {
          if (o.in_buf[2] < 0 || o.i[1] < 0 || o.i[1] >= (int)P->bufs.size()) {
            lhn_set_error("lhn_plan_run: fused MSRB round: extra source out of range");
            rc = 1;
            break;
          }
          extra[0] = mkview(P, ws, o.in_buf[2], o.in_coff[2], o.in_C[2]);
          extra[1] = mkview(P, ws, o.i[1], o.i[2], o.i[3]);
        }
        const float coef2[2] = {o.f[4], o.f[5]};
        lhn_view y = mkview(P, ws, o.out_buf, o.out_coff, o.out_C, false);
        rc = lhn_msrb_round_fwd(x, two ? extra : nullptr, two ? coef2 : nullptr, prm<const float>(params, o.p[0]), prm<const float>(params, o.p[1]),
                                &y, reinterpret_cast<float*>(at(ws, o.ws[0])), o.i[0], o.i[0], at(ws, o.ws[1]), stream);
        break;
      }
      case OP_FINALIZE: {
        if (skip_tables) break;
        const lhn_buf& b = P->bufs[o.out_buf];
        const int src = o.in_buf[0] >= 0 ? o.in_buf[0] : o.out_buf;
        const lhn_buf& sb = P->bufs[src];
        rc = lhn_bn_finalize(reinterpret_cast<const double*>(at(ws, o.ws[0])), prm<const float>(params, o.p[0]),
                             prm<const float>(params, o.p[1]), prm<float>(params, o.p[2]), prm<float>(params, o.p[3]),
                             prm<int64_t>(params, o.p[4]), reinterpret_cast<float*>(at(ws, b.table_off)), b.C, o.out_coff,
                             o.out_C, reinterpret_cast<float*>(at(ws, o.ws[1])), (double)sb.N * sb.H * sb.W, o.f[0], o.f[1],
                             o.f[2], training, nullptr, stream);
        break;
      }
      case OP_EW: {
        lhn_view srcs[3];
        for (int k = 0; k < o.i[0]; ++k) {
          srcs[k] = mkview(P, ws, o.in_buf[k], o.in_coff[k], o.in_C[k]);
        }
        lhn_view d = mkview(P, ws, o.out_buf, o.out_coff, o.out_C);
        const float coef[3] = {o.f[4], o.f[5], o.f[6]};
        rc = lhn_ew_fwd3(srcs, o.i[0], o.i[1] ? coef : nullptr, &d, o.f[0], o.i[2], stream);
        break;
      }
      case OP_MAXPOOL: {
        lhn_view x = mkview(P, ws, o.in_buf[0], o.in_coff[0], o.in_C[0]);
        lhn_view y = mkview(P, ws, o.out_buf, o.out_coff, o.out_C);
        rc = lhn_maxpool2_fwd(&x, &y, stream);
        break;
      }
      case OP_SHUFFLE: {
        lhn_view a = mkview(P, ws, o.in_buf[0], o.in_coff[0], o.in_C[0]);
        lhn_view b = mkview(P, ws, o.in_buf[1], o.in_coff[1], o.in_C[1]);
        lhn_view d = mkview(P, ws, o.out_buf, o.out_coff, o.out_C);
        rc = lhn_shuffle2_fwd(&a, &b, &d, stream);
        break;
      }
      case OP_AVGPOOL: {
        lhn_view x = mkview(P, ws, o.in_buf[0], o.in_coff[0], o.in_C[0], o.i[2] == 0);
        if (o.ws[1] >= 0 || o.in_buf[1] >= 0) {
          const lhn_bn_slices sl = mkslices(ws, &o.i[5], &o.ws[2], nullptr);
          lhn_view src;
          if (o.in_buf[1] >= 0) src = mkview(P, ws, o.in_buf[1], o.in_coff[1], o.in_C[1]);
          rc = lhn_avgpool_fwd4(&x, reinterpret_cast<float*>(at(ws, o.ws[0])), o.i[0], o.i[1],
                                o.ws[1] >= 0 ? reinterpret_cast<float*>(at(ws, o.ws[1])) : nullptr, &sl, o.in_buf[1] >= 0 ? &src : nullptr, stream);
          break;
        }
        rc = lhn_avgpool_fwd2(&x, reinterpret_cast<float*>(at(ws, o.ws[0])), o.i[0], o.i[1], o.i[3] > 0 ? o.i[3] : x.C, o.i[4], stream);
        break;
      }
      case OP_CA_MLP: {
        const lhn_buf& b = P->bufs[o.out_buf];
        if ((!training || o.ws[3] < 0) && !h0) break;
        rc = lhn_ca_mlp_fwd(reinterpret_cast<const float*>(at(ws, o.ws[0])), prm<const float>(params, o.p[0]),
                            prm<const float>(params, o.p[1]), prm<const float>(params, o.p[2]), prm<float>(params, o.p[3]),
                            prm<float>(params, o.p[4]), prm<int64_t>(params, o.p[5]), prm<const float>(params, o.p[6]),
                            prm<const float>(params, o.p[7]), prm<const float>(params, o.p[8]), prm<const float>(params, o.p[9]),
                            (training && o.ws[2] >= 0) ? reinterpret_cast<const float*>(at(ws, o.ws[2])) : nullptr,
                            reinterpret_cast<float*>(at(ws, b.gate_off)), b.C, o.out_coff,
                            reinterpret_cast<float*>(at(ws, o.ws[1])), b.N, o.out_C, o.f[0], o.f[1], training,
                            (training && o.ws[3] >= 0) ? stage : 0, o.ws[3] >= 0 ? reinterpret_cast<double*>(at(ws, o.ws[3])) : nullptr,
                            cscale, stream);
        break;
      }
      case OP_ATT_MLP: {
        const lhn_buf& b = P->bufs[o.out_buf];
        if ((!training || o.ws[3] < 0) && !h0) break;
        rc = lhn_att_mlp_fwd(reinterpret_cast<const float*>(at(ws, o.ws[0])), prm<const float>(params, o.p[0]),
                             prm<const float>(params, o.p[1]), prm<float>(params, o.p[2]), prm<float>(params, o.p[3]),
                             prm<int64_t>(params, o.p[4]), prm<const float>(params, o.p[5]), prm<const float>(params, o.p[6]),
                             prm<const float>(params, o.p[7]), prm<const float>(params, o.p[8]),
                             (training && o.ws[2] >= 0) ? reinterpret_cast<const float*>(at(ws, o.ws[2])) : nullptr,
                             reinterpret_cast<float*>(at(ws, b.gate_off)), b.C, o.out_coff,
                             reinterpret_cast<float*>(at(ws, o.ws[1])), b.N, o.out_C, o.f[0], o.f[1], training,
                             (training && o.ws[3] >= 0) ? stage : 0, o.ws[3] >= 0 ? reinterpret_cast<double*>(at(ws, o.ws[3])) : nullptr,
                             cscale, stream);
        break;
      }
      case OP_SE_MLP: {
        const lhn_buf& b = P->bufs[o.out_buf];
        rc = lhn_se_mlp_fwd2(reinterpret_cast<const float*>(at(ws, o.ws[0])), prm<const float>(params, o.p[0]),
                             prm<const float>(params, o.p[1]), prm<const float>(params, o.p[2]), prm<const float>(params, o.p[3]),
                             reinterpret_cast<float*>(at(ws, b.gate_off)), b.C, o.out_coff, reinterpret_cast<float*>(at(ws, o.ws[1])),
                             b.N, o.out_C, o.i[0], o.i[1], stream);
        break;
      }
      case OP_STEM_BWD: {
        lhn_view y = mkview(P, ws, o.out_buf, o.out_coff, o.out_C);
        lhn_gradview g = mkgrad(P, ws, o.out_buf, o.i[5] != 0);
        rc = lhn_conv_stem_bwd(static_cast<const float*>(io[0]), &y, &g, prm<float>(grads, o.p[1]), o.i[3], o.i[4], o.i[0],
                               o.i[1], o.i[2], nrep, rstr, stream);
        break;
      }
      case OP_PW_BWD: {
        lhn_view x = mkview(P, ws, o.in_buf[0], o.in_coff[0], o.in_C[0]);
        lhn_view y;
        lhn_gradview g;
        const float* nchw = nullptr;
        if (o.i[1]) {
          y = x;
          y.data = nullptr; y.table = nullptr; y.gate = nullptr;
          y.cstride = o.out_C; y.coff = 0; y.C = o.out_C;
          g.dz = nullptr; g.dpool = nullptr; g.coef = nullptr;
          nchw = static_cast<const float*>(io[1]);
        } else {
          y = mkview(P, ws, o.out_buf, o.out_coff, o.out_C);
          g = mkgrad(P, ws, o.out_buf, o.i[5] != 0);
        }
        float* dx = o.i[2] ? reinterpret_cast<float*>(at(ws, P->bufs[o.in_buf[0]].grad_off)) : nullptr;
        lhn_pw_opts po;
        memset(&po, 0, sizeof(po));
        po.w_rows = o.i[3]; po.w_cols = o.i[4];
        if (nchw && o.i[7] > 1) {
          const int64_t khw = (int64_t)o.out_C * y.H * y.W;
          nchw += (int64_t)o.i[6] * khw;
          po.nchw_batch_stride = (int64_t)o.i[7] * khw;
        }
        const lhn_bnsum bs = mkbns(ws, o.ws[0], o.ws[1], (int)o.f[6], (int)o.f[7]);
        lhn_gatesum gsum;
        lhn_bn_slices gsl;
        memset(&gsum, 0, sizeof(gsum));
        if (phase == 1 && whole && head_gate_fold_at(P, ops, oi)) {
          const lhn_op& nx = ops[oi + 1];
          gsl = mkslices(ws, &nx.i[0], &nx.ws[5], nullptr);
          gsum.dgate = reinterpret_cast<float*>(at(ws, nx.ws[3]));
          gsum.slices = &gsl;
          gfold_at = oi + 1;
        }
        const int flags = (phase == 1 && whole && P->pw_dz_dead[oi] && !pw_bwd_dy_store()) ? LHN_PW_BWD_DZ_DEAD : 0;
        rc = lhn_conv_pw_bwd6(&x, prm<const float>(params, o.p[0]), &y, &g, dx, o.i[2] == 2, prm<float>(grads, o.p[1]),
                              prm<float>(grads, o.p[2]), o.i[0], nchw, nrep, rstr, &po, bs.sums ? &bs : nullptr,
                              cfin_for == oi ? &cfin : nullptr, gsum.dgate ? &gsum : nullptr, flags, stream);
        break;
      }
      case OP_DW_BWD: {
        lhn_view x = mkview(P, ws, o.in_buf[0], o.in_coff[0], o.in_C[0]);
        lhn_view y = mkview(P, ws, o.out_buf, o.out_coff, o.out_C);
        lhn_gradview g = mkgrad(P, ws, o.out_buf, o.i[5] != 0);
        float* dx = o.i[4] ? reinterpret_cast<float*>(at(ws, P->bufs[o.in_buf[0]].grad_off)) : nullptr;
        if (cfin_for == oi) {
          const bool adds = o.ws[2] >= 0 || o.ws[3] >= 0;
          const lhn_bnsum bs = mkbns(ws, adds ? -1 : o.ws[4], adds ? -1 : o.ws[5], o.i[6], o.i[7]);
          rc = lhn_conv_dw_bwd4(&x, prm<const float>(params, o.p[0]), &y, &g, dx, o.i[4] == 2, prm<float>(grads, o.p[1]), o.i[0], o.i[1],
                                o.i[2], o.i[3], nrep, rstr, bs.sums ? &bs : nullptr,
                                o.ws[2] >= 0 ? reinterpret_cast<const float*>(at(ws, o.ws[2])) : nullptr,
                                o.ws[3] >= 0 ? reinterpret_cast<const float*>(at(ws, o.ws[3])) : nullptr, &cfin, stream);
          break;
        }
        if (o.ws[2] >= 0 || o.ws[3] >= 0) {
          rc = lhn_conv_dw_bwd3(&x, prm<const float>(params, o.p[0]), &y, &g, dx, o.i[4] == 2, prm<float>(grads, o.p[1]), o.i[0], o.i[1],
                                o.i[2], o.i[3], nrep, rstr, o.ws[2] >= 0 ? reinterpret_cast<const float*>(at(ws, o.ws[2])) : nullptr,
                                o.ws[3] >= 0 ? reinterpret_cast<const float*>(at(ws, o.ws[3])) : nullptr, stream);
          break;
        }
        rc = lhn_conv_dw_bwd2(&x, prm<const float>(params, o.p[0]), &y, &g, dx, o.i[4] == 2, prm<float>(grads, o.p[1]), o.i[0],
                              o.i[1], o.i[2], o.i[3], nrep, rstr, o.ws[4] >= 0 ? reinterpret_cast<double*>(at(ws, o.ws[4])) : nullptr,
                              o.ws[5] >= 0 ? reinterpret_cast<const float*>(at(ws, o.ws[5])) : nullptr, o.i[6], o.i[7], stream);
        break;
      }
      case OP_KXK_BWD: {
        lhn_view x = mkview(P, ws, o.in_buf[0], o.in_coff[0], o.in_C[0]);
        lhn_view y = mkview(P, ws, o.out_buf, o.out_coff, o.out_C);
        lhn_gradview g = mkgrad(P, ws, o.out_buf, o.i[5] != 0);
        float* dx = o.i[2] ? reinterpret_cast<float*>(at(ws, P->bufs[o.in_buf[0]].grad_off)) : nullptr;
        rc = lhn_conv_kxk_bwd(&x, prm<const float>(params, o.p[0]), &y, &g, dx, o.i[2] == 2, prm<float>(grads, o.p[1]), o.i[0],
                              nrep, rstr, o.ws[3] >= 0 ? reinterpret_cast<float*>(at(ws, o.ws[3])) : nullptr, stream);
        break;
      }
      case OP_BN_BWD: {
        const lhn_buf& b = P->bufs[o.out_buf];
        lhn_view y = mkview(P, ws, o.out_buf, o.out_coff, o.out_C);
        lhn_gradview g = mkgrad(P, ws, o.out_buf, false);
        double* sums = reinterpret_cast<double*>(at(ws, o.ws[0]));
        const float* save = reinterpret_cast<const float*>(at(ws, o.ws[1]));
        lhn_bnbwdfin fin;
        fin.counter = reinterpret_cast<uint32_t*>(at(ws, o.ws[2]));
        fin.gamma = prm<const float>(params, o.p[0]);
        fin.coef = reinterpret_cast<float*>(at(ws, b.coef_off));
        fin.dgamma = prm<float>(grads, o.p[1]);
        fin.dbeta = prm<float>(grads, o.p[2]);
        fin.count = (double)b.N * b.H * b.W * cscale;
        fin.cstride = b.C; fin.coff = o.out_coff; fin.C = o.out_C;
        if (fin.counter && fuse_finalize() && whole && !o.i[1]) {
          rc = lhn_bn_bwd_reduce(&y, &g, save, sums, &fin, stream);
        } else {
          if (h0 && !o.i[1]) rc = lhn_bn_bwd_reduce(&y, &g, save, sums, nullptr, stream);
          const lhn_op* nx = oi + 1 < ops.size() ? &ops[oi + 1] : nullptr;
          if (!rc && h1 && whole && bwd_fin_consumer() && !fuse_finalize() && o.i[0] == 0 && nx &&
              (nx->kind == OP_DW_BWD || (nx->kind == OP_PW_BWD && !nx->i[1])) && nx->out_buf == o.out_buf && nx->out_coff == o.out_coff &&
              nx->out_C == o.out_C && nx->i[5] != 0) {
            cfin.sums = sums;
            cfin.save_mean_invstd = save;
            cfin.gamma = fin.gamma;
            cfin.dgamma = fin.dgamma;
            cfin.dbeta = fin.dbeta;
            cfin.count = fin.count;
            cfin.pgrad_scale = pscale;
            cfin.stat_channels = o.out_C;
            cfin_for = oi + 1;
          } else if (!rc && h1)
            rc = lhn_bn_bwd_finalize2(sums, fin.gamma, save, fin.coef, b.C, o.out_coff, o.i[0] > 0 ? o.i[0] : o.out_C, o.out_C, fin.count,
                                      fin.dgamma, fin.dbeta, pscale, stream);
        }
        break;
      }
      case OP_EW_BWD: {
        lhn_view src = mkview(P, ws, o.in_buf[0], o.in_coff[0], o.in_C[0]);
        lhn_view d = mkview(P, ws, o.out_buf, o.out_coff, o.out_C);
        const lhn_buf& db = P->bufs[o.out_buf];
        if (o.i[1] == 1) {
          lhn_view other = mkview(P, ws, o.in_buf[1], o.in_coff[1], o.in_C[1]);
          rc = lhn_ew_mul_bwd(&src, &other, &d, reinterpret_cast<const float*>(at(ws, db.grad_off)),
                              reinterpret_cast<float*>(at(ws, P->bufs[o.in_buf[0]].grad_off)), o.i[0], stream);
        } else if (o.i[1] == 2) {
          rc = lhn_bilinear_bwd(&src, &d, reinterpret_cast<const float*>(at(ws, db.grad_off)),
                                reinterpret_cast<float*>(at(ws, P->bufs[o.in_buf[0]].grad_off)), o.i[0], o.f[0], stream);
        } else if (o.i[1] == 3) {
          lhn_view srcs[3];
          float* dsrcs[3];
          int acc[3] = {o.i[0], o.i[2], o.i[3]};
          lhn_bnsum bsv[3] = {mkbns(ws, o.ws[0], o.ws[1], o.i[4], o.i[5]), mkbns(ws, o.ws[2], o.ws[3], o.i[6], o.i[7]),
                              mkbns(ws, o.ws[4], o.ws[5], (int)o.f[4], (int)o.f[5])};
          const lhn_bnsum* bsp[3];
          int ns = 0;
          for (; ns < 3 && o.in_buf[ns] >= 0; ++ns) {
            srcs[ns] = mkview(P, ws, o.in_buf[ns], o.in_coff[ns], o.in_C[ns]);
            dsrcs[ns] = reinterpret_cast<float*>(at(ws, P->bufs[o.in_buf[ns]].grad_off));
            bsp[ns] = bsv[ns].sums ? &bsv[ns] : nullptr;
          }
          rc = lhn_ew_bwd_multi(srcs, ns, &d, reinterpret_cast<const float*>(at(ws, db.grad_off)),
                                reinterpret_cast<const float*>(at(ws, db.dpool_off)), o.f[0], dsrcs, acc, bsp, stream);
        } else {
          const lhn_bnsum bs = mkbns(ws, o.ws[0], o.ws[1], o.i[4], o.i[5]);
          rc = lhn_ew_bwd3(&src, &d, reinterpret_cast<const float*>(at(ws, db.grad_off)),
                           reinterpret_cast<const float*>(at(ws, db.dpool_off)), o.f[0],
                           reinterpret_cast<float*>(at(ws, P->bufs[o.in_buf[0]].grad_off)), o.i[0], bs.sums ? &bs : nullptr, stream);
        }
        break;
      }
      case OP_MAXPOOL_BWD: {
        lhn_view x = mkview(P, ws, o.in_buf[0], o.in_coff[0], o.in_C[0]);
        lhn_view y = mkview(P, ws, o.out_buf, o.out_coff, o.out_C);
        const lhn_bnsum bs = mkbns(ws, o.ws[0], o.ws[1], o.i[4], o.i[5]);
        lhn_grad_adds ad;
        memset(&ad, 0, sizeof(ad));
        if (o.ws[2] >= 0) {
          ad.same = reinterpret_cast<const float*>(at(ws, o.ws[2]));
          ad.same_cstride = o.i[1]; ad.same_coff = o.i[2];
        }
        if (o.ws[3] >= 0) {
          ad.pooled = reinterpret_cast<const float*>(at(ws, o.ws[3]));
          ad.pooled_cstride = o.i[3]; ad.pooled_coff = o.i[6];
          ad.OH = o.i[7] >> 16; ad.OW = o.i[7] & 0xffff;
        }
        rc = lhn_maxpool2_bwd3(&x, &y, reinterpret_cast<const float*>(at(ws, P->bufs[o.out_buf].grad_off)),
                               reinterpret_cast<float*>(at(ws, P->bufs[o.in_buf[0]].grad_off)), o.i[0], bs.sums ? &bs : nullptr,
                               (ad.same || ad.pooled) ? &ad : nullptr, stream);
        break;
      }
      case OP_AVGPOOL_BWD: {
        lhn_view x = mkview(P, ws, o.in_buf[0], o.in_coff[0], o.in_C[0]);
        const lhn_bnsum bs = mkbns(ws, o.ws[1], o.ws[2], o.i[5], o.i[6]);
        rc = lhn_avgpool_bwd3(&x, reinterpret_cast<const float*>(at(ws, o.ws[0])), o.i[0], o.i[1], o.i[3] > 0 ? o.i[3] : x.C, o.i[4],
                              reinterpret_cast<float*>(at(ws, P->bufs[o.in_buf[0]].grad_off)), o.i[2], bs.sums ? &bs : nullptr, stream);
        break;
      }
      case OP_SHUFFLE_BWD: {
        lhn_view a = mkview(P, ws, o.in_buf[0], o.in_coff[0], o.in_C[0]);
        lhn_view b = mkview(P, ws, o.in_buf[1], o.in_coff[1], o.in_C[1]);
        lhn_view d = mkview(P, ws, o.out_buf, o.out_coff, o.out_C);
        rc = lhn_shuffle2_bwd(&a, &b, &d, reinterpret_cast<const float*>(at(ws, P->bufs[o.out_buf].grad_off)),
                              o.i[0] ? reinterpret_cast<float*>(at(ws, P->bufs[o.in_buf[0]].grad_off)) : nullptr, o.i[0] == 2,
                              o.i[1] ? reinterpret_cast<float*>(at(ws, P->bufs[o.in_buf[1]].grad_off)) : nullptr, o.i[1] == 2, stream);
        break;
      }
      case OP_GATE_REDUCE: {
        if (gfold_at == oi) break;
        lhn_view y = mkview(P, ws, o.out_buf, o.out_coff, o.out_C, false);
        float* dg = reinterpret_cast<float*>(at(ws, o.ws[3]));
        const lhn_bn_slices sl = mkslices(ws, &o.i[0], &o.ws[5], nullptr);
        rc = lhn_gate_bwd_reduce3(&y, reinterpret_cast<const float*>(at(ws, P->bufs[o.out_buf].grad_off)), dg,
                                  o.ws[4] >= 0 ? dg + (size_t)y.N * y.C : nullptr, &sl, 1, stream);
        break;
      }
      case OP_CA_MLP_BWD: {
        const lhn_buf& b = P->bufs[o.out_buf];
        if (o.ws[4] < 0 && !h0) break;
        const lhn_bn_slices sl = mkslices(ws, &o.i[0], &o.ws[6], &o.ws[8]);
        const float* dgp = reinterpret_cast<const float*>(at(ws, o.ws[3]));
        rc = lhn_ca_mlp_bwd2(reinterpret_cast<const float*>(at(ws, o.ws[0])), prm<const float>(params, o.p[0]),
                            prm<const float>(params, o.p[1]), prm<const float>(params, o.p[2]), prm<const float>(params, o.p[3]),
                            o.ws[2] >= 0 ? reinterpret_cast<const float*>(at(ws, o.ws[2])) : nullptr,
                            reinterpret_cast<const float*>(at(ws, o.ws[1])), reinterpret_cast<const float*>(at(ws, o.ws[3])),
                            reinterpret_cast<float*>(at(ws, b.dpool_off)), b.C, o.out_coff, b.H, b.W, prm<float>(grads, o.p[4]),
                            prm<float>(grads, o.p[5]), prm<float>(grads, o.p[6]), prm<float>(grads, o.p[7]),
                            prm<float>(grads, o.p[8]), prm<float>(grads, o.p[9]), prm<float>(grads, o.p[10]), b.N, o.out_C,
                            o.ws[4] >= 0 ? stage : 0, o.ws[4] >= 0 ? reinterpret_cast<double*>(at(ws, o.ws[4])) : nullptr, cscale, pscale,
                            o.ws[5] >= 0 ? dgp + (size_t)b.N * b.C : nullptr, o.ws[5] >= 0 ? reinterpret_cast<const float*>(at(ws, o.ws[5])) : nullptr,
                            &sl, stream);
        break;
      }
      case OP_ATT_MLP_BWD: {
        const lhn_buf& b = P->bufs[o.out_buf];
        if (o.ws[4] < 0 && !h0) break;
        rc = lhn_att_mlp_bwd(reinterpret_cast<const float*>(at(ws, o.ws[0])), prm<const float>(params, o.p[0]),
                             prm<const float>(params, o.p[1]), prm<const float>(params, o.p[2]), prm<const float>(params, o.p[3]),
                             o.ws[2] >= 0 ? reinterpret_cast<const float*>(at(ws, o.ws[2])) : nullptr,
                             reinterpret_cast<float*>(at(ws, o.ws[1])), reinterpret_cast<const float*>(at(ws, o.ws[3])),
                             reinterpret_cast<float*>(at(ws, b.dpool_off)), b.C, o.out_coff, b.H, b.W, prm<float>(grads, o.p[4]),
                             prm<float>(grads, o.p[5]), prm<float>(grads, o.p[6]), prm<float>(grads, o.p[7]),
                             prm<float>(grads, o.p[8]), prm<float>(grads, o.p[9]), b.N, o.out_C,
                             o.ws[4] >= 0 ? stage : 0, o.ws[4] >= 0 ? reinterpret_cast<double*>(at(ws, o.ws[4])) : nullptr, cscale, pscale,
                             stream);
        break;
      }
      case OP_SE_MLP_BWD: {
        const lhn_buf& b = P->bufs[o.out_buf];
        rc = lhn_se_mlp_bwd2(reinterpret_cast<const float*>(at(ws, o.ws[0])), prm<const float>(params, o.p[0]),
                             prm<const float>(params, o.p[1]), reinterpret_cast<const float*>(at(ws, o.ws[1])),
                             reinterpret_cast<const float*>(at(ws, o.ws[3])), reinterpret_cast<float*>(at(ws, b.dpool_off)), b.C,
                             o.out_coff, b.H, b.W, prm<float>(grads, o.p[2]), prm<float>(grads, o.p[3]), prm<float>(grads, o.p[4]),
                             prm<float>(grads, o.p[5]), b.N, o.out_C, o.i[0], o.i[1], stream);
        break;
      }
      case OP_CBAM: {
        lhn_view p = mkview(P, ws, o.in_buf[0], o.in_coff[0], o.in_C[0]), r = mkview(P, ws, o.in_buf[1], o.in_coff[1], o.in_C[1]);
        lhn_view y = mkview(P, ws, o.out_buf, o.out_coff, o.out_C);
        rc = lhn_cbam_fwd(&p, &r, prm<const float>(params, o.p[0]), prm<const float>(params, o.p[1]), prm<const float>(params, o.p[2]),
                          &y, reinterpret_cast<float*>(at(ws, o.ws[0])), stream);
        break;
      }
      case OP_CBAM_BWD: {
        lhn_view p = mkview(P, ws, o.in_buf[0], o.in_coff[0], o.in_C[0]), r = mkview(P, ws, o.in_buf[1], o.in_coff[1], o.in_C[1]);
        lhn_view y = mkview(P, ws, o.out_buf, o.out_coff, o.out_C);
        rc = lhn_cbam_bwd(&p, &r, prm<const float>(params, o.p[0]), prm<const float>(params, o.p[1]), prm<const float>(params, o.p[2]),
                          &y, reinterpret_cast<const float*>(at(ws, P->bufs[o.out_buf].grad_off)),
                          reinterpret_cast<float*>(at(ws, P->bufs[o.in_buf[0]].grad_off)),
                          reinterpret_cast<float*>(at(ws, P->bufs[o.in_buf[1]].grad_off)), prm<float>(grads, o.p[3]),
                          prm<float>(grads, o.p[4]), prm<float>(grads, o.p[5]), reinterpret_cast<const float*>(at(ws, o.ws[0])),
// ... 112 lines not shown
```

Baseline: 9432 images/s.

## Fuse BN backward sums into stride-2 depthwise backward; add per-wave loader for 32x32 pw bwd

Extends the stride-2 3x3 depthwise backward kernel with a BNS template variant. While it produces dX, the kernel also accumulates the BatchNorm backward reductions (sum of dy and sum of dy*xhat) for the producing BN. The plan detects a dw-stride-2 backward followed by its BN backward and skips that BN's separate reduce pass, so one full read of activations and gradients goes away. Separately, the 32->32 pointwise backward kernel gets a per-wave loading mode that swaps block-wide __syncthreads for wave barriers. Both paths are enabled by default and can be turned off with environment variables. The cost is extra LDS and per-block double atomics, plus more register pressure.

```diff
diff --git a/include/lhn.h b/include/lhn.h
--- a/include/lhn.h
+++ b/include/lhn.h
@@ -366,6 +366,7 @@
 void  lhn_plan_destroy(void* plan);
 int   lhn_plan_head_gate_fold(void* plan);
 int   lhn_plan_pw_dz_dead(void* plan, int bwd_index);
+int   lhn_plan_dws2_bns(void* plan);
 #define LHN_RUN_TABLES_CURRENT 2
 #define LHN_RUN_GRAPH 4
 int   lhn_plan_run(void* plan, int phase, void* workspace, void* const* params, void* const* grads,
diff --git a/litehandnet_amd/_lib.py b/litehandnet_amd/_lib.py
--- a/litehandnet_amd/_lib.py
+++ b/litehandnet_amd/_lib.py
@@ -43,7 +43,7 @@
     "lhn_loss_balanced_mse_fwd", "lhn_loss_balanced_mse_bwd", "lhn_affine_warp_normalize", "lhn_affine_warp_normalize2", "lhn_random_flip", "lhn_hsv_jitter", "lhn_simdr_encode", "lhn_simdr_loss_fwd", "lhn_simdr_loss_bwd",
     "lhn_conv_pw_fwd", "lhn_conv_pw_fwd2", "lhn_conv_pw_bwd2", "lhn_conv_dw_fwd", "lhn_conv_dw_fwd2", "lhn_conv_dw_fwd3", "lhn_conv_pw_dw3_fwd", "lhn_conv_dw3_pw_fwd", "lhn_msrb_round_scratch_bytes", "lhn_msrb_round_fwd", "lhn_bottleneck_fwd", "lhn_stem_tail_fwd", "lhn_conv_stem_fwd", "lhn_conv_kxk_fwd", "lhn_conv_kxk_fwd_bf16x3",
     "lhn_bn_finalize", "lhn_table_fill", "lhn_table_bias", "lhn_fold_bn", "lhn_ew_fwd", "lhn_ew_fwd2", "lhn_ew_fwd3", "lhn_ew_mul_bwd", "lhn_bilinear_bwd", "lhn_shuffle2_fwd", "lhn_shuffle2_bwd", "lhn_bn_finalize2", "lhn_bn_bwd_finalize2", "lhn_maxpool2_fwd", "lhn_avgpool_fwd", "lhn_avgpool_fwd2", "lhn_avgpool_bwd2", "lhn_se_mlp_fwd2", "lhn_se_mlp_bwd2", "lhn_ca_mlp_fwd", "lhn_att_mlp_fwd", "lhn_att_mlp_bwd", "lhn_se_mlp_fwd", "lhn_se_mlp_bwd",
-    "lhn_bn_bwd_reduce", "lhn_bn_bwd_finalize", "lhn_conv_pw_bwd", "lhn_conv_dw_bwd", "lhn_conv_dw_bwd2", "lhn_conv_dw_bwd3", "lhn_conv_dw_bwd4", "lhn_conv_pw_bwd4", "lhn_conv_pw_bwd5", "lhn_conv_pw_bwd6", "lhn_plan_head_gate_fold", "lhn_plan_pw_dz_dead", "lhn_conv_stem_bwd",
+    "lhn_bn_bwd_reduce", "lhn_bn_bwd_finalize", "lhn_conv_pw_bwd", "lhn_conv_dw_bwd", "lhn_conv_dw_bwd2", "lhn_conv_dw_bwd3", "lhn_conv_dw_bwd4", "lhn_conv_pw_bwd4", "lhn_conv_pw_bwd5", "lhn_conv_pw_bwd6", "lhn_plan_head_gate_fold", "lhn_plan_pw_dz_dead", "lhn_plan_dws2_bns", "lhn_conv_stem_bwd",
     "lhn_conv_kxk_bwd", "lhn_ew_bwd", "lhn_ew_bwd2", "lhn_maxpool2_bwd", "lhn_maxpool2_bwd2", "lhn_maxpool2_bwd3", "lhn_ew_bwd3", "lhn_ew_bwd_multi", "lhn_avgpool_bwd3", "lhn_conv_pw_bwd3", "lhn_avgpool_bwd", "lhn_gate_bwd_reduce", "lhn_gate_bwd_reduce2", "lhn_gate_bwd_reduce3", "lhn_adam_step", "lhn_avgpool_fwd3", "lhn_avgpool_fwd4", "lhn_ca_mlp_bwd2",
     "lhn_ca_mlp_bwd", "lhn_reduce_replicas", "lhn_fold_stat_replicas", "lhn_plan_create", "lhn_plan_destroy", "lhn_plan_run", "lhn_plan_run_range",
     "lhn_cbam_layout", "lhn_cbam_fwd", "lhn_cbam_bwd",
diff --git a/litehandnet_amd/csrc/k_conv_dw.hip b/litehandnet_amd/csrc/k_conv_dw.hip
--- a/litehandnet_amd/csrc/k_conv_dw.hip
+++ b/litehandnet_amd/csrc/k_conv_dw.hip
@@ -386,7 +386,7 @@
 struct DwBnSum;
 static int dws2_fwd(const lhn_view* x, const float* w, const lhn_view* y, double* stats, lhn_bnfin fin, hipStream_t s);
 static int dws2_bwd(const lhn_view* x, const float* w, const lhn_view* y, const lhn_gradview* gy, float* dx, int dx_acc, float* dw,
-                    int nrep, int64_t rep_stride, hipStream_t s);
+                    int nrep, int64_t rep_stride, hipStream_t s, const DwBnSum* bsp = nullptr);
 int lhn_dwk_bwd_lds(const lhn_view* x, const float* w, const lhn_view* y, const lhn_gradview* gy, float* dx, int dx_acc,
                     float* dw, int k, int dil, int nrep, int64_t rep_stride, hipStream_t s, const DwBnSum* bs,
                     const lhn_bnbwdsrc* fs = nullptr);
@@ -877,6 +877,9 @@
 static int dw_bwd_fused(const lhn_view* x, const float* w, const lhn_view* y, const lhn_gradview* gy, float* dx, float* dw, int k,
                         int dil, int nrep, int64_t rep_stride, double* bn_sums, const float* bn_save, int bn_C, int bn_coff, hipStream_t s);
 
+static int dws2_bwd_fused(const lhn_view* x, const float* w, const lhn_view* y, const lhn_gradview* gy, float* dx, float* dw, int nrep,
+                          int64_t rep_stride, double* bn_sums, const float* bn_save, int bn_C, int bn_coff, hipStream_t s);
+
 extern "C" int lhn_conv_dw_bwd2(const lhn_view* x, const float* w, const lhn_view* y, const lhn_gradview* gy, float* dx,
                                 int dx_accumulate, float* dw, int k, int stride, int pad, int dil, int nrep, int64_t rep_stride,
                                 double* bn_sums, const float* bn_save, int bn_C, int bn_coff, void* stream) {
@@ -884,6 +887,15 @@
   if (nrep < 1) nrep = 1;
   LHN_CHECK_ARG(lhn_view_ok(x) && lhn_view_ok(y) && gy && gy->dz && w && dw && dx && bn_save && lhn_no_pend(x) && lhn_no_pend(y),
                 "lhn_conv_dw_bwd2: bad view / null pointer");
+  if (stride == 2) {
+    LHN_CHECK_ARG(!dx_accumulate && !x->gate && k == 3 && pad == 1 && dil == 1 && x->C == y->C && x->C <= 512 && bn_coff >= 0 &&
+                      bn_coff + x->C <= bn_C && y->H == (x->H + 1) / 2 && y->W == (x->W + 1) / 2,
+                  "lhn_conv_dw_bwd2: fused BatchNorm sums at stride 2 need a 3x3 / pad 1 convolution that is the only, ungated reader of x (dx stored)");
+    const int rc = dws2_bwd_fused(x, w, y, gy, dx, dw, nrep, rep_stride, bn_sums, bn_save, bn_C, bn_coff, (hipStream_t)stream);
+    LHN_CHECK_ARG(rc == 1, "lhn_conv_dw_bwd2: cannot reserve the stride-2 tile kernel's LDS");
+    LHN_CHECK_LAUNCH("lhn_conv_dw_bwd2");
+    return 0;
+  }
   LHN_CHECK_ARG(!dx_accumulate && !x->gate && stride == 1 && pad == dil * (k - 1) / 2 && x->C % 32 == 0 && x->W >= 8 && x->C == y->C &&
                     bn_coff >= 0 && bn_coff + x->C <= bn_C,
                 "lhn_conv_dw_bwd2: fused BatchNorm sums need this convolution to be the only, ungated, stride-1 reader of x (dx stored)");
@@ -1835,14 +1847,17 @@
   }
 }
 
+template <bool BNS = false>
 __global__ void __launch_bounds__(256, 2) k_dws2_bwd_lds(lhn_view x, const float* __restrict__ w, lhn_view y, lhn_gradview gy,
                                                       float* __restrict__ dx, int dx_acc, float* __restrict__ dw, int tiles_h,
-                                                      int tiles_w, int cgroups, int nrep, int64_t rep_stride) {
+                                                      int tiles_w, int cgroups, int nrep, int64_t rep_stride, DwBnSum bs) {
   using T = DwS2;
   extern __shared__ __attribute__((aligned(16))) float smem[];
   f4* tx = reinterpret_cast<f4*>(smem);
   f4* tdy = tx + T::XPIX * 8;
   f4* wl = tdy + T::DPIX * 8;
+  f4* tmi = wl + 72;
+  f4* cst = tmi + 16;
   const int tid = threadIdx.x, c4 = tid & 7, pl = tid >> 3;
   const int ntile = y.N * tiles_h * tiles_w * cgroups;
   const int cg = blockIdx.x % cgroups;
@@ -1850,16 +1865,52 @@
   const bool cok = c4 < cvalid;
   const int c4e = cok ? c4 : 0;
   const int cx = x.coff + cg * 32 + 4 * c4e, cy = y.coff + cg * 32 + 4 * c4e;
-  const Xf4 xxf = lhn_load_xf(x, cx), yxf = lhn_load_xf(y, cy);
-  const Gr4 ygr = lhn_load_coef(gy, y.cstride, cy);
+  Xf4 xxf_r, yxf_r;
+  Gr4 ygr_r;
+  if (!BNS) {
+    xxf_r = lhn_load_xf(x, cx);
+    yxf_r = lhn_load_xf(y, cy);
+    ygr_r = lhn_load_coef(gy, y.cstride, cy);
+  }
+  auto xf_of = [&](int kind0, const Xf4& reg) __attribute__((always_inline)) {
+    if (!BNS) return reg;
+    Xf4 t;
+    t.sc = cst[kind0 * 8 + c4];
+    t.sh = cst[(kind0 + 1) * 8 + c4];
+    t.sl = cst[(kind0 + 2) * 8 + c4];
+    return t;
+  };
   for (int i = tid; i < 72; i += 256) {
     const int k = i >> 3, cc = cg * 32 + 4 * min(i & 7, cvalid - 1);
     wl[i] = (f4){w[(cc + 0) * 9 + k], w[(cc + 1) * 9 + k], w[(cc + 2) * 9 + k], w[(cc + 3) * 9 + k]};
   }
+  if (BNS && tid < 16) {
+    const int kind = tid >> 3, cc = min(tid & 7, cvalid - 1);
+    tmi[tid] = *reinterpret_cast<const f4*>(bs.save + kind * bs.C + bs.coff + cg * 32 + 4 * cc);
+  } else if (BNS && tid >= 64 && tid < 64 + 72) {
+    const int i = tid - 64, kind = i >> 3, ca = cg * 32 + 4 * min(i & 7, cvalid - 1), j = kind % 3;
+    const f4 z = (f4){0.f, 0.f, 0.f, 0.f}, one = (f4){1.f, 1.f, 1.f, 1.f};
+    const float* tab = kind < 3 ? x.table : kind < 6 ? y.table : gy.coef;
+    const int cs = kind < 3 ? x.cstride : y.cstride, co = kind < 3 ? x.coff : y.coff;
+    cst[i] = tab ? *reinterpret_cast<const f4*>(tab + j * cs + co + ca) : ((kind < 6 ? j != 1 : j == 0) ? one : z);
+  }
   f4 accw[9];
 #pragma unroll
   for (int k = 0; k < 9; ++k) accw[k] = (f4){0.f, 0.f, 0.f, 0.f};
+  double sdu[4] = {0, 0, 0, 0}, sdux[4] = {0, 0, 0, 0};
   constexpr int NITX = (T::XPIX + 31) / 32, NITD = (T::DPIX + 31) / 32;
+  static_assert(NITX == T::XH + 1 && T::XW == 33, "BNS load order: XH rows of columns 1 .. 32, then column 0");
+  auto xpos = [&](int it, int& ph, int& pw) __attribute__((always_inline)) {
+    if (BNS) {
+      ph = it < T::XH ? it : min(pl, T::XH - 1);
+      pw = it < T::XH ? pl + 1 : 0;
+      return it < T::XH || pl < T::XH;
+    }
+    const int i = min(pl + 32 * it, T::XPIX - 1);
+    ph = i / T::XW;
+    pw = i - ph * T::XW;
+    return pl + 32 * it < T::XPIX;
+  };
   for (int t = blockIdx.x; t < ntile; t += gridDim.x) {
     int r = t / cgroups;
     const int tw = r % tiles_w;
@@ -1871,8 +1922,8 @@
     f4 rx[NITX], ry[NITD], rz[NITD];
 #pragma unroll
     for (int it = 0; it < NITX; ++it) {
-      const int i = min(pl + 32 * it, T::XPIX - 1);
-      const int ph = i / T::XW, pw = i - ph * T::XW;
+      int ph, pw;
+      (void)xpos(it, ph, pw);
       const int ih = min(max(h0 + ph, 0), x.H - 1), iw = min(max(w0 + pw, 0), x.W - 1);
       rx[it] = *reinterpret_cast<const f4*>(x.data + ((size_t)(n * x.H + ih) * x.W + iw) * x.cstride + cx);
     }
@@ -1886,15 +1937,22 @@
       rz[it] = *reinterpret_cast<const f4*>(gy.dz + off);
     }
     __syncthreads();
+    const Xf4 xxf = xf_of(0, xxf_r);
 #pragma unroll
     for (int it = 0; it < NITX; ++it) {
-      const int i = pl + 32 * it;
-      if (i < T::XPIX) {
-        const int ph = i / T::XW, pw = i - ph * T::XW;
+      int ph, pw;
+      if (xpos(it, ph, pw)) {
         const int ih = h0 + ph, iw = w0 + pw;
         const bool inb = ih >= 0 && ih < x.H && iw >= 0 && iw < x.W;
-        tx[i * 8 + c4] = inb ? lhn_apply_xf(rx[it], xxf) * xgate : (f4){0.f, 0.f, 0.f, 0.f};
-      }
+        tx[(ph * T::XW + pw) * 8 + c4] = inb ? lhn_apply_xf(rx[it], xxf) * xgate : (f4){0.f, 0.f, 0.f, 0.f};
+      }
+    }
+    const Xf4 yxf = xf_of(3, yxf_r);
+    Gr4 ygr = ygr_r;
+    if (BNS) {
+      ygr.A = cst[48 + c4];
+      ygr.B = cst[56 + c4];
+      ygr.Cc = cst[64 + c4];
     }
 #pragma unroll
     for (int it = 0; it < NITD; ++it) {
@@ -1940,6 +1998,17 @@
               accx += d0[colA * 8] * wl[(0 + bA) * 8 + c4] + d2[colA * 8] * wl[(6 + bA) * 8 + c4];
               if (nb == 2) accx += d0[colB * 8] * wl[(0 + 2) * 8 + c4] + d2[colB * 8] * wl[(6 + 2) * 8 + c4];
             }
+            if (BNS) {
+              const f4 raw = rx[rr + 1], da = lhn_dact_xf(raw, xf_of(0, xxf_r)), mean = tmi[c4], inv = tmi[8 + c4];
+              const float av[4] = {accx.x, accx.y, accx.z, accx.w}, dv[4] = {da.x, da.y, da.z, da.w}, rv[4] = {raw.x, raw.y, raw.z, raw.w};
+              const float mv[4] = {mean.x, mean.y, mean.z, mean.w}, iv[4] = {inv.x, inv.y, inv.z, inv.w};
+#pragma unroll
+              for (int j = 0; j < 4; ++j) {
+                const double du = (double)av[j] * (double)dv[j];
+                sdu[j] += du;
+                sdux[j] += du * (((double)rv[j] - (double)mv[j]) * (double)iv[j]);
+              }
+            }
             float* o = dx + ((size_t)(n * x.H + ih) * x.W + iw) * x.cstride + cx;
             if (dx_acc) accx += *reinterpret_cast<const f4*>(o);
             *reinterpret_cast<f4*>(o) = accx;
@@ -1947,6 +2016,10 @@
         }
       }
     }
+  }
+  if (BNS) {
+    double* sts = bs.sums + (size_t)((blockIdx.x / cgroups) % LHN_STAT_REPLICAS) * 2 * bs.C + bs.coff + cg * 32;
+    lhn_block_stat_atomics_d(sdu, sdux, 8, reinterpret_cast<double*>(tdy), sts, sts + bs.C, cvalid);
   }
   float* dwr = dw + (size_t)((blockIdx.x / cgroups) % nrep) * rep_stride;
 #pragma unroll
@@ -1986,16 +2059,25 @@
   hipLaunchKernelGGL(k_dws2_fwd_lds, dim3(dw3_grid(ntile, cg, 6)), dim3(256), lds, s, *x, w, *y, stats, th, tw, cg, fin);
   return 1;
 }
-static int dws2_bwd(const lhn_view* x, const float* w, const lhn_view* y, const lhn_gradview* gy, float* dx, int dx_acc, float* dw,
-                    int nrep, int64_t rep_stride, hipStream_t s) {
+template <bool BNS>
+static int launch_dws2_bwd(const lhn_view* x, const float* w, const lhn_view* y, const lhn_gradview* gy, float* dx, int dx_acc, float* dw,
+                           int nrep, int64_t rep_stride, hipStream_t s, const DwBnSum& bs) {
   using T = DwS2;
   const int cg = (x->C + 31) / 32;
   const int th = (y->H + T::TH - 1) / T::TH, tw = (y->W + T::TW - 1) / T::TW, ntile = y->N * th * tw * cg;
-  const size_t lds = (size_t)((T::XPIX + T::DPIX) * 8 + 72) * 16;
+  const size_t lds = (size_t)((T::XPIX + T::DPIX) * 8 + 72 + (BNS ? 16 + 72 : 0)) * 16;
   static LhnKernelCfg cfg;
-  if (!lhn_kernel_cfg(cfg, &k_dws2_bwd_lds, lds, 4, nullptr)) return 0;
-  hipLaunchKernelGGL(k_dws2_bwd_lds, dim3(dw3_grid(ntile, cg, 4)), dim3(256), lds, s, *x, w, *y, *gy, dx, dx_acc, dw, th, tw, cg, nrep, rep_stride);
+  if (!lhn_kernel_cfg(cfg, &k_dws2_bwd_lds<BNS>, lds, 4, nullptr)) return 0;
+  hipLaunchKernelGGL(k_dws2_bwd_lds<BNS>, dim3(dw3_grid(ntile, cg, 4)), dim3(256), lds, s, *x, w, *y, *gy, dx, dx_acc, dw, th, tw, cg, nrep,
+                     rep_stride, bs);
   return 1;
+}
+static int dws2_bwd(const lhn_view* x, const float* w, const lhn_view* y, const lhn_gradview* gy, float* dx, int dx_acc, float* dw,
+                    int nrep, int64_t rep_stride, hipStream_t s, const DwBnSum* bsp) {
+  if (bsp && bsp->sums) return launch_dws2_bwd<true>(x, w, y, gy, dx, dx_acc, dw, nrep, rep_stride, s, *bsp);
+  DwBnSum bs;
+  bs.sums = nullptr; bs.save = nullptr; bs.C = bs.coff = 0; bs.add[0] = bs.add[1] = nullptr;
+  return launch_dws2_bwd<false>(x, w, y, gy, dx, dx_acc, dw, nrep, rep_stride, s, bs);
 }
 
 int lhn_dwk_fwd_lds(const lhn_view* x, const float* w, const lhn_view* y, double* stats, int k, int dil, lhn_bnfin fin,
@@ -2080,6 +2162,17 @@
   return lhn_dwk_bwd_lds(x, w, y, gy, dx, dx_acc, dw, k, dil, nrep, rep_stride, s, &bs, fin);
 }
 
+static int dws2_bwd_fused(const lhn_view* x, const float* w, const lhn_view* y, const lhn_gradview* gy, float* dx, float* dw, int nrep,
+                          int64_t rep_stride, double* bn_sums, const float* bn_save, int bn_C, int bn_coff, hipStream_t s) {
+  DwBnSum bs;
+  bs.sums = bn_sums;
+  bs.save = bn_save;
+  bs.C = bn_C;
+  bs.coff = bn_coff;
+  bs.add[0] = bs.add[1] = nullptr;
+  return dws2_bwd(x, w, y, gy, dx, 0, dw, nrep, rep_stride, s, &bs);
+}
+
 static int dw_bwd_fused(const lhn_view* x, const float* w, const lhn_view* y, const lhn_gradview* gy, float* dx, float* dw, int k,
                         int dil, int nrep, int64_t rep_stride, double* bn_sums, const float* bn_save, int bn_C, int bn_coff, hipStream_t s) {
   DwBnSum bs;
diff --git a/litehandnet_amd/csrc/k_conv_pw.hip b/litehandnet_amd/csrc/k_conv_pw.hip
--- a/litehandnet_amd/csrc/k_conv_pw.hip
+++ b/litehandnet_amd/csrc/k_conv_pw.hip
@@ -933,7 +933,7 @@
   return launch_pw_bwd_t<CIN, NTO, false>(x, w, y, gy, dx, dx_acc, dw, dbias, stride, dy_nchw, cout, nrep, rep_stride, geo, s, bs);
 }
 
-template <int CIN, int COUT, int PX, int PF, bool DYST, bool BNS, int OCC>
+template <int CIN, int COUT, int PX, int PF, bool DYST, bool BNS, int OCC, bool WL = false>
 __global__ void __launch_bounds__(256, OCC) k_pw_bwd_wr(lhn_view x, const float* __restrict__ w, lhn_view y, lhn_gradview gy,
                                                         float* __restrict__ dx, int dx_acc, float* __restrict__ dw, float* __restrict__ dbias,
                                                         int M, int ntiles, int nrep, int64_t rep_stride, lhn_bnsum bs, lhn_bnbwdsrc fs) {
@@ -946,6 +946,7 @@
   static_assert(ONE ? (NTO == 1 && PX == 128) : ((NTI == 2 || NTI == 4) && (NTO == 2 || NTO == 4) && (PX == 64 || (PX == 32 && NTI == 4))),
                 "32 -> 32 at 128 pixels; 64 / 128 channels on either side at 64 (or 32) pixels");
   static_assert(!BNS || NDX == 1, "reader-side sums: one dX sub-tile per wave");
+  static_assert(!WL || ONE, "per-wave loader: the instance whose waves consume their own 32 rows of the tile");
   extern __shared__ __attribute__((aligned(16))) float smem[];
   float* dYs = smem;
   float* Xs = dYs + PX * LDY;
@@ -962,17 +963,19 @@
   constexpr int ZCH = YPF < 4 ? YPF : 4;
   const int xc4 = tid % XC4, xr0 = tid / XC4, xabs = x.coff + 4 * xc4;
   const int yc4 = tid % YC4, yr0 = tid / YC4, yabs = y.coff + 4 * yc4;
+  auto xrow = [&](int p) __attribute__((always_inline)) { return WL ? 32 * wave + (lane >> 3) + 8 * p : xr0 + p * XRP; };
+  auto yrow = [&](int p) __attribute__((always_inline)) { return WL ? 32 * wave + (lane >> 3) + 8 * p : yr0 + p * YRP; };
 
   f4 xraw[XPF], yraw[YPF], ydz[YPF];
   auto issue = [&](int tile) __attribute__((always_inline)) {
 #pragma unroll
     for (int p = 0; p < XPF; ++p) {
-      const int m = min(tile * PX + xr0 + p * XRP, M - 1);
+      const int m = min(tile * PX + xrow(p), M - 1);
       xraw[p] = *reinterpret_cast<const f4*>(x.data + (int64_t)m * x.cstride + xabs);
     }
 #pragma unroll
     for (int p = 0; p < YPF; ++p) {
-      const int m = min(tile * PX + yr0 + p * YRP, M - 1);
+      const int m = min(tile * PX + yrow(p), M - 1);
       if (PF >= 1) yraw[p] = *reinterpret_cast<const f4*>(y.data + (int64_t)m * y.cstride + yabs);
       if (PF >= 2) ydz[p] = *reinterpret_cast<const f4*>(gy.dz + (int64_t)m * y.cstride + yabs);
     }
@@ -985,7 +988,7 @@
     xxf.sl = *reinterpret_cast<const f4*>(xt + 2 * CIN + 4 * xc4);
 #pragma unroll
     for (int p = 0; p < XPF; ++p) {
-      const int row = xr0 + p * XRP, m = tile * PX + row;
+      const int row = xrow(p), m = tile * PX + row;
       f4 v = (f4){0.f, 0.f, 0.f, 0.f};
       if (m < M) {
         v = lhn_apply_xf(xraw[p], xxf);
@@ -1007,12 +1010,12 @@
       if (PF < 2 && p % ZCH == 0) {
 #pragma unroll
         for (int q = p; q < p + ZCH; ++q) {
-          const int mq = min(tile * PX + yr0 + q * YRP, M - 1);
+          const int mq = min(tile * PX + yrow(q), M - 1);
           if (PF < 1) yraw[q] = *reinterpret_cast<const f4*>(y.data + (int64_t)mq * y.cstride + yabs);
           ydz[q] = *reinterpret_cast<const f4*>(gy.dz + (int64_t)mq * y.cstride + yabs);
         }
       }
-      const int row = yr0 + p * YRP, m = tile * PX + row;
+      const int row = yrow(p), m = tile * PX + row;
       f4 v = (f4){0.f, 0.f, 0.f, 0.f};
       if (m < M) {
         int n = 0, h = 0, ww = 0;
@@ -1085,9 +1088,17 @@
   }
   __syncthreads();
 
+  auto tile_sync = [&]() __attribute__((always_inline)) {
+    if (WL) {
+      __builtin_amdgcn_fence(__ATOMIC_ACQ_REL, "wavefront");
+      __builtin_amdgcn_wave_barrier();
+    } else {
+      __syncthreads();
+    }
+  };
   for (; tile < ntiles; tile += gridDim.x) {
     commit(tile);
-    __syncthreads();
+    tile_sync();
     if (tile + (int)gridDim.x < ntiles) issue(tile + gridDim.x);
     {
       const float* ap = dYs + ((ONE ? 32 * wave : 0) + lh) * LDY + l31 + (ONE ? 0 : 32 * (wave / NTI));
@@ -1159,8 +1170,9 @@
         }
       }
     }
-    __syncthreads();
-  }
+    tile_sync();
+  }
+  if (WL) __syncthreads();
 
   if (BNS) {
     float* bred = Xs;
@@ -1222,7 +1234,7 @@
   }
 }
 
-template <int CIN, int COUT, int PX, int PF, bool DYST = true, bool BNS = false, int OCC = 2>
+template <int CIN, int COUT, int PX, int PF, bool DYST = true, bool BNS = false, int OCC = 2, bool WL = false>
 static int launch_pw_bwd_wr(const lhn_view* x, const float* w, const lhn_view* y, const lhn_gradview* gy, float* dx, int dx_acc, float* dw,
                             float* dbias, int nrep, int64_t rep_stride, hipStream_t s, const lhn_bnsum& bs, const lhn_bnbwdsrc* fsp = nullptr) {
   const int M = y->N * y->H * y->W, ntiles = (M + PX - 1) / PX;
@@ -1231,13 +1243,13 @@
   const size_t lds = (size_t)(PX * (COUT + 4) + PX * (CIN + 4) + 3 * CIN + 6 * COUT + (BNS ? PX * CIN : 0)) * sizeof(float);
   static LhnKernelCfg cfg;
   int per_cu = 1;
-  if (!lhn_kernel_cfg(cfg, &k_pw_bwd_wr<CIN, COUT, PX, PF, DYST, BNS, OCC>, lds, OCC, &per_cu)) {
+  if (!lhn_kernel_cfg(cfg, &k_pw_bwd_wr<CIN, COUT, PX, PF, DYST, BNS, OCC, WL>, lds, OCC, &per_cu)) {
     lhn_set_error("lhn_conv_pw_bwd: cannot reserve %zu B of LDS", lds);
     return 2;
   }
   int grid = lhn_num_cus() * per_cu;
   if (grid > ntiles) grid = ntiles;
-  hipLaunchKernelGGL((k_pw_bwd_wr<CIN, COUT, PX, PF, DYST, BNS, OCC>), dim3(grid), dim3(256), lds, s, *x, w, *y, *gy, dx, dx_acc, dw, dbias,
+  hipLaunchKernelGGL((k_pw_bwd_wr<CIN, COUT, PX, PF, DYST, BNS, OCC, WL>), dim3(grid), dim3(256), lds, s, *x, w, *y, *gy, dx, dx_acc, dw, dbias,
                      M, ntiles, nrep, rep_stride, bs, fs);
   return 0;
 }
@@ -1249,6 +1261,15 @@
     off = (e && e[0] == '0') ? 1 : 0;
   }
   return off == 1;
+}
+
+static bool pw_bwd_waveload() {
+  static int v = -1;
+  if (v < 0) {
+    const char* e = getenv("LHN_PW_BWD_WAVELOAD");
+    v = (e && e[0] == '0') ? 0 : 1;
+  }
+  return v == 1;
 }
 
 static bool pw_bwd_split_forced() {
@@ -1366,6 +1387,9 @@
     int rc;
     if (Cin == 64) rc = bs.sums ? launch_pw_bwd_wr<64, 64, 64, 2, false, true>(x, w, y, gy, dx, dx_accumulate, dw, dbias, nrep, rep_stride, s, bs, fin)
                                 : launch_pw_bwd_wr<64, 64, 64, 2, false, false>(x, w, y, gy, dx, dx_accumulate, dw, dbias, nrep, rep_stride, s, bs, fin);
+    else if (pw_bwd_waveload())
+      rc = bs.sums ? launch_pw_bwd_wr<32, 32, 128, 2, false, true, 2, true>(x, w, y, gy, dx, dx_accumulate, dw, dbias, nrep, rep_stride, s, bs, fin)
+                   : launch_pw_bwd_wr<32, 32, 128, 2, false, false, 3, true>(x, w, y, gy, dx, dx_accumulate, dw, dbias, nrep, rep_stride, s, bs, fin);
     else rc = bs.sums ? launch_pw_bwd_wr<32, 32, 128, 2, false, true>(x, w, y, gy, dx, dx_accumulate, dw, dbias, nrep, rep_stride, s, bs, fin)
                       : launch_pw_bwd_wr<32, 32, 128, 2, false, false, 3>(x, w, y, gy, dx, dx_accumulate, dw, dbias, nrep, rep_stride, s, bs, fin);
     if (rc) return rc;
diff --git a/litehandnet_amd/csrc/lhn_plan.cpp b/litehandnet_amd/csrc/lhn_plan.cpp
--- a/litehandnet_amd/csrc/lhn_plan.cpp
+++ b/litehandnet_amd/csrc/lhn_plan.cpp
@@ -38,6 +38,7 @@
   std::vector<lhn_buf> bufs;
   std::vector<lhn_op> fwd, bwd;
   std::vector<uint8_t> pw_dz_dead;
+  std::vector<uint8_t> dws2_bns;
   std::vector<GraphEntry> graphs;
   uint64_t tick = 0;
   int graph_misses = 0;
@@ -123,6 +124,24 @@
   const lhn_buf& b = P->bufs[o.in_buf[0]];
   return o.in_coff[0] == 0 && o.in_C[0] == b.C && b.gate_off >= 0 && nx.kind == OP_GATE_REDUCE && nx.out_buf == o.in_buf[0] &&
          nx.out_coff == 0 && nx.out_C == b.C && nx.ws[3] >= 0 && nx.ws[4] >= 0;
+}
+static bool dws2_bns_on() {
+  static int v = -1;
+  if (v < 0) {
+    const char* e = getenv("LHN_DWS2_BNS");
+    v = (e && e[0] == '0') ? 0 : 1;
+  }
+  return v == 1;
+}
+static bool dws2_bns_at(const Plan* P, const std::vector<lhn_op>& ops, size_t oi) {
+  if (!dws2_bns_on() || fuse_finalize() || oi + 1 >= ops.size()) return false;
+  const lhn_op &o = ops[oi], &nx = ops[oi + 1];
+  if (o.kind != OP_DW_BWD || o.i[0] != 3 || o.i[1] != 2 || o.i[2] != 1 || o.i[3] != 1 || o.i[4] != 1 || o.in_buf[0] < 0) return false;
+  if (o.p[0] < 0 || o.p[1] < 0 || o.ws[2] >= 0 || o.ws[3] >= 0 || o.ws[4] >= 0 || o.ws[5] >= 0) return false;
+  const lhn_buf& b = P->bufs[o.in_buf[0]];
+  return o.in_coff[0] == 0 && o.in_C[0] == b.C && b.C <= 512 && b.gate_off < 0 && b.dpool_off < 0 && b.grad_off >= 0 &&
+         nx.kind == OP_BN_BWD && nx.out_buf == o.in_buf[0] && nx.out_coff == 0 && nx.out_C == b.C && !nx.i[0] && !nx.i[1] &&
+         nx.ws[0] >= 0 && nx.ws[1] >= 0;
 }
 static bool pw_bwd_dy_store() {
   static int v = -1;
@@ -196,6 +215,8 @@
     }
   p->pw_dz_dead.resize(p->bwd.size());
   for (size_t oi = 0; oi < p->bwd.size(); ++oi) p->pw_dz_dead[oi] = pw_dz_dead_at(p, p->bwd, oi) ? 1 : 0;
+  p->dws2_bns.resize(p->bwd.size());
+  for (size_t oi = 0; oi < p->bwd.size(); ++oi) p->dws2_bns[oi] = dws2_bns_at(p, p->bwd, oi) ? 1 : 0;
   return p;
 }
 
@@ -211,6 +232,14 @@
   const Plan* p = static_cast<const Plan*>(plan);
   if (!p || bwd_index < 0 || (size_t)bwd_index >= p->pw_dz_dead.size()) return -1;
   return p->pw_dz_dead[bwd_index];
+}
+
+int lhn_plan_dws2_bns(void* plan) {
+  const Plan* p = static_cast<const Plan*>(plan);
+  if (!p) return -1;
+  int n = 0;
+  for (uint8_t v : p->dws2_bns) n += v;
+  return n;
 }
 
 void lhn_plan_destroy(void* plan) {
@@ -600,9 +629,10 @@
         lhn_view y = mkview(P, ws, o.out_buf, o.out_coff, o.out_C);
         lhn_gradview g = mkgrad(P, ws, o.out_buf, o.i[5] != 0);
         float* dx = o.i[4] ? reinterpret_cast<float*>(at(ws, P->bufs[o.in_buf[0]].grad_off)) : nullptr;
+        const lhn_op* s2 = (phase == 1 && whole && P->dws2_bns[oi]) ? &ops[oi + 1] : nullptr;
         if (cfin_for == oi) {
           const bool adds = o.ws[2] >= 0 || o.ws[3] >= 0;
-          const lhn_bnsum bs = mkbns(ws, adds ? -1 : o.ws[4], adds ? -1 : o.ws[5], o.i[6], o.i[7]);
+          const lhn_bnsum bs = s2 ? mkbns(ws, s2->ws[0], s2->ws[1], s2->out_C, 0) : mkbns(ws, adds ? -1 : o.ws[4], adds ? -1 : o.ws[5], o.i[6], o.i[7]);
           rc = lhn_conv_dw_bwd4(&x, prm<const float>(params, o.p[0]), &y, &g, dx, o.i[4] == 2, prm<float>(grads, o.p[1]), o.i[0], o.i[1],
                                 o.i[2], o.i[3], nrep, rstr, bs.sums ? &bs : nullptr,
                                 o.ws[2] >= 0 ? reinterpret_cast<const float*>(at(ws, o.ws[2])) : nullptr,
@@ -613,6 +643,12 @@
           rc = lhn_conv_dw_bwd3(&x, prm<const float>(params, o.p[0]), &y, &g, dx, o.i[4] == 2, prm<float>(grads, o.p[1]), o.i[0], o.i[1],
                                 o.i[2], o.i[3], nrep, rstr, o.ws[2] >= 0 ? reinterpret_cast<const float*>(at(ws, o.ws[2])) : nullptr,
                                 o.ws[3] >= 0 ? reinterpret_cast<const float*>(at(ws, o.ws[3])) : nullptr, stream);
+          break;
+        }
+        if (s2) {
+          rc = lhn_conv_dw_bwd2(&x, prm<const float>(params, o.p[0]), &y, &g, dx, 0, prm<float>(grads, o.p[1]), o.i[0], o.i[1], o.i[2],
+                                o.i[3], nrep, rstr, reinterpret_cast<double*>(at(ws, s2->ws[0])),
+                                reinterpret_cast<const float*>(at(ws, s2->ws[1])), s2->out_C, 0, stream);
           break;
         }
         rc = lhn_conv_dw_bwd2(&x, prm<const float>(params, o.p[0]), &y, &g, dx, o.i[4] == 2, prm<float>(grads, o.p[1]), o.i[0],
@@ -646,7 +682,8 @@
         if (fin.counter && fuse_finalize() && whole && !o.i[1]) {
           rc = lhn_bn_bwd_reduce(&y, &g, save, sums, &fin, stream);
         } else {
-          if (h0 && !o.i[1]) rc = lhn_bn_bwd_reduce(&y, &g, save, sums, nullptr, stream);
+          const bool by_dws2 = phase == 1 && whole && oi > 0 && P->dws2_bns[oi - 1];
+          if (h0 && !o.i[1] && !by_dws2) rc = lhn_bn_bwd_reduce(&y, &g, save, sums, nullptr, stream);
           const lhn_op* nx = oi + 1 < ops.size() ? &ops[oi + 1] : nullptr;
           if (!rc && h1 && whole && bwd_fin_consumer() && !fuse_finalize() && o.i[0] == 0 && nx &&
               (nx->kind == OP_DW_BWD || (nx->kind == OP_PW_BWD && !nx->i[1])) && nx->out_buf == o.out_buf && nx->out_coff == o.out_coff &&
```

New measurement: 9504 images/s (median of 6 runs). No clear change (+0.8%).
